# tumaer/lagrangebench

Measured on AMD Instinct MI355X. Metric: rollout particle-steps/sec, higher is better.
Workload: dtype f32 (GEMMs as fp16 hi/lo split products, fp32 accumulate)

## Files before the change

include/lbhip.h:

```cpp
#ifndef LBHIP_H
#define LBHIP_H

#include <stdint.h>

#ifdef __cplusplus
extern "C" {
#endif

#define LB_OK 0
#define LB_ERR_ARG (-1)
#define LB_ERR_HIP (-2)
#define LB_ERR_STATE (-3)
#define LB_ERR_DENSITY (-4)
#define LB_ERR_UNSUPPORTED (-5)

#define LB_FORCE_NONE 0
#define LB_FORCE_PIECEWISE 1
#define LB_FORCE_BUFFER 2

typedef struct lb_engine lb_engine;
typedef struct lb_gns lb_gns;

typedef struct lb_case_desc {
  int32_t dim;
  int32_t n_particles;
  int32_t batch;
  int32_t isl;
  int32_t periodic;
  int32_t has_bound;
  int32_t has_vel_mag;
  int32_t force_kind;
  int32_t force_axis;
  int32_t geometry_f32;
  double box[3];
  double r_cutoff;
  double capacity_multiplier;
  double vel_mean[3], vel_std[3], acc_mean[3], acc_std[3];
  double bound_lo[3], bound_hi[3];
  double force_split;
  double force_lo[3], force_hi[3];
} lb_case_desc;

typedef struct lb_gns_desc {
  int32_t latent_size;
  int32_t blocks_per_step;
  int32_t num_mp_steps;
  int32_t embedding_size;
  int32_t num_particle_types;
  int32_t node_in;
  int32_t edge_in;
  int32_t out_dim;
} lb_gns_desc;

const char* lb_strerror(int code);
const char* lb_last_error(void);
int lb_version(void);


int lb_engine_create(const lb_case_desc* desc, void* hip_stream, lb_engine** out);
void lb_engine_destroy(lb_engine* eng);

int lb_set_particle_type(lb_engine* eng, const int32_t* ptype_dev);

int lb_set_force(lb_engine* eng, const double* force_dev);

int lb_load_window(lb_engine* eng, const double* traj_dev, int32_t T, int32_t t0, int32_t step);

#define LB_TRAIN_BATCH_MAX 128
int lb_train_batch(lb_engine* eng, const void* pos_dev, int32_t pos_is_f64, const int32_t* ptype_dev, int32_t n_traj,
                   int32_t seq_len, const int32_t* traj_host, const int32_t* t0_host, const int32_t* slot_host,
                   uint64_t seed, int64_t step, double noise_std, int32_t T, int32_t unroll_steps, double* traj_out_dev,
                   int32_t* ptype_out_dev, double* target_acc_dev, double* target_vel_dev, double* target_pos_dev,
                   double* want_normals_dev);

int lb_read_window(lb_engine* eng, double* win_out_dev);


int lb_nl_allocate(lb_engine* eng, int32_t* cell_capacity_out, int32_t* e_cap_out,
                   int32_t* occupancy_out );

int lb_nl_set_capacity(lb_engine* eng, int32_t cell_capacity, int32_t e_cap);

int lb_nl_update(lb_engine* eng);

int lb_nl_read_flags(lb_engine* eng, int32_t* overflow_out_dev);

int lb_nl_read_idx(lb_engine* eng, int32_t* idx_out_dev, int32_t* n_edges_out_dev);


int lb_node_features(lb_engine* eng, double* vel_hist_out_dev, double* vel_mag_out_dev,
                     double* bound_out_dev, double* force_out_dev);

int lb_edge_features(lb_engine* eng, double* rel_disp_out_dev, double* rel_dist_out_dev);


int lb_gns_create(lb_engine* eng, const lb_gns_desc* desc, const float* weights_host,
                  int64_t n_floats, lb_gns** out);
void lb_gns_destroy(lb_gns* gns);

int lb_gns_forward(lb_engine* eng, lb_gns* gns, float* acc_out_dev);

int lb_set_fused_aggregation(lb_engine* eng, int32_t on);

int lb_gns_set_tap(lb_gns* gns, float* node_latents_out_dev);


int lb_integrate(lb_engine* eng, const float* acc_dev, const double* target_dev,
                 double* pred_out_dev, int32_t pred_T);

int lb_case_integrate(lb_engine* eng, int32_t mode, const float* pred_dev, const double* pos_seq_dev,
                      int32_t T, double* next_out_dev);

int lb_rollout(lb_engine* eng, lb_gns* gns, const double* traj_dev, int32_t T, int32_t n_steps,
               double* pred_out_dev, int32_t* n_realloc_out);


typedef struct lb_gns_train lb_gns_train;
int lb_gns_train_create(lb_engine* eng, const lb_gns_desc* desc, const float* weights_host, int64_t n_floats,
                        lb_gns_train** out);
void lb_gns_train_destroy(lb_gns_train* t);
int lb_gns_train_loss_grad(lb_gns_train* t, const float* target_dev, float loss_weight, double* loss_out,
                           float* pred_out_dev);
int lb_gns_train_zero_grad(lb_gns_train* t);
int lb_adamw_step(lb_gns_train* t, float lr, float b1, float b2, float eps, float weight_decay);
int lb_gns_train_read(lb_gns_train* t, int32_t which, float* out_host, int64_t n_floats);
int lb_gns_train_write(lb_gns_train* t, int32_t which, const float* in_host, int64_t n_floats, int64_t step);
int64_t lb_gns_train_step_count(lb_gns_train* t);
int lb_gns_train_device_blob(lb_gns_train* t, int32_t which, float** dev_out, int64_t* n_floats_out);
int lb_adamw_step_gathered(lb_gns_train* t, const float* gathered_dev, int32_t world, float grad_scale, float lr,
                           float b1, float b2, float eps, float weight_decay);
int32_t lb_gns_train_math_fallbacks(lb_gns_train* t);
int32_t lb_gns_train_sort_fallbacks(lb_gns_train* t);

int lb_train_forward(lb_gns_train* t, float* pred_out_dev);
int lb_train_backward(lb_gns_train* t, const float* dpred_dev, double* dpos_out_dev);
int lb_train_exact_math(lb_gns_train* t, int32_t exact);

int lb_gns_train_sync_model(lb_gns_train* t, lb_gns* g);
int64_t lb_gns_image_bytes(lb_gns* g);
int lb_gns_image_read(lb_gns* g, void* out_host, int64_t n_bytes);
int64_t lb_gns_pack_selftest(const lb_gns_desc* desc, int32_t node_in_kq, const float* weights_host, int64_t n_floats,
                             int64_t* n_bytes_out);

typedef struct lb_segnn lb_segnn;

typedef struct lb_segnn_desc {
  int32_t hidden;
  int32_t blocks_per_step;
  int32_t num_mp_steps;
  int32_t homogeneous;
  int32_t n_vels;
  int32_t velocity_avg;
  int32_t lmax_hidden;
  int32_t lmax_attributes;
  int32_t norm;
  float norm_eps;
} lb_segnn_desc;

int lb_segnn_create(lb_engine* eng, const lb_segnn_desc* desc, const float* weights_host,
                    int64_t n_floats, lb_segnn** out);

int lb_segnn_train_create(lb_engine* eng, const lb_segnn_desc* desc, const float* weights_host, int64_t n_floats,
                          lb_gns_train** out);
int lb_segnn_train_loss_grad(lb_gns_train* t, const float* target_dev, float loss_weight, double* loss_out,
                             float* pred_out_dev);
void lb_segnn_destroy(lb_segnn* segnn);

int lb_segnn_forward(lb_engine* eng, lb_segnn* segnn, float* acc_out_dev);

typedef struct lb_egnn lb_egnn;
typedef struct lb_egnn_desc {
  int32_t hidden;
  int32_t num_mp_steps;
  int32_t n_vels;
  int32_t homogeneous;
  int32_t residual;
  int32_t normalize;
  int32_t tanh_pos;
} lb_egnn_desc;

int lb_egnn_create(lb_engine* eng, const lb_egnn_desc* desc, const float* weights_host, int64_t n_floats,
                   lb_egnn** out);
void lb_egnn_destroy(lb_egnn* egnn);
int lb_egnn_forward(lb_engine* eng, lb_egnn* egnn, double* pos_out_dev);
int lb_egnn_set_tap(lb_egnn* egnn, float* h_out_dev, float* pos_out_dev);
int lb_egnn_rollout(lb_engine* eng, lb_egnn* egnn, const double* traj_dev, int32_t T, int32_t n_steps,
                    double* pred_out_dev, int32_t* n_realloc_out);

int lb_egnn_train_create(lb_engine* eng, const lb_egnn_desc* desc, const float* weights_host, int64_t n_floats,
                         lb_gns_train** out);
int lb_egnn_train_loss_grad(lb_gns_train* t, const double* tgt_pos, const double* tgt_vel, const double* tgt_acc,
                            float w_pos, float w_vel, float w_acc, double* loss_out, float* pred_pos_out_dev);
int lb_egnn_train_model(lb_gns_train* t, lb_egnn** out);

typedef struct lb_painn lb_painn;
typedef struct lb_painn_desc {
  int32_t hidden;
  int32_t num_mp_steps;
  int32_t n_vels;
  int32_t homogeneous;
  int32_t shared_filters;
  int32_t shared_interactions;
  int32_t n_rbf;
  int32_t has_cutoff;
  float cutoff;
} lb_painn_desc;

int lb_painn_create(lb_engine* eng, const lb_painn_desc* desc, const float* weights_host, int64_t n_floats,
                    lb_painn** out);
void lb_painn_destroy(lb_painn* painn);
int lb_painn_forward(lb_engine* eng, lb_painn* painn, float* acc_out_dev);
int lb_painn_set_tap(lb_painn* painn, float* s_out_dev, float* v_out_dev);
int lb_painn_rollout(lb_engine* eng, lb_painn* painn, const double* traj_dev, int32_t T, int32_t n_steps,
                     double* pred_out_dev, int32_t* n_realloc_out);

int lb_painn_train_create(lb_engine* eng, const lb_painn_desc* desc, const float* weights_host, int64_t n_floats,
                          int32_t rbf_trainable, lb_gns_train** out);
int lb_painn_train_model(lb_gns_train* t, lb_painn** out);

typedef struct lb_linear lb_linear;
typedef struct lb_linear_desc {
  int32_t n_in;
  int32_t out_dim;
} lb_linear_desc;

int lb_linear_create(lb_engine* eng, const lb_linear_desc* desc, const float* weights_host, int64_t n_floats,
                     lb_linear** out);
void lb_linear_destroy(lb_linear* linear);
int lb_linear_forward(lb_engine* eng, lb_linear* linear, float* acc_out_dev);
int lb_linear_rollout(lb_engine* eng, lb_linear* linear, const double* traj_dev, int32_t T, int32_t n_steps,
                      double* pred_out_dev, int32_t* n_realloc_out);
int lb_linear_train_create(lb_engine* eng, const lb_linear_desc* desc, const float* weights_host, int64_t n_floats,
                           lb_gns_train** out);
int lb_linear_train_model(lb_gns_train* t, lb_linear** out);

int lb_blob_train_create(lb_engine* eng, const float* weights_host, int64_t n_floats, lb_gns_train** out);

int lb_math_mode(lb_engine* eng, int32_t set_mode, int32_t* mode_out, int32_t* flags_out);

int32_t lb_math_fallbacks(lb_engine* eng);

int lb_debug_inject_guard(lb_engine* eng, int32_t flags, int32_t step);

int lb_segnn_set_tap(lb_segnn* segnn, float* hidden_out_dev);
int32_t lb_segnn_row_floats(lb_segnn* segnn);

int lb_segnn_rollout(lb_engine* eng, lb_segnn* segnn, const double* traj_dev, int32_t T,
                     int32_t n_steps, double* pred_out_dev, int32_t* n_realloc_out);

int lb_metrics(lb_engine* eng, const double* pred_dev, int32_t pred_T, const double* target_dev,
               int32_t target_T, int32_t n_steps, double* mse_out_dev, double* mae_out_dev);

int lb_ekin(lb_engine* eng, const double* rollout_dev, int32_t T, int32_t stride, double dt, double dx,
            double* out_dev, int32_t n_out);

int lb_sinkhorn(lb_engine* eng, const double* pred_dev, int32_t pred_T, const double* target_dev,
                int32_t target_T, int32_t stride, double threshold, double* out_dev, int32_t n_out,
                int32_t* iters_out_host);

int lb_sinkhorn_pot(lb_engine* eng, const double* pred_dev, int32_t pred_T, const double* target_dev,
                    int32_t target_T, int32_t stride, double reg, int32_t num_iter_max, double stop_thr,
                    double* out_dev, int32_t n_out, int32_t* info_out_host);


int lb_timers_enable(lb_engine* eng, int32_t on);
int lb_timers_reset(lb_engine* eng);
int32_t lb_timer_count(void);
const char* lb_timer_name(int32_t cls);
int lb_timer_get(lb_engine* eng, int32_t cls, double* ms_out, int64_t* launches_out);

int lb_stats(lb_engine* eng, int64_t* n_edges_total, int32_t* e_cap, int32_t* cell_capacity);

int lb_edge_accounting(lb_engine* eng, int64_t* sum_edges, int64_t* n_builds, int64_t* first_edges, int64_t* last_edges,
                       int32_t reset);

int lb_kernel_names(lb_engine* eng, char* out, int32_t cap);

int lb_segment_sum(lb_engine* eng, const float* msg_dev, float* out_dev, int32_t D);

int lb_graph_gather(lb_engine* eng, int32_t role, const float* x_dev , float* out_dev , int32_t C);
int lb_graph_segment_sum(lb_engine* eng, int32_t role, const float* msg_dev , float* out_dev ,
                         int32_t C);
int lb_graph_degree(lb_engine* eng, int32_t role, int32_t* out_dev );
int lb_graph_segment_max(lb_engine* eng, int32_t role, const float* msg_dev , float* out_dev ,
                         int32_t* win_dev , int32_t C);
int lb_graph_segment_min(lb_engine* eng, int32_t role, const float* msg_dev , float* out_dev ,
                         int32_t* win_dev , int32_t C);
int lb_graph_segment_max_backward(lb_engine* eng, int32_t role, const float* d_out_dev ,
                                  const int32_t* win_dev , float* d_msg_dev , int32_t C);
int lb_graph_segment_softmax(lb_engine* eng, int32_t role, const float* logits_dev ,
                             float* out_dev , int32_t C);
int lb_graph_segment_softmax_backward(lb_engine* eng, int32_t role, const float* y_dev ,
                                      const float* d_y_dev , float* d_x_dev , int32_t C);
int lb_graph_attend(lb_engine* eng, int32_t role, const float* logits_dev ,
                    const float* values_dev , float* out_dev , float* m_dev ,
// ... 11 lines not shown
```

lagrangebench_amd/_lib.py:

```python
from __future__ import annotations

import ctypes as C
import os
from typing import Optional

_HERE = os.path.dirname(os.path.abspath(__file__))
LIB_PATH = os.path.join(_HERE, "csrc", "liblbhip.so")

LB_OK = 0
LB_FORCE_NONE, LB_FORCE_PIECEWISE, LB_FORCE_BUFFER = 0, 1, 2
LB_TRAIN_BATCH_MAX = 128

D3 = C.c_double * 3


class CaseDesc(C.Structure):

    _fields_ = [
        ("dim", C.c_int32), ("n_particles", C.c_int32), ("batch", C.c_int32), ("isl", C.c_int32),
        ("periodic", C.c_int32), ("has_bound", C.c_int32), ("has_vel_mag", C.c_int32),
        ("force_kind", C.c_int32), ("force_axis", C.c_int32), ("geometry_f32", C.c_int32),
        ("box", D3), ("r_cutoff", C.c_double), ("capacity_multiplier", C.c_double),
        ("vel_mean", D3), ("vel_std", D3), ("acc_mean", D3), ("acc_std", D3),
        ("bound_lo", D3), ("bound_hi", D3),
        ("force_split", C.c_double), ("force_lo", D3), ("force_hi", D3),
    ]


class GnsDesc(C.Structure):

    _fields_ = [
        ("latent_size", C.c_int32), ("blocks_per_step", C.c_int32), ("num_mp_steps", C.c_int32),
        ("embedding_size", C.c_int32), ("num_particle_types", C.c_int32), ("node_in", C.c_int32),
        ("edge_in", C.c_int32), ("out_dim", C.c_int32),
    ]


class SegnnDesc(C.Structure):

    _fields_ = [
        ("hidden", C.c_int32), ("blocks_per_step", C.c_int32), ("num_mp_steps", C.c_int32),
        ("homogeneous", C.c_int32), ("n_vels", C.c_int32), ("velocity_avg", C.c_int32),
        ("lmax_hidden", C.c_int32), ("lmax_attributes", C.c_int32), ("norm", C.c_int32), ("norm_eps", C.c_float),
    ]

    def __init__(self, *args, **kw):
        super().__init__(*args, **kw)
        if "lmax_hidden" not in kw and len(args) < 7:
            self.lmax_hidden = 1
        if "lmax_attributes" not in kw and len(args) < 8:
            self.lmax_attributes = 1


class EgnnDesc(C.Structure):

    _fields_ = [
        ("hidden", C.c_int32), ("num_mp_steps", C.c_int32), ("n_vels", C.c_int32), ("homogeneous", C.c_int32),
        ("residual", C.c_int32), ("normalize", C.c_int32), ("tanh_pos", C.c_int32),
    ]


class PainnDesc(C.Structure):

    _fields_ = [
        ("hidden", C.c_int32), ("num_mp_steps", C.c_int32), ("n_vels", C.c_int32), ("homogeneous", C.c_int32),
        ("shared_filters", C.c_int32), ("shared_interactions", C.c_int32), ("n_rbf", C.c_int32),
        ("has_cutoff", C.c_int32), ("cutoff", C.c_float),
    ]


class LinearDesc(C.Structure):

    _fields_ = [("n_in", C.c_int32), ("out_dim", C.c_int32)]


_P = C.c_void_p
_SIGS = {
    "lb_strerror": (C.c_char_p, [C.c_int]),
    "lb_last_error": (C.c_char_p, []),
    "lb_version": (C.c_int, []),
    "lb_engine_create": (C.c_int, [C.POINTER(CaseDesc), _P, C.POINTER(_P)]),
    "lb_engine_destroy": (None, [_P]),
    "lb_set_particle_type": (C.c_int, [_P, _P]),
    "lb_set_force": (C.c_int, [_P, _P]),
    "lb_load_window": (C.c_int, [_P, _P, C.c_int32, C.c_int32, C.c_int32]),
    "lb_train_batch": (C.c_int, [_P, _P, C.c_int32, _P, C.c_int32, C.c_int32, C.POINTER(C.c_int32), C.POINTER(C.c_int32),
                                 C.POINTER(C.c_int32), C.c_uint64, C.c_int64, C.c_double, C.c_int32, C.c_int32, _P, _P, _P, _P, _P,
                                 _P]),
    "lb_read_window": (C.c_int, [_P, _P]),
    "lb_nl_allocate": (C.c_int, [_P, C.POINTER(C.c_int32), C.POINTER(C.c_int32), C.POINTER(C.c_int32)]),
    "lb_nl_set_capacity": (C.c_int, [_P, C.c_int32, C.c_int32]),
    "lb_nl_update": (C.c_int, [_P]),
    "lb_nl_read_flags": (C.c_int, [_P, _P]),
    "lb_nl_read_idx": (C.c_int, [_P, _P, _P]),
    "lb_node_features": (C.c_int, [_P, _P, _P, _P, _P]),
    "lb_edge_features": (C.c_int, [_P, _P, _P]),
    "lb_gns_create": (C.c_int, [_P, C.POINTER(GnsDesc), _P, C.c_int64, C.POINTER(_P)]),
    "lb_gns_destroy": (None, [_P]),
    "lb_gns_forward": (C.c_int, [_P, _P, _P]),
    "lb_set_fused_aggregation": (C.c_int, [_P, C.c_int32]),
    "lb_gns_set_tap": (C.c_int, [_P, _P]),
    "lb_math_mode": (C.c_int, [_P, C.c_int32, C.POINTER(C.c_int32), C.POINTER(C.c_int32)]),
    "lb_math_fallbacks": (C.c_int32, [_P]),
    "lb_debug_inject_guard": (C.c_int, [_P, C.c_int32, C.c_int32]),
    "lb_integrate": (C.c_int, [_P, _P, _P, _P, C.c_int32]),
    "lb_case_integrate": (C.c_int, [_P, C.c_int32, _P, _P, C.c_int32, _P]),
    "lb_rollout": (C.c_int, [_P, _P, _P, C.c_int32, C.c_int32, _P, C.POINTER(C.c_int32)]),
    "lb_ekin": (C.c_int, [_P, _P, C.c_int32, C.c_int32, C.c_double, C.c_double, _P, C.c_int32]),
    "lb_sinkhorn": (C.c_int, [_P, _P, C.c_int32, _P, C.c_int32, C.c_int32, C.c_double, _P, C.c_int32, _P]),
    "lb_sinkhorn_pot": (C.c_int, [_P, _P, C.c_int32, _P, C.c_int32, C.c_int32, C.c_double, C.c_int32, C.c_double, _P,
                                  C.c_int32, _P]),
    "lb_metrics": (C.c_int, [_P, _P, C.c_int32, _P, C.c_int32, C.c_int32, _P, _P]),
    "lb_timers_enable": (C.c_int, [_P, C.c_int32]),
    "lb_timers_reset": (C.c_int, [_P]),
    "lb_timer_count": (C.c_int32, []),
    "lb_timer_name": (C.c_char_p, [C.c_int32]),
    "lb_timer_get": (C.c_int, [_P, C.c_int32, C.POINTER(C.c_double), C.POINTER(C.c_int64)]),
    "lb_stats": (C.c_int, [_P, C.POINTER(C.c_int64), C.POINTER(C.c_int32), C.POINTER(C.c_int32)]),
    "lb_edge_accounting": (C.c_int, [_P, C.POINTER(C.c_int64), C.POINTER(C.c_int64), C.POINTER(C.c_int64),
                                     C.POINTER(C.c_int64), C.c_int32]),
    "lb_kernel_names": (C.c_int, [_P, C.c_char_p, C.c_int32]),
    "lb_gns_train_create": (C.c_int, [_P, C.POINTER(GnsDesc), C.POINTER(C.c_float), C.c_int64, C.POINTER(_P)]),
    "lb_gns_train_destroy": (None, [_P]),
    "lb_gns_train_loss_grad": (C.c_int, [_P, _P, C.c_float, C.POINTER(C.c_double), _P]),
    "lb_gns_train_zero_grad": (C.c_int, [_P]),
    "lb_adamw_step": (C.c_int, [_P, C.c_float, C.c_float, C.c_float, C.c_float, C.c_float]),
    "lb_gns_train_read": (C.c_int, [_P, C.c_int32, C.POINTER(C.c_float), C.c_int64]),
    "lb_gns_train_write": (C.c_int, [_P, C.c_int32, C.POINTER(C.c_float), C.c_int64, C.c_int64]),
    "lb_gns_train_step_count": (C.c_int64, [_P]),
    "lb_gns_train_device_blob": (C.c_int, [_P, C.c_int32, C.POINTER(_P), C.POINTER(C.c_int64)]),
    "lb_adamw_step_gathered": (C.c_int, [_P, _P, C.c_int32, C.c_float, C.c_float, C.c_float, C.c_float, C.c_float,
                                         C.c_float]),
    "lb_gns_train_math_fallbacks": (C.c_int32, [_P]),
    "lb_gns_train_sort_fallbacks": (C.c_int32, [_P]),
    "lb_train_forward": (C.c_int, [_P, _P]),
    "lb_train_backward": (C.c_int, [_P, _P, _P]),
    "lb_train_exact_math": (C.c_int, [_P, C.c_int32]),
    "lb_gns_train_sync_model": (C.c_int, [_P, _P]),
    "lb_gns_image_bytes": (C.c_int64, [_P]),
    "lb_gns_image_read": (C.c_int, [_P, _P, C.c_int64]),
    "lb_gns_pack_selftest": (C.c_int64, [C.POINTER(GnsDesc), C.c_int32, C.POINTER(C.c_float), C.c_int64, C.POINTER(C.c_int64)]),
    "lb_segnn_train_create": (C.c_int, [_P, C.POINTER(SegnnDesc), C.POINTER(C.c_float), C.c_int64, C.POINTER(_P)]),
    "lb_segnn_train_loss_grad": (C.c_int, [_P, _P, C.c_float, C.POINTER(C.c_double), _P]),
    "lb_segment_sum": (C.c_int, [_P, _P, _P, C.c_int32]),
    "lb_segnn_create": (C.c_int, [_P, C.POINTER(SegnnDesc), _P, C.c_int64, C.POINTER(_P)]),
    "lb_segnn_destroy": (None, [_P]),
    "lb_segnn_forward": (C.c_int, [_P, _P, _P]),
    "lb_segnn_row_floats": (C.c_int32, [_P]),
    "lb_segnn_set_tap": (C.c_int, [_P, _P]),
    "lb_segnn_rollout": (C.c_int, [_P, _P, _P, C.c_int32, C.c_int32, _P, C.POINTER(C.c_int32)]),
    "lb_egnn_create": (C.c_int, [_P, C.POINTER(EgnnDesc), C.POINTER(C.c_float), C.c_int64, C.POINTER(_P)]),
    "lb_egnn_destroy": (None, [_P]),
    "lb_egnn_forward": (C.c_int, [_P, _P, _P]),
    "lb_egnn_set_tap": (C.c_int, [_P, _P, _P]),
    "lb_egnn_rollout": (C.c_int, [_P, _P, _P, C.c_int32, C.c_int32, _P, C.POINTER(C.c_int32)]),
    "lb_egnn_train_create": (C.c_int, [_P, C.POINTER(EgnnDesc), C.POINTER(C.c_float), C.c_int64, C.POINTER(_P)]),
    "lb_egnn_train_loss_grad": (C.c_int, [_P, _P, _P, _P, C.c_float, C.c_float, C.c_float, C.POINTER(C.c_double), _P]),
    "lb_egnn_train_model": (C.c_int, [_P, C.POINTER(_P)]),
    "lb_painn_create": (C.c_int, [_P, C.POINTER(PainnDesc), C.POINTER(C.c_float), C.c_int64, C.POINTER(_P)]),
    "lb_painn_destroy": (None, [_P]),
    "lb_painn_forward": (C.c_int, [_P, _P, _P]),
    "lb_painn_set_tap": (C.c_int, [_P, _P, _P]),
    "lb_painn_rollout": (C.c_int, [_P, _P, _P, C.c_int32, C.c_int32, _P, C.POINTER(C.c_int32)]),
    "lb_painn_train_create": (C.c_int, [_P, C.POINTER(PainnDesc), C.POINTER(C.c_float), C.c_int64, C.c_int32, C.POINTER(_P)]),
    "lb_painn_train_model": (C.c_int, [_P, C.POINTER(_P)]),
    "lb_linear_create": (C.c_int, [_P, C.POINTER(LinearDesc), C.POINTER(C.c_float), C.c_int64, C.POINTER(_P)]),
    "lb_linear_destroy": (None, [_P]),
    "lb_linear_forward": (C.c_int, [_P, _P, _P]),
    "lb_linear_rollout": (C.c_int, [_P, _P, _P, C.c_int32, C.c_int32, _P, C.POINTER(C.c_int32)]),
    "lb_linear_train_create": (C.c_int, [_P, C.POINTER(LinearDesc), C.POINTER(C.c_float), C.c_int64, C.POINTER(_P)]),
    "lb_linear_train_model": (C.c_int, [_P, C.POINTER(_P)]),
    "lb_blob_train_create": (C.c_int, [_P, C.POINTER(C.c_float), C.c_int64, C.POINTER(_P)]),
    "lb_graph_gather": (C.c_int, [_P, C.c_int32, _P, _P, C.c_int32]),
    "lb_graph_segment_sum": (C.c_int, [_P, C.c_int32, _P, _P, C.c_int32]),
    "lb_graph_sender_sorts": (C.c_int32, [_P]),
    "lb_graph_degree": (C.c_int, [_P, C.c_int32, _P]),
    "lb_graph_segment_max": (C.c_int, [_P, C.c_int32, _P, _P, _P, C.c_int32]),
    "lb_graph_segment_min": (C.c_int, [_P, C.c_int32, _P, _P, _P, C.c_int32]),
    "lb_graph_segment_max_backward": (C.c_int, [_P, C.c_int32, _P, _P, _P, C.c_int32]),
    "lb_graph_segment_softmax": (C.c_int, [_P, C.c_int32, _P, _P, C.c_int32]),
    "lb_graph_segment_softmax_backward": (C.c_int, [_P, C.c_int32, _P, _P, _P, C.c_int32]),
    "lb_graph_attend": (C.c_int, [_P, C.c_int32, _P, _P, _P, _P, _P, C.c_int32, C.c_int32]),
    "lb_graph_attend_backward": (C.c_int, [_P, C.c_int32, _P, _P, _P, _P, _P, _P, _P, C.c_int32, C.c_int32]),
}

_lib: Optional[C.CDLL] = None


class LbHipError(RuntimeError):
    pass


def load() -> C.CDLL:
    global _lib
    if _lib is not None:
        return _lib
    if not os.path.exists(LIB_PATH):
        raise LbHipError(
            f"{LIB_PATH} not found: the HIP engine is not built. Run "
            "`python -m lagrangebench_amd.build` (needs hipcc). There is no CPU fallback."
        )
    lib = C.CDLL(LIB_PATH)
    for name, (res, args) in _SIGS.items():
        fn = getattr(lib, name)
        fn.restype = res
        fn.argtypes = args
    _lib = lib
    return lib


def check(rc: int, what: str = "") -> None:
    if rc != LB_OK:
        lib = load()
        msg = lib.lb_last_error().decode() or lib.lb_strerror(rc).decode()
        raise LbHipError(f"{what or 'liblbhip'} failed ({rc}: {lib.lb_strerror(rc).decode()}): {msg}")


def ptr(t) -> int:
    if t is None:
        return None
    return t.data_ptr()
```

lagrangebench_amd/csrc/lb_edge16.hip:

```cpp
#include <stdlib.h>
#include <string.h>

#include "lb_device.h"
#include "lb_gns_repack.h"

#define MFMA16(a, b, c) __builtin_amdgcn_mfma_f32_16x16x4f32((a), (b), (c), 0, 0, 0)

typedef _Float16 h8 __attribute__((ext_vector_type(8)));
#define MFMA16H(a, b, c) __builtin_amdgcn_mfma_f32_16x16x32_f16((a), (b), (c), 0, 0, 0)


void lb_pack_weight16h(const float* w, int K, int M, int Kpad, float* out, int Mpad) {
  uint16_t* o = reinterpret_cast<uint16_t*>(out);
  const int NP = Kpad / 32, NMBO = Mpad / 16;
  for (int p = 0; p < NP; ++p)
    for (int mbo = 0; mbo < NMBO; ++mbo)
      for (int lane = 0; lane < 64; ++lane)
        for (int i = 0; i < 8; ++i) {
          const int g = lane >> 4;
          const int k = 32 * p + (i < 4 ? 4 * g + i : 16 + 4 * g + (i - 4));
          const int m = 16 * mbo + (lane & 15);
          const float x = (k < K && m < M) ? w[(size_t)k * M + m] : 0.f;
          const uint16_t hi = lb_f32_to_f16_rne(x);
          const uint16_t lo = lb_f32_to_f16_rne(x - lb_f16_to_f32(hi));
// ... 85 lines not shown
      a0 = n0;
      a1 = n1;
      __builtin_amdgcn_sched_barrier(0);
    }
  }
}

template <bool PROC, bool F16, int ABL = 0>
__global__ void __launch_bounds__(E16_THREADS, 2) k_edge16(lb_edge16_args a) {
  constexpr int NW0 = PROC ? 4096 : (F16 ? 1024 : 512);
  __shared__ f32x4 sW[NW0 + 4096 + 128];
  if (a.ctrl->overflow_step >= 0) return;
  const int tid = threadIdx.x;
  {
    const f32x4* g0 = reinterpret_cast<const f32x4*>(a.w0p);
    const f32x4* g1 = reinterpret_cast<const f32x4*>(a.w1p);
    for (int i = tid; i < NW0; i += E16_THREADS) sW[i] = g0[i];
    for (int i = tid; i < 4096; i += E16_THREADS) sW[NW0 + i] = g1[i];
    if (tid < 128) {
      const float* src = tid < 32 ? a.b1 : (tid < 64 ? a.ln_s : (tid < 96 ? a.ln_o : a.b0));
      sW[NW0 + 4096 + tid] = src ? reinterpret_cast<const f32x4*>(src)[tid & 31] : f32x4{0.f, 0.f, 0.f, 0.f};
    }
  }
  __syncthreads();
  const int E = a.ctrl->n_edges_total;
  const int ntiles = (E + 15) >> 4;
  const int lane = tid & 63, wave = tid >> 6;
  const int n = lane & 15, g = lane >> 4;
  const int xcd = blockIdx.x & 7, slot = (blockIdx.x >> 3) * E16_WAVES + wave;
  const int stride = (gridDim.x >> 3) * E16_WAVES;
  const int t_lo = (int)(((int64_t)ntiles * xcd) >> 3), t_hi = (int)(((int64_t)ntiles * (xcd + 1)) >> 3);
  int t = t_lo + slot;
  if (t >= t_hi) return;

  auto ld0 = [&](int step, int hf) -> f32x4 { return sW[(step * 2 + hf) * 64 + lane]; };
  auto ld1 = [&](int step, int hf) -> f32x4 { return sW[NW0 + (step * 2 + hf) * 64 + lane]; };
  auto ldh0 = [&](int p, int mbo, int part) -> f32x4 { return sW[((p * 8 + mbo) * 2 + part) * 64 + lane]; };
  auto ldh1 = [&](int p, int mbo, int part) -> f32x4 {
    return sW[NW0 + ((p * 8 + mbo) * 2 + part) * 64 + lane];
  };
  auto rowc_of = [&](int tt) -> int64_t {
    const int row = tt * 16 + n;
    return row < E ? row : E - 1;
  };
  const f32x4* psr4 = reinterpret_cast<const f32x4*>(a.psr);
  const f32x4* b1_4 = &sW[NW0 + 4096];
  const f32x4* lns4 = &sW[NW0 + 4096 + 32];
  const f32x4* lno4 = &sW[NW0 + 4096 + 64];
  const f32x4* b0_4 = &sW[NW0 + 4096 + 96];

  const int n_iter = (t_hi - 1 - t) / stride + 1;
  const int t_last = t + (n_iter - 1) * stride;
  f32x4 ve_n[8], ps_n[8], pr_n[8];
  f32x4 vin_n = {0.f, 0.f, 0.f, 0.f};
  int s_n = 0, r_n = 0, r_pref = 0;
  auto issue = [&](int tt, int s, int r) {
    const int64_t rc = rowc_of(tt);
    if (PROC) {
      const f32x4* er = reinterpret_cast<const f32x4*>(a.elat) + (int64_t)tt * 512 + lane;
      const f32x4* ps = psr4 + (int64_t)s * 64 + g;
      const f32x4* pr = psr4 + (int64_t)r * 64 + 32 + g;
#pragma unroll
      for (int mb = 0; mb < 8; ++mb) {
        ve_n[mb] = (ABL & 2) ? f32x4{1.f, 2.f, (float)rc, (float)mb} : er[64 * mb];
        ps_n[mb] = (ABL & 1) ? f32x4{.1f, .2f, (float)s, (float)mb} : ps[4 * mb];
        pr_n[mb] = (ABL & 1) ? f32x4{.3f, .1f, (float)r, (float)mb} : pr[4 * mb];
      }
    } else {
      vin_n = reinterpret_cast<const f32x4*>(a.efeat)[rc * 2 + (g & 1)];
    }
  };
  {
    const int64_t rc = rowc_of(t);
    int s0 = 0, r0 = 0;
    if (PROC) {
      s0 = a.senders[rc];
      r0 = a.receivers[rc];
    }
    issue(t, s0, r0);
    r_pref = r0;
    if (PROC) {
      const int64_t rn = rowc_of(min(t + stride, t_last));
      s_n = a.senders[rn];
      r_n = a.receivers[rn];
    }
  }

  for (int it = 0; it < n_iter; ++it, t += stride) {
    f32x4 acc[8], ve[8];
    f32x4 vin[1];
    const int r_cur = r_pref;
    if (PROC) {
#pragma unroll
      for (int mb = 0; mb < 8; ++mb) {
        ve[mb] = ve_n[mb];
        acc[mb] = ps_n[mb] + pr_n[mb];
      }
    } else {
      vin[0] = (g < 2) ? vin_n : f32x4{0.f, 0.f, 0.f, 0.f};
#pragma unroll
      for (int mb = 0; mb < 8; ++mb) acc[mb] = b0_4[4 * mb + g];
    }
    issue(min(t + stride, t_last), s_n, r_n);
    r_pref = r_n;
    if (PROC) {
      const int64_t rn = rowc_of(min(t + 2 * stride, t_last));
      s_n = a.senders[rn];
      r_n = a.receivers[rn];
    }
    if constexpr (ABL & 32) {
    } else if constexpr (F16) {
      if constexpr (PROC) {
        lb_gemm16h<4>(ldh0, ve, acc);
      } else {
        f32x4 vin2[2] = {vin[0], f32x4{0.f, 0.f, 0.f, 0.f}};
        lb_gemm16h<1>(ldh0, vin2, acc);
      }
    } else {
      if (PROC)
        lb_gemm16<8>(ld0, ve, acc);
      else
        lb_gemm16<1>(ld0, vin, acc);
    }
#pragma unroll
    for (int mb = 0; mb < 8; ++mb)
#pragma unroll
      for (int j = 0; j < 4; ++j) acc[mb][j] = fmaxf(acc[mb][j], 0.f);
    f32x4 acc2[8];
#pragma unroll
    for (int mb = 0; mb < 8; ++mb) acc2[mb] = b1_4[4 * mb + g];
    if constexpr (ABL & 16) {
#pragma unroll
      for (int mb = 0; mb < 8; ++mb) acc2[mb] = acc2[mb] + acc[mb];
    } else if constexpr (F16)
      lb_gemm16h<4>(ldh1, acc, acc2);
    else
      lb_gemm16<8>(ld1, acc, acc2);
    float sm = 0.f;
#pragma unroll
    for (int mb = 0; mb < 8; ++mb) sm += (acc2[mb][0] + acc2[mb][1]) + (acc2[mb][2] + acc2[mb][3]);
    sm += __shfl_xor(sm, 16);
    sm += __shfl_xor(sm, 32);
    const float mean = sm * a.ctrl->ln_inv_d;
    float vs = 0.f;
#pragma unroll
    for (int mb = 0; mb < 8; ++mb)
#pragma unroll
      for (int j = 0; j < 4; ++j) {
        const float d = acc2[mb][j] - mean;
        vs += d * d;
      }
    vs += __shfl_xor(vs, 16);
    vs += __shfl_xor(vs, 32);
    const float rs = 1.0f / sqrtf(fmaxf(vs - a.ctrl->ln_pad * (mean * mean), 0.f) * a.ctrl->ln_inv_d + 1e-5f);
    f32x4 y[8];
#pragma unroll
    for (int mb = 0; mb < 8; ++mb) {
      const f32x4 sc = lns4[4 * mb + g], of = lno4[4 * mb + g];
#pragma unroll
      for (int j = 0; j < 4; ++j)
        y[mb][j] = (ABL & 8) ? acc2[mb][j] : (sc[j] * rs) * (acc2[mb][j] - mean) + of[j];
    }
    const int row = t * 16 + n;
    const bool valid = row < E;
    const bool do_store = !((ABL & 4) && a.row_ptr[0] != -12345);
    if (do_store) {
      f32x4* er = reinterpret_cast<f32x4*>(a.elat) + (int64_t)t * 512 + lane;
      if (PROC) {
        if (!a.skip_elat_store) {
#pragma unroll
          for (int mb = 0; mb < 8; ++mb) er[64 * mb] = ve[mb] + y[mb];
        }
        if (!a.fused && valid) {
          f32x4* mr = reinterpret_cast<f32x4*>(a.msg) + (int64_t)row * 32 + g;
#pragma unroll
          for (int mb = 0; mb < 8; ++mb) mr[4 * mb] = y[mb];
        }
      } else {
#pragma unroll
        for (int mb = 0; mb < 8; ++mb) er[64 * mb] = y[mb];
      }
    }
    if (PROC && a.fused && !(ABL & 64)) {
      const int rr = valid ? r_cur : (-1 - n);
      const int r_prev = __builtin_amdgcn_update_dpp(-2, rr, 0x111, 0xF, 0xF, false);
      const bool head = (n == 0) || (rr != r_prev);
      const unsigned H = (unsigned)(__ballot(head) & 0xffffull);
      const unsigned below = H & ((2u << n) - 1u);
      const int segstart = 31 - __clz(below);
      const bool tail = (n == 15) || ((H >> (n + 1)) & 1u);
      const float m1 = (n >= 1 && segstart <= n - 1) ? 1.f : 0.f, m2 = (n >= 2 && segstart <= n - 2) ? 1.f : 0.f;
      const float m4 = (n >= 4 && segstart <= n - 4) ? 1.f : 0.f, m8 = (n >= 8 && segstart <= n - 8) ? 1.f : 0.f;
#pragma unroll
      for (int mb = 0; mb < 8; ++mb)
#pragma unroll
        for (int j = 0; j < 4; ++j) {
          float x = valid ? y[mb][j] : 0.f;
          x = __builtin_fmaf(__builtin_bit_cast(float, __builtin_amdgcn_update_dpp(0, __builtin_bit_cast(int, x), 0x111, 0xF, 0xF, true)), m1, x);
          x = __builtin_fmaf(__builtin_bit_cast(float, __builtin_amdgcn_update_dpp(0, __builtin_bit_cast(int, x), 0x112, 0xF, 0xF, true)), m2, x);
          x = __builtin_fmaf(__builtin_bit_cast(float, __builtin_amdgcn_update_dpp(0, __builtin_bit_cast(int, x), 0x114, 0xF, 0xF, true)), m4, x);
          x = __builtin_fmaf(__builtin_bit_cast(float, __builtin_amdgcn_update_dpp(0, __builtin_bit_cast(int, x), 0x118, 0xF, 0xF, true)), m8, x);
          y[mb][j] = x;
        }
      if (tail && valid && do_store) {
        const int k0 = a.row_ptr[rr], k1 = a.row_ptr[rr + 1];
        const bool complete = (k0 >> 4) == ((k1 - 1) >> 4);
        float* dst = complete ? a.agg + (int64_t)rr * 128
                              : a.part + ((int64_t)t * 2 + (k0 <= t * 16 ? 0 : 1)) * 128;
        f32x4* d4 = reinterpret_cast<f32x4*>(dst) + g;
#pragma unroll
        for (int mb = 0; mb < 8; ++mb) d4[4 * mb] = y[mb];
      }
    }
  }
}

int lbk_edge16(lb_engine* e, const lb_edge16_args& a, bool proc, bool f16x2) {
  if (proc && f16x2)
    hipLaunchKernelGGL((k_edge16<true, true>), dim3(256), dim3(E16_THREADS), 0, e->stream, a);
  else if (proc)
    hipLaunchKernelGGL((k_edge16<true, false>), dim3(256), dim3(E16_THREADS), 0, e->stream, a);
  else
    hipLaunchKernelGGL((k_edge16<false, false>), dim3(256), dim3(E16_THREADS), 0, e->stream, a);
  LB_HIP(hipGetLastError());
  return LB_OK;
}
```

lagrangebench_amd/csrc/lb_edge16v.hip:

```cpp
#include <stdlib.h>

#include "lb_f16x2.h"

template <int WPS, bool RELOAD, bool SKIP, int ABL = 0, bool PRIO = false, bool NT = true, int GUARD = 0, bool TICKET = false>
__global__ void __launch_bounds__(WPS * 256, WPS) k_edge16v(lb_edge16_args a) {
  constexpr int THREADS = WPS * 256, WAVES = WPS * 4;
  constexpr int NW0 = 4096;
  __shared__ f32x4 sW[NW0 + 4096 + 96];
  __shared__ int s_ticket;
  const int poisoned = a.ctrl->overflow_step;
  const int E = a.ctrl->n_edges_total;
  const float ln_inv_d = a.ctrl->ln_inv_d, ln_pad = a.ctrl->ln_pad;
  const int tid = threadIdx.x;
  constexpr int NST = (NW0 + 4096 + THREADS - 1) / THREADS;
  f32x4 st[NST];
  {
    const f32x4* g0 = reinterpret_cast<const f32x4*>(a.w0p);
    const f32x4* g1 = reinterpret_cast<const f32x4*>(a.w1p);
#pragma unroll
    for (int k = 0; k < NST; ++k) {
      const int i = tid + k * THREADS;
      st[k] = i < NW0 ? g0[i] : g1[(i < NW0 + 4096 ? i : NW0 + 4095) - NW0];
    }
  }
  const int ntiles = (E + 15) >> 4;
  const int lane = tid & 63, wave = __builtin_amdgcn_readfirstlane(tid >> 6);
  const int n = lane & 15, g = lane >> 4;
  const int xcd = blockIdx.x & 7;
  int stride = (gridDim.x >> 3) * WAVES;
  int t_lo = (int)(((int64_t)ntiles * xcd) >> 3), t_hi = (int)(((int64_t)ntiles * (xcd + 1)) >> 3);
  int t = t_lo + (blockIdx.x >> 3) * WAVES + wave;
  if constexpr (TICKET) {
    stride = gridDim.x >> 3;
    t_lo += (blockIdx.x >> 3);
    t = t_lo + wave * stride;
  }
  auto rowc_of = [&](int tt) -> int64_t {
    const int row = tt * 16 + n;
    return row < E ? row : (E > 0 ? E - 1 : 0);
  };
  int s_c = 0, r_c = 0;
  if (t < t_hi) {
    const int64_t rc = rowc_of(t);
    s_c = a.senders[rc];
    r_c = a.receivers[rc];
  }
  if (poisoned >= 0) return;
  {
#pragma unroll
    for (int k = 0; k < NST; ++k) {
      const int i = tid + k * THREADS;
      if (i < NW0 + 4096) sW[i] = st[k];
    }
    if (tid < 96) {
      const float* src = tid < 32 ? a.b1 : (tid < 64 ? a.ln_s : a.ln_o);
      sW[NW0 + 4096 + tid] = reinterpret_cast<const f32x4*>(src)[tid & 31];
    }
    if (TICKET && tid == 0) s_ticket = WAVES;
  }
  __syncthreads();
  if (t >= t_hi) return;
  uint32_t off0 = (uint32_t)(uintptr_t)(lds_cptr)(sW + lane);
  uint32_t off1 = (uint32_t)(uintptr_t)(lds_cptr)(sW + NW0 + lane);
  uint32_t off2 = (uint32_t)(uintptr_t)(lds_cptr)(sW + NW0 + 4096 + g);
  asm volatile("" : "+v"(off0), "+v"(off1), "+v"(off2));
  const lds_cptr w0b = (lds_cptr)(uintptr_t)off0, w1b = (lds_cptr)(uintptr_t)off1, vecb = (lds_cptr)(uintptr_t)off2;
  const f32x4* psr4 = reinterpret_cast<const f32x4*>(a.psr);
  const int n_iter = TICKET ? 0x7fffffff : (t_hi - 1 - t) / stride + 1;
  const int t_last = TICKET ? t_hi - 1 : t + (n_iter - 1) * stride;
  asm volatile("" : "+v"(s_c), "+v"(r_c));
  int guard_tiny = 0;
  for (int it = 0; it < n_iter && t < t_hi; ++it) {
    int t_next = t + stride;
    if constexpr (TICKET) {
      int k = 0;
      if (lane == 0) k = atomicAdd(&s_ticket, 1);
      t_next = t_lo + __builtin_amdgcn_readfirstlane(k) * stride;
    }
    f32x4 acc[8], ve[8];
    const int r_cur = r_c;
    const f32x4* er = reinterpret_cast<const f32x4*>(a.elat) + (int64_t)t * 512 + lane;
    {
      const f32x4* ps = psr4 + (int64_t)s_c * 64 + g;
      const f32x4* pr = psr4 + (int64_t)r_c * 64 + 32 + g;
      f32x4 p0[8];
#pragma unroll
      for (int mb = 0; mb < 8; ++mb) {
        ve[mb] = (ABL & 2) ? f32x4{1.f, 2.f, (float)(t & 1023), (float)mb}
                           : ((RELOAD || !NT) ? er[64 * mb] : __builtin_nontemporal_load(&er[64 * mb]));
        p0[mb] = (ABL & 1) ? f32x4{.1f, .2f, (float)(s_c & 255), (float)mb} : ps[4 * mb];
        acc[mb] = (ABL & 1) ? f32x4{.3f, .1f, (float)(r_c & 255), (float)mb} : pr[4 * mb];
      }
      const int64_t rn = rowc_of(min(t_next, t_last));
      s_c = a.senders[rn];
      r_c = a.receivers[rn];
#pragma unroll
      for (int mb = 0; mb < 8; ++mb) acc[mb] = lb_pk_add(acc[mb], p0[mb]);
    }
    int rb = lb_edge_probe(a.receivers, t, lane, E);
    if (it == 0) lb_range_probe(a.ctrl, ve, 8);
    if constexpr (PRIO) __builtin_amdgcn_s_setprio(2);
    uint32_t or_e = 0, or_h = 0;
    if constexpr (!(ABL & 8)) lb_gemm16v<false, 4, GUARD>(w0b, ve, acc, &or_e);
    if (it == 0) lb_range_probe(a.ctrl, acc, 8);
    f32x4 acc2[8];
#pragma unroll
    for (int mb = 0; mb < 8; ++mb) acc2[mb] = vecb[4 * mb];
    if constexpr (!(ABL & 8)) {
      lb_gemm16v<true, 4, GUARD>(w1b, acc, acc2, &or_h);
      if constexpr (PRIO) __builtin_amdgcn_s_setprio(0);
      if constexpr (GUARD == 2) guard_tiny |= (int)lb_tile_tiny(or_e) | (int)lb_tile_tiny(or_h);
      if constexpr (GUARD != 0) guard_tiny |= (int)lb_rows_tiny(or_e) | (int)lb_rows_tiny(or_h);
    } else {
#pragma unroll
      for (int mb = 0; mb < 8; ++mb)
#pragma unroll
        for (int j = 0; j < 4; ++j) acc2[mb][j] += acc[mb][j] + ve[mb][j];
    }
    if constexpr (RELOAD && !SKIP && !(ABL & 2)) {
#pragma unroll
      for (int mb = 0; mb < 8; ++mb) ve[mb] = er[64 * mb];
    }
    asm volatile("" : "+v"(s_c), "+v"(r_c), "+v"(rb));
    f32x4 y[8];
    lb_layernorm16<!(ABL & 16)>(acc2, vecb + 32, vecb + 64, y, ln_inv_d, ln_pad);
    const int row = t * 16 + n;
    const bool valid = row < E;
    if constexpr (!SKIP && !(ABL & 4)) {
      f32x4* ew = reinterpret_cast<f32x4*>(a.elat_out ? a.elat_out : a.elat) + (int64_t)t * 512 + lane;
#pragma unroll
      for (int mb = 0; mb < 8; ++mb) {
        if constexpr (NT)
          __builtin_nontemporal_store(lb_pk_add(ve[mb], y[mb]), &ew[64 * mb]);
        else
          ew[64 * mb] = lb_pk_add(ve[mb], y[mb]);
      }
    }
    const int rr = valid ? r_cur : (-1 - n);
    const int r_prev = __builtin_amdgcn_update_dpp(-2, rr, 0x111, 0xF, 0xF, false);
    const bool head = (n == 0) || (rr != r_prev);
    const unsigned H = (unsigned)(__ballot(head) & 0xffffull);
    const unsigned below = H & ((2u << n) - 1u);
    const int segstart = 31 - __clz(below);
    const bool tail = (n == 15) || ((H >> (n + 1)) & 1u);
    const float m1 = (n >= 1 && segstart <= n - 1) ? 1.f : 0.f, m2 = (n >= 2 && segstart <= n - 2) ? 1.f : 0.f;
    const float m4 = (n >= 4 && segstart <= n - 4) ? 1.f : 0.f, m8 = (n >= 8 && segstart <= n - 8) ? 1.f : 0.f;
    if (!valid) {
#pragma unroll
      for (int mb = 0; mb < 8; ++mb) y[mb] = f32x4{0.f, 0.f, 0.f, 0.f};
    }
    if constexpr (!(ABL & 16))
#pragma unroll
    for (int mb = 0; mb < 8; mb += 2) lb_scan8(y[mb], y[mb + 1], m1, m2, m4, m8);
    if (tail && valid && !(ABL & 4)) {
      int slot01;
      const bool complete = lb_seg_complete(rb, rr, segstart, n, t, E, slot01);
      float* dst = complete ? a.agg + (int64_t)rr * 128 : a.part + ((int64_t)t * 2 + slot01) * 128;
      f32x4* d4 = reinterpret_cast<f32x4*>(dst) + g;
#pragma unroll
      for (int mb = 0; mb < 8; ++mb) d4[4 * mb] = y[mb];
    }
    t = t_next;
  }
  if (guard_tiny && lane == 0) lb_raise_math(a.ctrl, LB_MATH_TINY);
}

template <int WPS>
__global__ void __launch_bounds__(WPS * 256, WPS) k_edge_enc16v(lb_edge16_args a) {
  constexpr int THREADS = WPS * 256, WAVES = WPS * 4;
  constexpr int NW0 = 1024;
  __shared__ f32x4 sW[NW0 + 4096 + 128];
  const int poisoned = a.ctrl->overflow_step;
  const int E = a.ctrl->n_edges_total;
  const int tid = threadIdx.x;
  {
    const f32x4* g0 = reinterpret_cast<const f32x4*>(a.w0p);
    const f32x4* g1 = reinterpret_cast<const f32x4*>(a.w1p);
    for (int i = tid; i < NW0; i += THREADS) sW[i] = g0[i];
    for (int i = tid; i < 4096; i += THREADS) sW[NW0 + i] = g1[i];
    if (tid < 128) {
      const float* src = tid < 32 ? a.b1 : (tid < 64 ? a.ln_s : (tid < 96 ? a.ln_o : a.b0));
      sW[NW0 + 4096 + tid] = reinterpret_cast<const f32x4*>(src)[tid & 31];
    }
  }
  if (poisoned >= 0) return;
  __syncthreads();
  const float ln_inv_d = a.ctrl->ln_inv_d, ln_pad = a.ctrl->ln_pad;
  const int ntiles = (E + 15) >> 4;
  const int lane = tid & 63, wave = __builtin_amdgcn_readfirstlane(tid >> 6);
  const int n = lane & 15, g = lane >> 4;
  const int xcd = blockIdx.x & 7, slot = (blockIdx.x >> 3) * WAVES + wave;
  const int stride = (gridDim.x >> 3) * WAVES;
  const int t_lo = (int)(((int64_t)ntiles * xcd) >> 3), t_hi = (int)(((int64_t)ntiles * (xcd + 1)) >> 3);
  int t = t_lo + slot;
  if (t >= t_hi) return;
  const lds_cptr w0b = (lds_cptr)(sW + lane), w1b = (lds_cptr)(sW + NW0 + lane);
  const lds_cptr vecb = (lds_cptr)(sW + NW0 + 4096 + g);
  const f32x4* ef4 = reinterpret_cast<const f32x4*>(a.efeat);
  const f32x4 zero = {0.f, 0.f, 0.f, 0.f};
  auto feat_of = [&](int tt) -> f32x4 {
    const int row = tt * 16 + n;
    const int64_t rc = row < E ? row : E - 1;
    return ef4[rc * 2 + (g & 1)];
  };
  const int n_iter = (t_hi - 1 - t) / stride + 1;
  const int t_last = t + (n_iter - 1) * stride;
  f32x4 f_n = feat_of(t);
  asm volatile("" : "+v"(f_n));
  for (int it = 0; it < n_iter; ++it, t += stride) {
    const f32x4 v2[2] = {g < 2 ? f_n : zero, zero};
    f_n = feat_of(min(t + stride, t_last));
    f32x4 acc[8], acc2[8];
#pragma unroll
    for (int mb = 0; mb < 8; ++mb) acc[mb] = vecb[96 + 4 * mb];
    lb_gemm16v<false, 1>(w0b, v2, acc);
    if (it == 0) lb_range_probe(a.ctrl, acc, 8);
#pragma unroll
    for (int mb = 0; mb < 8; ++mb) acc2[mb] = vecb[4 * mb];
    lb_gemm16v<true>(w1b, acc, acc2);
    asm volatile("" : "+v"(f_n));
    f32x4 y[8];
    lb_layernorm16<true>(acc2, vecb + 32, vecb + 64, y, ln_inv_d, ln_pad);
    f32x4* ew = reinterpret_cast<f32x4*>(a.elat) + (int64_t)t * 512 + lane;
#pragma unroll
    for (int mb = 0; mb < 8; ++mb) __builtin_nontemporal_store(y[mb], &ew[64 * mb]);
  }
}

int lbk_edge_enc16v(lb_engine* e, const lb_edge16_args& a) {
  const int64_t tiles_cap = ((int64_t)e->e_cap * e->g.B + 15) / 16;
  auto grid_for = [&](int waves_per_block) {
    int64_t g = (tiles_cap + waves_per_block - 1) / waves_per_block;
    g = (g + 7) / 8 * 8;
    return (int)(g < 8 ? 8 : (g > 256 ? 256 : g));
  };
  if (tiles_cap <= 256 * 8 * 2)
    hipLaunchKernelGGL((k_edge_enc16v<2>), dim3(grid_for(8)), dim3(512), 0, e->stream, a);
  else
    hipLaunchKernelGGL((k_edge_enc16v<4>), dim3(256), dim3(1024), 0, e->stream, a);
  LB_HIP(hipGetLastError());
  return LB_OK;
}

int lbk_edge16v(lb_engine* e, const lb_edge16_args& a) {
  const bool small = ((int64_t)e->e_cap * e->g.B + 15) / 16 < 12288;
#define LB_E16V__(NT, G, GU, TK)                                                                        \
  do {                                                                                                  \
    if (a.skip_elat_store)                                                                              \
      LB_LAUNCH_TIMED(e, (k_edge16v<2, false, true, 0, true, NT, GU, TK>), dim3(G), dim3(512), a);      \
    else                                                                                                \
      LB_LAUNCH_TIMED(e, (k_edge16v<2, false, false, 0, true, NT, GU, TK>), dim3(G), dim3(512), a);     \
  } while (0)
#define LB_E16V(NT, G, TK)                       \
  do {                                           \
    if (e->guard_full)                           \
      LB_E16V__(NT, G, 2, TK);                   \
    else if (e->math_auto && !e->guard_sampled)  \
      LB_E16V__(NT, G, 1, TK);                   \
    else                                         \
      LB_E16V__(NT, G, 0, TK);                   \
  } while (0)
  const int64_t tiles_cap = ((int64_t)e->e_cap * e->g.B + 15) / 16;
  int64_t g = (tiles_cap + 7) / 8;
  g = (g + 7) / 8 * 8;
  const int grid = (int)(g < 8 ? 8 : (g > 256 ? 256 : g));
  if (small)
    LB_E16V(false, grid, true);
  else
    LB_E16V(true, grid, false);
#undef LB_E16V
#undef LB_E16V__
  LB_HIP(hipGetLastError());
  return LB_OK;
}
```

lagrangebench_amd/csrc/lb_edge16w.hip:

```cpp
#include <stdlib.h>

#include <type_traits>

#include "lb_f16x2.h"

typedef uint32_t u32x4w __attribute__((ext_vector_type(4)));

__device__ __forceinline__ const f32x4* ew_at(const void* base, uint32_t off) {
  return reinterpret_cast<const f32x4*>(reinterpret_cast<const char*>(base) + off);
}
__device__ __forceinline__ f32x4* ew_at(void* base, uint32_t off) {
  return reinterpret_cast<f32x4*>(reinterpret_cast<char*>(base) + off);
}

struct ew_tile {
  f32x4 a[8];
  f32x4 ve[8];
  int t;
  int r_cur;
  int rb;
  uint32_t or_e, or_h;
};

struct ew_ctx {
  lds_cptr vecb;
  float ln_inv_d, ln_pad;
  int E, n, g, lane;
  float* elat_out;
  __amdgpu_buffer_rsrc_t out_rs;
  uint32_t part_off;
};

struct ew_tmp {
  f32x2v tmp, s2, v2, m2, r2, dl, dh, tlo, thi, ylo, olo, ohi;
  float sm, mean, vs, rs;
  f32x4 scn, ofn, scc, ofc;
  int rr, segstart;
  bool valid, head, tail;
  unsigned H;
  float m1, m2f, m4, m8;
  uint32_t ew;
  uint32_t off;
};

__device__ __forceinline__ float ew_rowsum4(float x) {
  float p = x, q = x;
  asm volatile("s_nop 1\n\tv_permlane16_swap_b32 %0, %1\n\ts_nop 1" : "+v"(p), "+v"(q));
  p = q = p + q;
  asm volatile("s_nop 1\n\tv_permlane32_swap_b32 %0, %1\n\ts_nop 1" : "+v"(p), "+v"(q));
  return p + q;
}


#ifndef EW_SCALAR_LN
#define EW_SCALAR_LN 0
#endif
__device__ __forceinline__ f32x2v ew_add2(f32x2v a, f32x2v b) {
#if EW_SCALAR_LN
  return f32x2v{a[0] + b[0], a[1] + b[1]};
#else
  return a + b;
#endif
}
__device__ __forceinline__ f32x2v ew_sub2(f32x2v a, f32x2v b) {
#if EW_SCALAR_LN
  return f32x2v{a[0] - b[0], a[1] - b[1]};
#else
  return a - b;
#endif
}
__device__ __forceinline__ f32x2v ew_mul2(f32x2v a, f32x2v b) {
#if EW_SCALAR_LN
  return f32x2v{a[0] * b[0], a[1] * b[1]};
#else
  return a * b;
#endif
}
__device__ __forceinline__ f32x2v ew_fma2(f32x2v a, f32x2v b, f32x2v c) {
#if EW_SCALAR_LN
  return f32x2v{__builtin_fmaf(a[0], b[0], c[0]), __builtin_fmaf(a[1], b[1], c[1])};
#else
  return __builtin_elementwise_fma(a, b, c);
#endif
}
template <bool SKIP, int GUARD>
struct ew_plan {
  static constexpr int A0 = 0;
  static constexpr int A1 = A0 + 16;
  static constexpr int B0 = A1 + 3;
  static constexpr int B1 = B0 + 32;
  static constexpr int C0 = B1 + 3;
  static constexpr int D0 = C0 + 48;
  static constexpr int E0 = D0 + (SKIP ? 0 : 25);
  static constexpr int F0 = E0 + 6;
  static constexpr int G0 = F0 + 64;
  static constexpr int H0 = G0 + 9;
  static constexpr int M = H0 + (GUARD ? 1 : 0);
};

#define EW_DPP2(SHR, Y0, Y1, MSK)                                                                     \
  asm volatile("s_nop 1\n\t"                                                                          \
               "v_fmac_f32_dpp %0, %0, %2 row_shr:" #SHR " row_mask:0xf bank_mask:0xf bound_ctrl:1\n\t" \
               "v_fmac_f32_dpp %1, %1, %2 row_shr:" #SHR " row_mask:0xf bank_mask:0xf bound_ctrl:1"      \
               : "+v"(Y0), "+v"(Y1)                                                                   \
               : "v"(MSK))

template <bool SKIP, bool NT, int GUARD, bool PIPE = true>
__device__ __forceinline__ void ew_op(int k, ew_tile& P, ew_tmp& T, const ew_ctx& C, int& guard_tiny) {
  using PL = ew_plan<SKIP, GUARD>;
  if (k < PL::A1) {
    const int mb = k >> 1;
    if (!(k & 1))
      T.tmp = ew_add2(lb_lo2(P.a[mb]), lb_hi2(P.a[mb]));
    else
      T.s2 = mb == 0 ? T.tmp : ew_add2(T.s2, T.tmp);
  } else if (k < PL::B0) {
    const int j = k - PL::A1;
    if (j == 0)
      T.sm = T.s2[0] + T.s2[1];
    else if (j == 1)
      T.sm = ew_rowsum4(T.sm);
    else {
      T.mean = T.sm * C.ln_inv_d;
      T.m2 = f32x2v{T.mean, T.mean};
    }
  } else if (k < PL::B1) {
    const int j = k - PL::B0, mb = j >> 2, sub = j & 3;
    if (sub == 0)
      T.dl = ew_sub2(lb_lo2(P.a[mb]), T.m2);
    else if (sub == 1)
      T.dh = ew_sub2(lb_hi2(P.a[mb]), T.m2);
    else if (sub == 2)
      T.v2 = mb == 0 ? ew_mul2(T.dl, T.dl) : ew_fma2(T.dl, T.dl, T.v2);
    else {
      T.v2 = ew_fma2(T.dh, T.dh, T.v2);
      P.a[mb] = lb_cat2(T.dl, T.dh);
    }
  } else if (k < PL::C0) {
    const int j = k - PL::B1;
    if (j == 0) {
      T.vs = T.v2[0] + T.v2[1];
      if constexpr (PIPE) T.scn = C.vecb[32];
    } else if (j == 1) {
      T.vs = ew_rowsum4(T.vs);
      if constexpr (PIPE) T.ofn = C.vecb[64];
    } else {
      T.rs = 1.0f / sqrtf(fmaxf(T.vs - C.ln_pad * (T.mean * T.mean), 0.f) * C.ln_inv_d + 1e-5f);
      T.r2 = f32x2v{T.rs, T.rs};
    }
  } else if (k < PL::D0) {
    const int j = k - PL::C0, mb = j / 6, sub = j % 6;
    if (sub == 0) {
      if constexpr (PIPE) {
        T.scc = T.scn;
        if (mb < 7) T.scn = C.vecb[32 + 4 * (mb + 1)];
      } else {
        T.scc = C.vecb[32 + 4 * mb];
      }
    } else if (sub == 1) {
      if constexpr (PIPE) {
        T.ofc = T.ofn;
        if (mb < 7) T.ofn = C.vecb[64 + 4 * (mb + 1)];
      } else {
        T.ofc = C.vecb[64 + 4 * mb];
      }
    } else if (sub == 2)
      T.tlo = ew_mul2(lb_lo2(T.scc), T.r2);
    else if (sub == 3)
      T.thi = ew_mul2(lb_hi2(T.scc), T.r2);
    else if (sub == 4)
      T.ylo = ew_fma2(T.tlo, lb_lo2(P.a[mb]), lb_lo2(T.ofc));
    else
      P.a[mb] = lb_cat2(T.ylo, ew_fma2(T.thi, lb_hi2(P.a[mb]), lb_hi2(T.ofc)));
  } else if (!SKIP && k < PL::E0) {
    const int j = k - PL::D0;
    if (j == 0) {
      T.ew = (uint32_t)P.t * 8192u + (uint32_t)C.lane * 16u;
    } else {
      const int q = j - 1, mb = q / 3, sub = q % 3;
      if (sub == 0)
        T.olo = ew_add2(lb_lo2(P.ve[mb]), lb_lo2(P.a[mb]));
      else if (sub == 1)
        T.ohi = ew_add2(lb_hi2(P.ve[mb]), lb_hi2(P.a[mb]));
      else {
        const f32x4 o = lb_cat2(T.olo, T.ohi);
        if constexpr (NT)
          __builtin_nontemporal_store(o, ew_at(C.elat_out, T.ew) + 64 * mb);
        else
          ew_at(C.elat_out, T.ew)[64 * mb] = o;
      }
    }
  } else if (k < PL::F0) {
    const int j = k - PL::E0, n = C.n;
    if (j == 0) {
      T.valid = P.t * 16 + n < C.E;
      T.rr = T.valid ? P.r_cur : (-1 - n);
    } else if (j == 1) {
      const int r_prev = __builtin_amdgcn_update_dpp(-2, T.rr, 0x111, 0xF, 0xF, false);
      T.head = (n == 0) || (T.rr != r_prev);
    } else if (j == 2) {
      T.H = (unsigned)(__ballot(T.head) & 0xffffull);
      T.segstart = 31 - __clz(T.H & ((2u << n) - 1u));
    } else if (j == 3) {
      T.tail = (n == 15) || ((T.H >> (n + 1)) & 1u);
    } else if (j == 4) {
      T.m1 = (n >= 1 && T.segstart <= n - 1) ? 1.f : 0.f;
      T.m2f = (n >= 2 && T.segstart <= n - 2) ? 1.f : 0.f;
    } else {
      T.m4 = (n >= 4 && T.segstart <= n - 4) ? 1.f : 0.f;
      T.m8 = (n >= 8 && T.segstart <= n - 8) ? 1.f : 0.f;
    }
  } else if (k < PL::G0) {
    const int j = k - PL::F0, grp = j >> 4, step = (j >> 2) & 3, r = 2 * (j & 3) + 8 * grp;
    if constexpr (!PIPE) {
      if ((j & 15) == 0) lb_scan8(P.a[2 * grp], P.a[2 * grp + 1], T.m1, T.m2f, T.m4, T.m8);
    } else if (step == 0)
      EW_DPP2(1, P.a[r >> 2][r & 3], P.a[(r + 1) >> 2][(r + 1) & 3], T.m1);
    else if (step == 1)
      EW_DPP2(2, P.a[r >> 2][r & 3], P.a[(r + 1) >> 2][(r + 1) & 3], T.m2f);
    else if (step == 2)
      EW_DPP2(4, P.a[r >> 2][r & 3], P.a[(r + 1) >> 2][(r + 1) & 3], T.m4);
    else
      EW_DPP2(8, P.a[r >> 2][r & 3], P.a[(r + 1) >> 2][(r + 1) & 3], T.m8);
  } else if (k < PL::H0) {
    const int j = k - PL::G0;
    if (j == 0) {
      int slot01;
      const bool complete = lb_seg_complete(P.rb, T.rr, T.segstart, C.n, P.t, C.E, slot01);
      const uint32_t row_off =
          complete ? (uint32_t)T.rr * 512u : C.part_off + ((uint32_t)P.t * 2u + (uint32_t)slot01) * 512u;
      T.off = (T.tail && T.valid) ? row_off + (uint32_t)C.g * 16u : 0x80000000u;
    } else {
      const int mb = j - 1;
      __builtin_amdgcn_raw_buffer_store_b128(__builtin_bit_cast(u32x4w, P.a[mb]), C.out_rs, (int)T.off, 64 * mb, 0);
    }
  } else if (GUARD != 0 && k < PL::M) {
    guard_tiny |= (int)lb_rows_tiny(P.or_e) | (int)lb_rows_tiny(P.or_h);
  }
}

template <int DF, int M>
__device__ __forceinline__ constexpr int ew_slot_lo(int s) { return DF + (s * (M - DF)) / 192; }

template <bool RELU, int GUARD, int S0, typename F>
__device__ __forceinline__ void ew_gemm(lds_cptr wbase, const f32x4 (&v)[8], f32x4 (&acc)[8], uint32_t* orv, F&& fill) {
  constexpr int NP = 4;
  auto frag = [&](int p, int mbo, int part) -> h8 {
    return __builtin_bit_cast(h8, wbase[((p * 8 + mbo) * 2 + part) * 64]);
  };
  h8 X[4], Y[4];
  h8 bh, bl;
  lb_split_regs R;
#pragma unroll
  for (int c = 0; c < 4; ++c) X[c] = frag(0, c, 1);
#pragma unroll
  for (int c = 0; c < 4; ++c) Y[c] = frag(0, c, 0);
  {
    f32x4 a0 = v[0], a1 = v[1];
    if constexpr (RELU) {
#pragma unroll
      for (int j = 0; j < 4; ++j) {
        const float f0 = a0[j], f1 = a1[j];
        a0[j] = __builtin_bit_cast(float, max(__builtin_bit_cast(int, f0), 0));
        a1[j] = __builtin_bit_cast(float, max(__builtin_bit_cast(int, f1), 0));
      }
    }
    lb_split8v(a0, a1, bh, bl);
    if constexpr (GUARD != 0) {
      const u32x4w u = __builtin_bit_cast(u32x4w, bh);
      *orv |= (u[0] | u[1]) | (u[2] | u[3]);
    }
  }
  SB();
#pragma unroll
  for (int blk = 0; blk < 2 * NP; ++blk) {
    const int p = blk >> 1, q = blk & 1;
    const int np = (blk + 1) >> 1, nq = (blk + 1) & 1;
    const bool fs = p < NP - 1;
    const int s0 = 12 * q, sl = S0 + 12 * blk;
    f32x4* a4 = &acc[4 * q];
    __builtin_amdgcn_s_waitcnt(LB_WAIT_LGKM(4));
#pragma unroll
    for (int c = 0; c < 4; ++c) {
      a4[c] = MFMA16H(X[c], bh, a4[c]);
      if (fs) lb_split_slot<RELU, GUARD>(s0 + c, v[2 * p + 2], v[2 * p + 3], R, orv);
      fill(sl + c);
      SB();
    }
    if (blk < 2 * NP - 1) {
#pragma unroll
      for (int c = 0; c < 4; ++c) X[c] = frag(np, 4 * nq + c, 1);
    }
    if (blk < 2 * NP - 1)
      __builtin_amdgcn_s_waitcnt(LB_WAIT_LGKM(4));
    else
      __builtin_amdgcn_s_waitcnt(LB_WAIT_LGKM(0));
#pragma unroll
    for (int c = 0; c < 4; ++c) {
      a4[c] = MFMA16H(Y[c], bl, a4[c]);
      if (fs) lb_split_slot<RELU, GUARD>(s0 + 4 + c, v[2 * p + 2], v[2 * p + 3], R, orv);
      fill(sl + 4 + c);
      SB();
    }
#pragma unroll
    for (int c = 0; c < 4; ++c) {
      a4[c] = MFMA16H(Y[c], bh, a4[c]);
      if (fs) lb_split_slot<RELU, GUARD>(s0 + 8 + c, v[2 * p + 2], v[2 * p + 3], R, orv);
      fill(sl + 8 + c);
      SB();
    }
    if (blk < 2 * NP - 1) {
#pragma unroll
      for (int c = 0; c < 4; ++c) Y[c] = frag(np, 4 * nq + c, 0);
    }
    if (q == 1 && fs) {
      bh = __builtin_bit_cast(h8, u32x4w{R.H[0], R.H[1], R.H[2], R.H[3]});
      bl = __builtin_bit_cast(h8, u32x4w{R.L[0], R.L[1], R.L[2], R.L[3]});
    }
    SB();
  }
}

template <bool SKIP, bool NT, int GUARD, bool TICKET, int DEFER = 1, int ABL = 0, int WPS = 2, int PF = 0, int WALK = 0>
__global__ void __launch_bounds__(WPS * 256, 1) k_edge16w(lb_edge16_args a) {
  static_assert(PF == 0 || PF == 2, "PF: 0 or 2");
  static_assert(!(PF == 2 && DEFER == 2 && !SKIP), "DEEP prefetch overwrites the previous tile's latents");
  constexpr int THREADS = WPS * 256, WAVES = WPS * 4;
  constexpr int NW0 = 4096;
  using PL = ew_plan<SKIP, GUARD>;
  constexpr int DF = DEFER == 2 ? 0 : (DEFER == 1 ? PL::E0 : PL::M);
  __shared__ f32x4 sW[NW0 + 4096 + 96];
  __shared__ int s_ticket;
  const int poisoned = a.ctrl->overflow_step;
  const int E = a.ctrl->n_edges_total;
  const float ln_inv_d = a.ctrl->ln_inv_d, ln_pad = a.ctrl->ln_pad;
  const int tid = threadIdx.x;
  constexpr int NST = (NW0 + 4096 + THREADS - 1) / THREADS;
  f32x4 st[NST];
  {
    const f32x4* g0 = reinterpret_cast<const f32x4*>(a.w0p);
    const f32x4* g1 = reinterpret_cast<const f32x4*>(a.w1p);
#pragma unroll
    for (int k = 0; k < NST; ++k) {
      const int i = tid + k * THREADS;
      st[k] = i < NW0 ? g0[i] : g1[(i < NW0 + 4096 ? i : NW0 + 4095) - NW0];
    }
  }
  const int ntiles = (E + 15) >> 4;
  const int lane = tid & 63, wave = __builtin_amdgcn_readfirstlane(tid >> 6);
  const int n = lane & 15, g = lane >> 4;
  const int xcd = blockIdx.x & 7;
  int stride = (gridDim.x >> 3) * WAVES;
  int t_lo = (int)(((int64_t)ntiles * xcd) >> 3), t_hi = (int)(((int64_t)ntiles * (xcd + 1)) >> 3);
  int t = t_lo + (blockIdx.x >> 3) * WAVES + wave;
  if constexpr (TICKET) {
    stride = gridDim.x >> 3;
    t_lo += (blockIdx.x >> 3);
    t = t_lo + wave * stride;
  }
  auto rowc_of = [&](int tt) -> int64_t {
    const int row = tt * 16 + n;
    return row < E ? row : (E > 0 ? E - 1 : 0);
  };
  const int t_lo0 = (int)(((int64_t)ntiles * xcd) >> 3);
  const int rev_sum = a.reverse ? t_lo0 + t_hi - 1 : 0;
  if constexpr (WALK == 1) {
    const int slot = (blockIdx.x >> 3) * WAVES + wave, nslot = (gridDim.x >> 3) * WAVES, ntx = t_hi - t_lo0;
    t = t_lo0 + (int)(((int64_t)ntx * slot) / nslot);
    t_hi = t_lo0 + (int)(((int64_t)ntx * (slot + 1)) / nslot);
    stride = 1;
  }
  auto tmap = [&](int tw) -> int { return a.reverse ? rev_sum - tw : tw; };
  int s_c = 0, r_c = 0;
  if (t < t_hi) {
    const int64_t rc = rowc_of(tmap(t));
    s_c = a.senders[rc];
    r_c = a.receivers[rc];
  }
  if (poisoned >= 0) return;
  {
#pragma unroll
    for (int k = 0; k < NST; ++k) {
      const int i = tid + k * THREADS;
      if (i < NW0 + 4096) sW[i] = st[k];
    }
    if (tid < 96) {
      const float* src = tid < 32 ? a.b1 : (tid < 64 ? a.ln_s : a.ln_o);
      sW[NW0 + 4096 + tid] = reinterpret_cast<const f32x4*>(src)[tid & 31];
    }
    if (TICKET && tid == 0) s_ticket = WAVES;
  }
  __syncthreads();
  if (t >= t_hi) return;
  uint32_t off0 = (uint32_t)(uintptr_t)(lds_cptr)(sW + lane);
  uint32_t off1 = (uint32_t)(uintptr_t)(lds_cptr)(sW + NW0 + lane);
  uint32_t off2 = (uint32_t)(uintptr_t)(lds_cptr)(sW + NW0 + 4096 + g);
  asm volatile("" : "+v"(off0), "+v"(off1), "+v"(off2));
  const lds_cptr w0b = (lds_cptr)(uintptr_t)off0, w1b = (lds_cptr)(uintptr_t)off1, vecb = (lds_cptr)(uintptr_t)off2;
  const int t_last = TICKET ? t_hi - 1 : t + ((t_hi - 1 - t) / stride) * stride;
  ew_ctx C;
  C.vecb = vecb;
  C.ln_inv_d = ln_inv_d;
  C.ln_pad = ln_pad;
  C.E = E;
  C.n = n;
  C.g = g;
  C.lane = lane;
  C.elat_out = a.elat_out ? a.elat_out : a.elat;
  C.out_rs = __builtin_amdgcn_make_buffer_rsrc(a.agg, 0, (int)a.aggpart_bytes, 0x00020000);
  C.part_off = (uint32_t)((const char*)a.part - (const char*)a.agg);
  asm volatile("" : "+v"(s_c), "+v"(r_c));
  int guard_tiny = 0;
  ew_tile S0, S1;
  ew_tmp T;
  f32x4 acc[8], p0[8];
  int t_next = 0, s_cur = 0;

  auto draw_next = [&](int tw) -> int {
    if constexpr (TICKET) {
      int k = 0;
      if (lane == 0) k = atomicAdd(&s_ticket, 1);
      return t_lo + __builtin_amdgcn_readfirstlane(k) * stride;
    } else {
      return tw + stride;
    }
  };
  auto issue_ve = [&](ew_tile& X, int tw) {
    const f32x4* er = ew_at(a.elat, (uint32_t)tmap(tw) * 8192u + (uint32_t)lane * 16u);
#pragma unroll
    for (int mb = 0; mb < 8; ++mb) X.ve[mb] = NT ? __builtin_nontemporal_load(&er[64 * mb]) : er[64 * mb];
  };
  auto issue_rest = [&](ew_tile& X, int tw, int tw_after, auto with_ps) {
    const int tt = tmap(tw);
    X.t = tt;
    X.r_cur = r_c;
    s_cur = s_c;
    const f32x4* pr = ew_at(a.psr, (uint32_t)r_c * 1024u + 512u + (uint32_t)g * 16u);
    const f32x4* ps = ew_at(a.psr, (uint32_t)s_c * 1024u + (uint32_t)g * 16u);
    const uint32_t rn = (uint32_t)rowc_of(tmap(min(tw_after, t_last))) * 4u;
    s_c = *reinterpret_cast<const int32_t*>(reinterpret_cast<const char*>(a.senders) + rn);
    r_c = *reinterpret_cast<const int32_t*>(reinterpret_cast<const char*>(a.receivers) + rn);
    int lane_o = lane;
    asm volatile("" : "+v"(lane_o));
    X.rb = lb_edge_probe(a.receivers, tt, lane_o, E);
#pragma unroll
    for (int mb = 0; mb < 8; ++mb) {
      acc[mb] = pr[4 * mb];
      if constexpr (decltype(with_ps)::value) p0[mb] = ps[4 * mb];
    }
  };
  std::true_type yes;
  std::false_type no;
  auto body = [&](auto has_prev, auto first, ew_tile& cur, ew_tile& prev) {
    constexpr bool HAS_PREV = decltype(has_prev)::value, FIRST = decltype(first)::value;
    if constexpr (PF == 0) {
      t_next = draw_next(t);
      issue_ve(cur, t);
      issue_rest(cur, t, t_next, no);
      {
        const f32x4* ps = ew_at(a.psr, (uint32_t)s_cur * 1024u + (uint32_t)g * 16u);
#pragma unroll
        for (int mb = 0; mb < 8; ++mb) p0[mb] = ps[4 * mb];
      }
      asm volatile("" : "+v"(s_c), "+v"(r_c), "+v"(cur.rb));
    } else {
      if (t_next < t_hi) issue_ve(prev, t_next);
    }
    f32x4 h[8];
#pragma unroll
    for (int mb = 0; mb < 8; ++mb) h[mb] = acc[mb];
    if constexpr (FIRST) lb_range_probe(a.ctrl, cur.ve, 8);
    if constexpr (ABL & 2) __builtin_amdgcn_s_setprio(2);
    cur.or_e = 0;
    cur.or_h = 0;
    if constexpr (HAS_PREV && (ABL & 1)) {
#pragma unroll
      for (int k = DF; k < PL::M; ++k) ew_op<SKIP, NT, GUARD, false>(k, prev, T, C, guard_tiny);
    }
    auto fill = [&](int s) {
      if constexpr (HAS_PREV && DF < PL::M && !(ABL & 1)) {
        const int lo = ew_slot_lo<DF, PL::M>(s), hi = ew_slot_lo<DF, PL::M>(s + 1);
#pragma unroll
        for (int u = 0; u < 3; ++u)
          if (lo + u < hi) ew_op<SKIP, NT, GUARD>(lo + u, prev, T, C, guard_tiny);
      }
    };
    ew_gemm<false, GUARD, 0>(w0b, cur.ve, h, &cur.or_e, fill);
#pragma unroll
    for (int mb = 0; mb < 8; ++mb) h[mb] = lb_pk_add(h[mb], p0[mb]);
    if constexpr (FIRST) lb_range_probe(a.ctrl, h, 8);
#pragma unroll
    for (int mb = 0; mb < 8; ++mb) cur.a[mb] = vecb[4 * mb];
    ew_gemm<true, GUARD, 96>(w1b, h, cur.a, &cur.or_h, fill);
    if constexpr (ABL & 2) __builtin_amdgcn_s_setprio(0);
    if constexpr (PF == 2) {
      const int t_nn = t_next < t_hi ? draw_next(t_next) : t_next;
      if (t_next < t_hi) issue_rest(prev, t_next, t_nn, yes);
      t = t_next;
      t_next = t_nn;
    } else {
      t = t_next;
    }
#pragma unroll
    for (int k = 0; k < DF; ++k) ew_op<SKIP, NT, GUARD, false>(k, cur, T, C, guard_tiny);
  };
  auto drain = [&](ew_tile& last) {
#pragma unroll
    for (int k = DF; k < PL::M; ++k) ew_op<SKIP, NT, GUARD, false>(k, last, T, C, guard_tiny);
  };
  if constexpr (PF == 2) {
    t_next = draw_next(t);
    issue_ve(S0, t);
    issue_rest(S0, t, t_next, yes);
  }
  body(no, yes, S0, S1);
  for (;;) {
    if (t >= t_hi) {
      drain(S0);
      break;
    }
    body(yes, no, S1, S0);
    if (t >= t_hi) {
      drain(S1);
      break;
    }
    body(yes, no, S0, S1);
  }
  if (guard_tiny && lane == 0) lb_raise_math(a.ctrl, LB_MATH_TINY);
}

#ifndef EW_NO_LAUNCHER
int lbk_edge16w(lb_engine* e, const lb_edge16_args& a) {
  const int64_t tiles_cap = ((int64_t)e->e_cap * e->g.B + 15) / 16;
  const bool small = tiles_cap < 12288;
  int64_t g = (tiles_cap + 7) / 8;
  g = (g + 7) / 8 * 8;
  const int grid = (int)(g < 8 ? 8 : (g > 256 ? 256 : g));
  const bool guard = e->math_auto && !e->guard_sampled;
#define LB_EW4(SK, NT_, GU, TK) \
  LB_LAUNCH_TIMED(e, (k_edge16w<SK, NT_, GU, TK, (SK ? 2 : 0)>), dim3(grid), dim3(512), a)
#define LB_EW2(SK, NT_, TK)  \
  do {                       \
    if (guard)               \
      LB_EW4(SK, NT_, 1, TK);\
    else                     \
      LB_EW4(SK, NT_, 0, TK);\
  } while (0)
#define LB_EW1(SK)              \
  do {                          \
    if (small)                  \
      LB_EW2(SK, false, true);  \
    else                        \
      LB_EW2(SK, true, false);  \
  } while (0)
  if (a.skip_elat_store)
    LB_EW1(true);
// ... 10 lines not shown
```

lagrangebench_amd/csrc/lb_f16x2.h:

```cpp
#pragma once
#include "lb_device.h"

typedef _Float16 h8 __attribute__((ext_vector_type(8)));
typedef _Float16 h2_t __attribute__((ext_vector_type(2)));
typedef __attribute__((address_space(3))) const f32x4* lds_cptr;
#define MFMA16H(a, b, c) __builtin_amdgcn_mfma_f32_16x16x32_f16((a), (b), (c), 0, 0, 0)
#define SB() __builtin_amdgcn_sched_barrier(0)
#define LB_WAIT_LGKM(n) (0xC07F | ((n) << 8))
typedef float f32x2v __attribute__((ext_vector_type(2)));
__device__ __forceinline__ f32x2v lb_lo2(const f32x4& x) { return f32x2v{x[0], x[1]}; }
__device__ __forceinline__ f32x2v lb_hi2(const f32x4& x) { return f32x2v{x[2], x[3]}; }
__device__ __forceinline__ f32x4 lb_cat2(f32x2v a, f32x2v b) { return f32x4{a[0], a[1], b[0], b[1]}; }
__device__ __forceinline__ f32x4 lb_pk_add(const f32x4& a, const f32x4& b) {
  return lb_cat2(lb_lo2(a) + lb_lo2(b), lb_hi2(a) + lb_hi2(b));
}

__device__ __forceinline__ void lb_range_probe(const lb_ctrl* ctrl, const f32x4* v, int nvec) {
  float m = 0.f;
  for (int i = 0; i < nvec; ++i)
#pragma unroll
    for (int j = 0; j < 4; ++j) m = fmaxf(m, fabsf(v[i][j]));
  bool bad = !(m == m) || m >= 32768.f;
#pragma unroll
  for (int off = 32; off > 0; off >>= 1) m = fmaxf(m, __shfl_xor(m, off));
  const bool any_bad = __any(bad);
  if ((threadIdx.x & 63) == 0) {
    int f = 0;
    if (any_bad || m >= 32768.f) f |= LB_MATH_LARGE;
    if (m > 0.f && m < 0.0009765625f) f |= LB_MATH_TINY;
    if (f) lb_raise_math(ctrl, f);
  }
}

__device__ __forceinline__ bool lb_tile_tiny(uint32_t orv) {
  return !__any((orv & 0x70007000u) != 0u) && __any((orv & 0x7fff7fffu) != 0u);
}

__device__ __forceinline__ bool lb_rows_tiny(uint32_t orv) {
  uint32_t a = orv, b = orv;
  asm volatile("s_nop 1\n\tv_permlane16_swap_b32 %0, %1\n\ts_nop 1" : "+v"(a), "+v"(b));
  a = b = a | b;
  asm volatile("s_nop 1\n\tv_permlane32_swap_b32 %0, %1\n\ts_nop 1" : "+v"(a), "+v"(b));
  const uint32_t r = a | b;
  return __any((r & 0x70007000u) == 0u && (r & 0x7fff7fffu) != 0u);
}

__device__ __forceinline__ void lb_split8v(const f32x4& x0, const f32x4& x1, h8& hi, h8& lo) {
  union {
    h8 v;
    uint32_t u[4];
  } H, L;
  asm("v_cvt_pk_f16_f32 %0, %8, %9\n"
      "v_cvt_pk_f16_f32 %1, %10, %11\n"
      "v_cvt_pk_f16_f32 %2, %12, %13\n"
      "v_cvt_pk_f16_f32 %3, %14, %15\n"
      "v_fma_mixlo_f16 %4, %8, 1.0, -%0 op_sel:[0,0,0] op_sel_hi:[0,0,1]\n"
      "v_fma_mixlo_f16 %5, %10, 1.0, -%1 op_sel:[0,0,0] op_sel_hi:[0,0,1]\n"
      "v_fma_mixlo_f16 %6, %12, 1.0, -%2 op_sel:[0,0,0] op_sel_hi:[0,0,1]\n"
      "v_fma_mixlo_f16 %7, %14, 1.0, -%3 op_sel:[0,0,0] op_sel_hi:[0,0,1]\n"
      "v_fma_mixhi_f16 %4, %9, 1.0, -%0 op_sel:[0,0,1] op_sel_hi:[0,0,1]\n"
      "v_fma_mixhi_f16 %5, %11, 1.0, -%1 op_sel:[0,0,1] op_sel_hi:[0,0,1]\n"
      "v_fma_mixhi_f16 %6, %13, 1.0, -%2 op_sel:[0,0,1] op_sel_hi:[0,0,1]\n"
      "v_fma_mixhi_f16 %7, %15, 1.0, -%3 op_sel:[0,0,1] op_sel_hi:[0,0,1]\n"
      "s_nop 1"
      : "=&v"(H.u[0]), "=&v"(H.u[1]), "=&v"(H.u[2]), "=&v"(H.u[3]), "=&v"(L.u[0]), "=&v"(L.u[1]), "=&v"(L.u[2]),
        "=&v"(L.u[3])
      : "v"(x0[0]), "v"(x0[1]), "v"(x0[2]), "v"(x0[3]), "v"(x1[0]), "v"(x1[1]), "v"(x1[2]), "v"(x1[3]));
  hi = H.v;
  lo = L.v;
}

template <bool RELU, int NP = 4, int GUARD = 0>
__device__ __forceinline__ void lb_gemm16v_r03(lds_cptr wbase, const f32x4 (&v)[2 * NP], f32x4 (&acc)[8], uint32_t* orv = nullptr) {
  auto note = [&](const h8& h, bool first = false) {
    if constexpr (GUARD == 2 || GUARD == 1) {
      if (GUARD == 1 && !first) return;
      typedef uint32_t u32x4g __attribute__((ext_vector_type(4)));
      const u32x4g u = __builtin_bit_cast(u32x4g, h);
      *orv |= (u[0] | u[1]) | (u[2] | u[3]);
    }
  };
  auto frag = [&](int p, int mbo, int part) -> h8 {
    return __builtin_bit_cast(h8, wbase[((p * 8 + mbo) * 2 + part) * 64]);
  };
  auto relu4 = [&](const f32x4& x) -> f32x4 {
    if (!RELU) return x;
    f32x4 r;
#pragma unroll
    for (int j = 0; j < 4; ++j) {
      const float f = x[j];
      r[j] = __builtin_bit_cast(float, max(__builtin_bit_cast(int, f), 0));
    }
    return r;
  };
  h8 X[4], Y[4];
  h8 bh, bl, nbh, nbl;
#pragma unroll
  for (int c = 0; c < 4; ++c) X[c] = frag(0, c, 1);
#pragma unroll
  for (int c = 0; c < 4; ++c) Y[c] = frag(0, c, 0);
  lb_split8v(relu4(v[0]), relu4(v[1]), bh, bl);
  note(bh, true);
  SB();
#pragma unroll
  for (int blk = 0; blk < 2 * NP; ++blk) {
    const int p = blk >> 1, q = blk & 1;
    const int np = (blk + 1) >> 1, nq = (blk + 1) & 1;
    f32x4* a4 = &acc[4 * q];
    __builtin_amdgcn_s_waitcnt(LB_WAIT_LGKM(4));
#pragma unroll
    for (int c = 0; c < 4; ++c) a4[c] = MFMA16H(X[c], bh, a4[c]);
    SB();
    if (blk < 2 * NP - 1) {
#pragma unroll
      for (int c = 0; c < 4; ++c) X[c] = frag(np, 4 * nq + c, 1);
    }
    if (q == 1 && p < NP - 1) {
      lb_split8v(relu4(v[2 * p + 2]), relu4(v[2 * p + 3]), nbh, nbl);
      note(nbh);
    }
    if (blk < 2 * NP - 1)
      __builtin_amdgcn_s_waitcnt(LB_WAIT_LGKM(4));
    else
      __builtin_amdgcn_s_waitcnt(LB_WAIT_LGKM(0));
#pragma unroll
    for (int c = 0; c < 4; ++c) a4[c] = MFMA16H(Y[c], bl, a4[c]);
#pragma unroll
    for (int c = 0; c < 4; ++c) a4[c] = MFMA16H(Y[c], bh, a4[c]);
    SB();
    if (blk < 2 * NP - 1) {
#pragma unroll
      for (int c = 0; c < 4; ++c) Y[c] = frag(np, 4 * nq + c, 0);
    }
    if (q == 1 && p < NP - 1) {
      bh = nbh;
      bl = nbl;
    }
    SB();
  }
}


#ifndef LB_GEMM_INTERLEAVE
#define LB_GEMM_INTERLEAVE 1
#endif
struct lb_split_regs {
  uint32_t H[4], L[4];
  f32x4 r0, r1;
};
template <bool RELU, int GUARD>
__device__ __forceinline__ void lb_split_slot(int s, const f32x4& x0, const f32x4& x1, lb_split_regs& R, uint32_t* orv) {
  if (s < 4) {
    if constexpr (RELU) {
      const float a = s < 2 ? x0[2 * s] : x1[2 * (s - 2)], b = s < 2 ? x0[2 * s + 1] : x1[2 * (s - 2) + 1];
      const float ra = __builtin_bit_cast(float, max(__builtin_bit_cast(int, a), 0));
      const float rb = __builtin_bit_cast(float, max(__builtin_bit_cast(int, b), 0));
      if (s < 2) {
        R.r0[2 * s] = ra;
        R.r0[2 * s + 1] = rb;
      } else {
        R.r1[2 * (s - 2)] = ra;
        R.r1[2 * (s - 2) + 1] = rb;
      }
    }
  } else if (s < 8) {
    const int i = s - 4;
    const f32x4& y = i < 2 ? (RELU ? R.r0 : x0) : (RELU ? R.r1 : x1);
    const float a = y[2 * (i & 1)], b = y[2 * (i & 1) + 1];
    asm volatile("v_cvt_pk_f16_f32 %0, %1, %2" : "=v"(R.H[i]) : "v"(a), "v"(b));
  } else if (s < 12) {
    const int i = s - 8;
    const f32x4& y = i < 2 ? (RELU ? R.r0 : x0) : (RELU ? R.r1 : x1);
    const float a = y[2 * (i & 1)];
    asm volatile("v_fma_mixlo_f16 %0, %1, 1.0, -%2 op_sel:[0,0,0] op_sel_hi:[0,0,1]" : "=&v"(R.L[i]) : "v"(a), "v"(R.H[i]));
  } else if (s < 16) {
    const int i = s - 12;
    const f32x4& y = i < 2 ? (RELU ? R.r0 : x0) : (RELU ? R.r1 : x1);
    const float b = y[2 * (i & 1) + 1];
    asm volatile("v_fma_mixhi_f16 %0, %1, 1.0, -%2 op_sel:[0,0,1] op_sel_hi:[0,0,1]" : "+v"(R.L[i]) : "v"(b), "v"(R.H[i]));
  } else if (s == 16) {
    if constexpr (GUARD == 2) *orv |= (R.H[0] | R.H[1]) | (R.H[2] | R.H[3]);
  }
}
template <bool RELU, int NP = 4, int GUARD = 0>
__device__ __forceinline__ void lb_gemm16v(lds_cptr wbase, const f32x4 (&v)[2 * NP], f32x4 (&acc)[8], uint32_t* orv = nullptr) {
  if constexpr (!LB_GEMM_INTERLEAVE || NP == 1) {
    lb_gemm16v_r03<RELU, NP, GUARD>(wbase, v, acc, orv);
    return;
  } else {
  auto frag = [&](int p, int mbo, int part) -> h8 {
    return __builtin_bit_cast(h8, wbase[((p * 8 + mbo) * 2 + part) * 64]);
  };
  h8 X[4], Y[4];
  h8 bh, bl;
  lb_split_regs R;
#pragma unroll
  for (int c = 0; c < 4; ++c) X[c] = frag(0, c, 1);
#pragma unroll
  for (int c = 0; c < 4; ++c) Y[c] = frag(0, c, 0);
  {
    f32x4 a0 = v[0], a1 = v[1];
    if constexpr (RELU) {
#pragma unroll
      for (int j = 0; j < 4; ++j) {
        const float f0 = a0[j], f1 = a1[j];
        a0[j] = __builtin_bit_cast(float, max(__builtin_bit_cast(int, f0), 0));
        a1[j] = __builtin_bit_cast(float, max(__builtin_bit_cast(int, f1), 0));
      }
    }
    lb_split8v(a0, a1, bh, bl);
    if constexpr (GUARD != 0) {
      typedef uint32_t u32x4g __attribute__((ext_vector_type(4)));
      const u32x4g u = __builtin_bit_cast(u32x4g, bh);
      *orv |= (u[0] | u[1]) | (u[2] | u[3]);
    }
  }
  SB();
#pragma unroll
  for (int blk = 0; blk < 2 * NP; ++blk) {
    const int p = blk >> 1, q = blk & 1;
    const int np = (blk + 1) >> 1, nq = (blk + 1) & 1;
    const bool fill = p < NP - 1;
    const int s0 = 12 * q;
    f32x4* a4 = &acc[4 * q];
    __builtin_amdgcn_s_waitcnt(LB_WAIT_LGKM(4));
#pragma unroll
    for (int c = 0; c < 4; ++c) {
      a4[c] = MFMA16H(X[c], bh, a4[c]);
      if (fill) lb_split_slot<RELU, GUARD>(s0 + c, v[2 * p + 2], v[2 * p + 3], R, orv);
      SB();
    }
    if (blk < 2 * NP - 1) {
#pragma unroll
      for (int c = 0; c < 4; ++c) X[c] = frag(np, 4 * nq + c, 1);
    }
    if (blk < 2 * NP - 1)
      __builtin_amdgcn_s_waitcnt(LB_WAIT_LGKM(4));
    else
      __builtin_amdgcn_s_waitcnt(LB_WAIT_LGKM(0));
#pragma unroll
    for (int c = 0; c < 4; ++c) {
      a4[c] = MFMA16H(Y[c], bl, a4[c]);
      if (fill) lb_split_slot<RELU, GUARD>(s0 + 4 + c, v[2 * p + 2], v[2 * p + 3], R, orv);
      SB();
    }
#pragma unroll
    for (int c = 0; c < 4; ++c) {
      a4[c] = MFMA16H(Y[c], bh, a4[c]);
      if (fill) lb_split_slot<RELU, GUARD>(s0 + 8 + c, v[2 * p + 2], v[2 * p + 3], R, orv);
      SB();
    }
    if (blk < 2 * NP - 1) {
#pragma unroll
      for (int c = 0; c < 4; ++c) Y[c] = frag(np, 4 * nq + c, 0);
    }
    if (q == 1 && fill) {
      typedef uint32_t u32x4s __attribute__((ext_vector_type(4)));
      bh = __builtin_bit_cast(h8, u32x4s{R.H[0], R.H[1], R.H[2], R.H[3]});
      bl = __builtin_bit_cast(h8, u32x4s{R.L[0], R.L[1], R.L[2], R.L[3]});
    }
    SB();
  }
  }
}

template <bool ENABLE = true>
__device__ __forceinline__ void lb_layernorm16(f32x4 (&pre)[8], lds_cptr lns, lds_cptr lno, f32x4 (&y)[8],
                                               float inv_d = 1.0f / 128.0f, float pad = 0.f) {
  if constexpr (!ENABLE) {
#pragma unroll
    for (int mb = 0; mb < 8; ++mb) y[mb] = pre[mb];
    return;
  }
  f32x2v s2 = {0.f, 0.f};
#pragma unroll
  for (int mb = 0; mb < 8; ++mb) s2 = s2 + (lb_lo2(pre[mb]) + lb_hi2(pre[mb]));
  float sm = s2[0] + s2[1];
  sm += __shfl_xor(sm, 16);
  sm += __shfl_xor(sm, 32);
  const float mean = sm * inv_d;
  const f32x2v m2 = {mean, mean};
  f32x2v v2 = {0.f, 0.f};
#pragma unroll
  for (int mb = 0; mb < 8; ++mb) {
    const f32x2v dl = lb_lo2(pre[mb]) - m2, dh = lb_hi2(pre[mb]) - m2;
    v2 = __builtin_elementwise_fma(dl, dl, v2);
    v2 = __builtin_elementwise_fma(dh, dh, v2);
    pre[mb] = lb_cat2(dl, dh);
  }
  float vs = v2[0] + v2[1];
  vs += __shfl_xor(vs, 16);
  vs += __shfl_xor(vs, 32);
  const float rs = 1.0f / sqrtf(fmaxf(vs - pad * (mean * mean), 0.f) * inv_d + 1e-5f);
  const f32x2v r2 = {rs, rs};
#pragma unroll
  for (int mb = 0; mb < 8; ++mb) {
    const f32x4 sc = lns[4 * mb], of = lno[4 * mb];
    y[mb] = lb_cat2(__builtin_elementwise_fma(lb_lo2(sc) * r2, lb_lo2(pre[mb]), lb_lo2(of)),
                    __builtin_elementwise_fma(lb_hi2(sc) * r2, lb_hi2(pre[mb]), lb_hi2(of)));
  }
}

__device__ __forceinline__ int lb_edge_probe(const int32_t* __restrict__ receivers, int t, int lane, int E) {
  int idx = t * 16 - 1 + 17 * (lane & 1);
  idx = idx < 0 ? 0 : (idx < E ? idx : E - 1);
  return receivers[idx];
}
__device__ __forceinline__ bool lb_seg_complete(int rb, int rr, int segstart, int n, int t, int E, int& slot01) {
  const int r_before = __builtin_amdgcn_readlane(rb, 0), r_after = __builtin_amdgcn_readlane(rb, 1);
  const bool starts_before = segstart == 0 && t > 0 && r_before == rr;
  const bool ends_after = n == 15 && t * 16 + 16 < E && r_after == rr;
  slot01 = segstart == 0 ? 0 : 1;
  return !starts_before && !ends_after;
}

__device__ __forceinline__ void lb_scan8(f32x4& a, f32x4& b, float m1, float m2, float m4, float m8) {
  asm volatile(
      "s_nop 1\n"
      "v_fmac_f32_dpp %0, %0, %8 row_shr:1 row_mask:0xf bank_mask:0xf bound_ctrl:1\n"
      "v_fmac_f32_dpp %1, %1, %8 row_shr:1 row_mask:0xf bank_mask:0xf bound_ctrl:1\n"
      "v_fmac_f32_dpp %2, %2, %8 row_shr:1 row_mask:0xf bank_mask:0xf bound_ctrl:1\n"
      "v_fmac_f32_dpp %3, %3, %8 row_shr:1 row_mask:0xf bank_mask:0xf bound_ctrl:1\n"
      "v_fmac_f32_dpp %4, %4, %8 row_shr:1 row_mask:0xf bank_mask:0xf bound_ctrl:1\n"
      "v_fmac_f32_dpp %5, %5, %8 row_shr:1 row_mask:0xf bank_mask:0xf bound_ctrl:1\n"
      "v_fmac_f32_dpp %6, %6, %8 row_shr:1 row_mask:0xf bank_mask:0xf bound_ctrl:1\n"
      "v_fmac_f32_dpp %7, %7, %8 row_shr:1 row_mask:0xf bank_mask:0xf bound_ctrl:1\n"
      "v_fmac_f32_dpp %0, %0, %9 row_shr:2 row_mask:0xf bank_mask:0xf bound_ctrl:1\n"
      "v_fmac_f32_dpp %1, %1, %9 row_shr:2 row_mask:0xf bank_mask:0xf bound_ctrl:1\n"
      "v_fmac_f32_dpp %2, %2, %9 row_shr:2 row_mask:0xf bank_mask:0xf bound_ctrl:1\n"
      "v_fmac_f32_dpp %3, %3, %9 row_shr:2 row_mask:0xf bank_mask:0xf bound_ctrl:1\n"
      "v_fmac_f32_dpp %4, %4, %9 row_shr:2 row_mask:0xf bank_mask:0xf bound_ctrl:1\n"
      "v_fmac_f32_dpp %5, %5, %9 row_shr:2 row_mask:0xf bank_mask:0xf bound_ctrl:1\n"
      "v_fmac_f32_dpp %6, %6, %9 row_shr:2 row_mask:0xf bank_mask:0xf bound_ctrl:1\n"
      "v_fmac_f32_dpp %7, %7, %9 row_shr:2 row_mask:0xf bank_mask:0xf bound_ctrl:1\n"
      "v_fmac_f32_dpp %0, %0, %10 row_shr:4 row_mask:0xf bank_mask:0xf bound_ctrl:1\n"
      "v_fmac_f32_dpp %1, %1, %10 row_shr:4 row_mask:0xf bank_mask:0xf bound_ctrl:1\n"
      "v_fmac_f32_dpp %2, %2, %10 row_shr:4 row_mask:0xf bank_mask:0xf bound_ctrl:1\n"
      "v_fmac_f32_dpp %3, %3, %10 row_shr:4 row_mask:0xf bank_mask:0xf bound_ctrl:1\n"
      "v_fmac_f32_dpp %4, %4, %10 row_shr:4 row_mask:0xf bank_mask:0xf bound_ctrl:1\n"
      "v_fmac_f32_dpp %5, %5, %10 row_shr:4 row_mask:0xf bank_mask:0xf bound_ctrl:1\n"
      "v_fmac_f32_dpp %6, %6, %10 row_shr:4 row_mask:0xf bank_mask:0xf bound_ctrl:1\n"
      "v_fmac_f32_dpp %7, %7, %10 row_shr:4 row_mask:0xf bank_mask:0xf bound_ctrl:1\n"
      "v_fmac_f32_dpp %0, %0, %11 row_shr:8 row_mask:0xf bank_mask:0xf bound_ctrl:1\n"
      "v_fmac_f32_dpp %1, %1, %11 row_shr:8 row_mask:0xf bank_mask:0xf bound_ctrl:1\n"
      "v_fmac_f32_dpp %2, %2, %11 row_shr:8 row_mask:0xf bank_mask:0xf bound_ctrl:1\n"
      "v_fmac_f32_dpp %3, %3, %11 row_shr:8 row_mask:0xf bank_mask:0xf bound_ctrl:1\n"
      "v_fmac_f32_dpp %4, %4, %11 row_shr:8 row_mask:0xf bank_mask:0xf bound_ctrl:1\n"
      "v_fmac_f32_dpp %5, %5, %11 row_shr:8 row_mask:0xf bank_mask:0xf bound_ctrl:1\n"
      "v_fmac_f32_dpp %6, %6, %11 row_shr:8 row_mask:0xf bank_mask:0xf bound_ctrl:1\n"
      "v_fmac_f32_dpp %7, %7, %11 row_shr:8 row_mask:0xf bank_mask:0xf bound_ctrl:1\n"
      "s_nop 1\n"
      : "+v"(a[0]), "+v"(a[1]), "+v"(a[2]), "+v"(a[3]), "+v"(b[0]), "+v"(b[1]), "+v"(b[2]), "+v"(b[3])
      : "v"(m1), "v"(m2), "v"(m4), "v"(m8));
}
```

lagrangebench_amd/csrc/lb_gns.hip:

```cpp
#include <stdio.h>

#include <algorithm>
#include <stdlib.h>

#include "lb_device.h"
#include "lb_msplit.h"

#define MFMA(a, b, c) __builtin_amdgcn_mfma_f32_32x32x2f32((a), (b), (c), 0, 0, 0)

void lb_pack_weight(const float* w, int K, int M, int Kpad, int Mpad, float* out) {
  const int NKQ = Kpad / 8, NMB = Mpad / 32;
  for (int kq = 0; kq < NKQ; ++kq)
    for (int mb = 0; mb < NMB; ++mb)
      for (int lane = 0; lane < 64; ++lane)
        for (int j = 0; j < 4; ++j) {
          const int k = 8 * kq + 4 * (lane >> 5) + j;
          const int m = 32 * mb + (lane & 31);
          out[(((size_t)kq * NMB + mb) * 64 + lane) * 4 + j] =
              (k < K && m < M) ? w[(size_t)k * M + m] : 0.f;
        }
}

template <int NKQ, int NMB, int PF = 1, typename LD>
__device__ __forceinline__ void lb_gemm(LD ld, const f32x4 (&v)[NKQ], f32x16 (&acc)[NMB]) {
// ... 180 lines not shown
      }
    }
  }
}

template <int D4>
__global__ void __launch_bounds__(256) k_segment_sum(const lb_ctrl* __restrict__ ctrl,
                                                    const int32_t* __restrict__ row_ptr,
                                                    const float* __restrict__ msg,
                                                    float* __restrict__ out, int64_t n_rows) {
  if (ctrl->overflow_step >= 0) return;
  const int per_block = 256 / D4;
  const int64_t row = (int64_t)blockIdx.x * per_block + threadIdx.x / D4;
  const int c = threadIdx.x % D4;
  if (row >= n_rows) return;
  const int E = ctrl->n_edges_total;
  int k0 = row_ptr[row], k1 = row_ptr[row + 1];
  k0 = k0 < E ? k0 : E;
  k1 = k1 < E ? k1 : E;
  const f32x4* m4 = reinterpret_cast<const f32x4*>(msg);
  f32x4 s = {0.f, 0.f, 0.f, 0.f};
  int k = k0;
  for (; k + 4 <= k1; k += 4) {
    const f32x4 a0 = m4[(int64_t)(k + 0) * D4 + c];
    const f32x4 a1 = m4[(int64_t)(k + 1) * D4 + c];
    const f32x4 a2 = m4[(int64_t)(k + 2) * D4 + c];
    const f32x4 a3 = m4[(int64_t)(k + 3) * D4 + c];
    s = s + a0;
    s = s + a1;
    s = s + a2;
    s = s + a3;
  }
  for (; k < k1; ++k) s = s + m4[(int64_t)k * D4 + c];
  reinterpret_cast<f32x4*>(out)[row * D4 + c] = s;
}

int lbk_segment_sum(lb_engine* e, const float* msg, float* out, int D) {
  if (D != 128) return lb_fail(LB_ERR_UNSUPPORTED, "segment_sum: D=%d not built (128 only)", D);
  const int64_t rows = e->BN;
  const int per_block = 256 / 32;
  const int nb = (int)((rows + per_block - 1) / per_block);
  hipLaunchKernelGGL((k_segment_sum<32>), dim3(nb), dim3(256), 0, e->stream, e->ctrl, e->row_ptr,
                     msg, out, rows);
  LB_HIP(hipGetLastError());
  return LB_OK;
}

static int lb_msplit_env() {
  static const int env = getenv("LB_MSPLIT") ? atoi(getenv("LB_MSPLIT")) : -1;
  return env;
}
static bool lb_use_msplit_edge(const lb_engine* e) {
  const int64_t max_tiles = 3072;
  const int env = lb_msplit_env();
  if (!e->f16x2 || !e->fused_agg || env == 0) return false;
  if (env == 1) return true;
  return ((int64_t)e->e_cap * e->g.B + 15) / 16 <= max_tiles;
}
static bool lb_use_edge_w(const lb_engine* e) {
  return !e->guard_full && e->aggpart_bytes < ((int64_t)1 << 31) &&
         (int64_t)(e->e_alloc + 32) * 512 < ((int64_t)1 << 32) && e->BN * 1024 < ((int64_t)1 << 32);
}
static bool lb_use_msplit_node(const lb_engine* e) {
  const int64_t max_nodes = 16384;
  const int env = lb_msplit_env();
  if (!e->f16x2 || env == 0) return false;
  if (env == 1) return true;
  return e->BN <= max_nodes;
}

extern "C" int lb_kernel_names(lb_engine* e, char* out, int32_t cap) {
  if (!e || !out || cap < 1) return lb_fail(LB_ERR_ARG, "null argument");
  const char* edge = !e->f16x2 ? "k_edge16<PROC,f32>"
                     : !e->fused_agg ? "k_edge16<PROC,f16x2> + k_segment_sum"
                     : lb_use_msplit_edge(e) ? "k_edge_ms (M-split, f16x2, fused segment_sum)"
                     : lb_use_edge_w(e) ? "k_edge16w<2 waves/SIMD, resident latents; last layer: deferred epilogue> (PROC, f16x2, fused segment_sum)"
                                        : "k_edge16v<2 waves/SIMD, resident latents, GEMM-phase priority> (PROC, f16x2, fused segment_sum)";
  const char* node = !e->f16x2 ? "k_node_mlp<f32>" : lb_use_msplit_node(e) ? "k_node_ms (M-split, f16x2)" : "k_node16s (f16x2)";
  snprintf(out, (size_t)cap, "edge=%s;node=%s", edge, node);
  return LB_OK;
}

int lbk_gns_forward(lb_engine* e, lb_gns* g) {
  LB_TRY(lb_gns_bind(e, g));
  if (g->generic) return lbk_gns_forward_generic(e, g);
  const bool ms_e = lb_use_msplit_edge(e), ms_n = lb_use_msplit_node(e);
  const bool ms_en = ms_n, ms_ee = ms_e, ms_pe = ms_e, ms_pn = ms_n;
  hipStream_t s = e->stream;
  const int64_t BN = e->BN;
  const int ntile_n = (int)((BN + LB_TILE - 1) / LB_TILE);
  const int L = g->desc.num_mp_steps;
  int rc;

  if (!(e->feat_done && e->feat_job.xnode == e->xnode)) {
    lb_tic(e, LB_T_NODEFEAT);
    rc = lbk_node_features(e, e->xnode, g->embed, g->desc.embedding_size,
                           g->desc.num_particle_types, nullptr, nullptr, nullptr, nullptr);
    lb_toc(e);
    if (rc) return rc;
  }

  auto node_mlp = [&](const lb_mlp_w& w, const float* xin, int kq, bool with_agg, bool resid, int next, bool ms,
                      bool dec = false) -> int {
    const bool proj = next < L;
    lb_node_args a{};
    a.ctrl = e->ctrl;
    a.n_rows = BN;
    a.xin = xin;
    a.agg = e->agg;
    a.nlat = e->nlat;
    a.w0p = w.w0;
    a.b0 = w.b0;
    a.w1p = w.w1;
    a.b1 = w.b1;
    a.ln_s = w.ln_s;
    a.ln_o = w.ln_o;
    a.wpp = proj ? g->proc_edge[next].proj_w : nullptr;
    a.bp = proj ? g->proc_edge[next].proj_b : nullptr;
    a.psr = e->psr;
    a.fused = e->fused_agg;
    a.tile_shift = 4;
    a.row_ptr = e->row_ptr;
    a.part = e->part;
    if (ms) {
      lb_nms_args m{};
      m.ctrl = e->ctrl;
      m.n_rows = BN;
      m.xin = xin;
      m.agg = e->agg;
      m.row_ptr = e->row_ptr;
      m.part = e->part;
      m.fused = e->fused_agg;
      m.nlat = e->nlat;
      m.w = w.ms;
      m.b0 = a.b0;
      m.b1 = a.b1;
      m.ln_s = a.ln_s;
      m.ln_o = a.ln_o;
      m.bp = a.bp;
      m.psr = e->psr;
      if (dec) {
        m.bd0 = g->dec.b0;
        m.bd1 = g->dec.b1;
        m.dec_unscale = g->dec_unscale;
        m.acc_out = e->acc;
        m.out_dim = g->desc.out_dim;
        if (e->integ_job.on && g->desc.out_dim == e->g.dim) {
          m.integ = e->integ_job;
          e->integ_done = true;
        }
      }
      return lbk_node_ms(e, m, kq / 4, with_agg, resid, proj, dec);
    }
    if (e->f16x2)
      return lbk_node16s(e, a, w.w0_16h, w.w1_16h, proj ? g->proc_edge[next].proj_w_h2 : nullptr, kq / 4, with_agg ? 4 : 0,
                         resid);
    if (with_agg)
      hipLaunchKernelGGL((k_node_mlp<16, 16, true>), dim3(ntile_n), dim3(64), 0, s, a);
    else if (kq == 4)
      hipLaunchKernelGGL((k_node_mlp<4, 0, false>), dim3(ntile_n), dim3(64), 0, s, a);
    else if (kq == 8)
      hipLaunchKernelGGL((k_node_mlp<8, 0, false>), dim3(ntile_n), dim3(64), 0, s, a);
    else if (kq == 12)
      hipLaunchKernelGGL((k_node_mlp<12, 0, false>), dim3(ntile_n), dim3(64), 0, s, a);
    else
      hipLaunchKernelGGL((k_node_mlp<16, 0, false>), dim3(ntile_n), dim3(64), 0, s, a);
    return LB_OK;
  };

  lb_tic(e, LB_T_ENC_NODE);
  rc = node_mlp(g->enc_node, e->xnode, g->kq_node, false, false, 0, ms_en);
  lb_toc(e);
  if (rc) return rc;

  bool decoded = false;
  lb_tic(e, LB_T_ENC_EDGE);
  if (ms_ee) {
    lb_ems_args m{};
    m.ctrl = e->ctrl;
    m.efeat = e->efeat;
    m.elat = e->elat;
    m.w = g->enc_edge.ms;
    m.b0 = g->enc_edge.b0;
    m.b1 = g->enc_edge.b1;
    m.ln_s = g->enc_edge.ln_s;
    m.ln_o = g->enc_edge.ln_o;
    rc = lbk_edge_enc_ms(e, m);
  } else {
    lb_edge16_args b{};
    b.ctrl = e->ctrl;
    b.efeat = e->efeat;
    b.elat = e->elat;
    b.w0p = e->f16x2 ? g->enc_edge.w0_16h : g->enc_edge.w0_16;
    b.b0 = g->enc_edge.b0;
    b.w1p = e->f16x2 ? g->enc_edge.w1_16h : g->enc_edge.w1_16;
    b.b1 = g->enc_edge.b1;
    b.ln_s = g->enc_edge.ln_s;
    b.ln_o = g->enc_edge.ln_o;
    rc = e->f16x2 ? lbk_edge_enc16v(e, b) : lbk_edge16(e, b, false, false);
  }
  lb_toc(e);
  if (rc) return rc;
  if (g->tap) LB_HIP(hipMemcpyAsync(g->tap, e->nlat, sizeof(float) * BN * LB_D, hipMemcpyDeviceToDevice, s));

  for (int k = 0; k < L; ++k) {
    const lb_mlp_w& pe = g->proc_edge[k];
    const bool skip = (k == L - 1) && e->fused_agg && !g->tap;
    lb_tic_single(e, skip ? LB_T_EDGE_LAST : LB_T_EDGE_MLP);
    if (ms_pe) {
      lb_ems_args m{};
      m.ctrl = e->ctrl;
      m.senders = e->senders;
      m.receivers = e->receivers;
      m.elat = e->elat;
      m.psr = e->psr;
      m.w = pe.ms;
      m.b1 = pe.b1;
      m.ln_s = pe.ln_s;
      m.ln_o = pe.ln_o;
      m.agg = e->agg;
      m.part = e->part;
      m.skip_elat_store = skip;
      rc = lbk_edge_ms(e, m);
    } else {
      lb_edge16_args b{};
      b.ctrl = e->ctrl;
      b.senders = e->senders;
      b.receivers = e->receivers;
      b.elat = e->elat;
      b.msg = e->msg;
      b.psr = e->psr;
      b.w0p = e->f16x2 ? pe.w0_16h : pe.w0_16;
      b.w1p = e->f16x2 ? pe.w1_16h : pe.w1_16;
      b.b1 = pe.b1;
      b.ln_s = pe.ln_s;
      b.ln_o = pe.ln_o;
      b.fused = e->fused_agg;
      b.row_ptr = e->row_ptr;
      b.agg = e->agg;
      b.part = e->part;
      b.aggpart_bytes = e->aggpart_bytes;
      b.skip_elat_store = skip;
      if (e->f16x2 && e->fused_agg)
        rc = lb_use_edge_w(e) ? lbk_edge16w(e, b) : lbk_edge16v(e, b);
      else
        rc = lbk_edge16(e, b, true, e->f16x2 != 0);
    }
    lb_toc(e);
    if (rc) return rc;
    if (!e->fused_agg) {
      lb_tic(e, LB_T_AGGREGATE);
      rc = lbk_segment_sum(e, e->msg, e->agg, LB_D);
      lb_toc(e);
      if (rc) return rc;
    }
    const bool ms_dec_ok = lb_fused_launches();
    const bool with_dec = ms_pn && ms_dec_ok && k == L - 1 && e->f16x2 && g->desc.out_dim <= 4;
    lb_tic_single(e, LB_T_NODE_MLP);
    rc = node_mlp(g->proc_node[k], e->nlat, 16, true, true, k + 1, ms_pn, with_dec);
    lb_toc(e);
    decoded = with_dec;
    if (rc) return rc;
    if (g->tap)
      LB_HIP(hipMemcpyAsync(g->tap + (size_t)(k + 1) * BN * LB_D, e->nlat, sizeof(float) * BN * LB_D,
                            hipMemcpyDeviceToDevice, s));
  }
  if (decoded) return LB_OK;
  lb_tic(e, LB_T_DECODER);
  rc = lbk_decoder16(e, g);
  lb_toc(e);
  if (rc) return rc;
  LB_HIP(hipGetLastError());
  return LB_OK;
}
```

lagrangebench_amd/csrc/lb_gns_repack.h:

```cpp
#pragma once
#include <stdint.h>

#include <vector>

#include "../../include/lbhip.h"

#if defined(__HIPCC__)
#define LB_HD __host__ __device__
#else
#define LB_HD
#endif

LB_HD static inline uint16_t lb_f32_to_f16_rne(float f) {
  uint32_t x = __builtin_bit_cast(uint32_t, f);
  const uint32_t sign = (x >> 16) & 0x8000u;
  x &= 0x7fffffffu;
  if (x >= 0x47800000u) return (uint16_t)(sign | (x > 0x7f800000u ? 0x7e00u : 0x7c00u));
  if (x < 0x38800000u) {
    if (x < 0x33000000u) return (uint16_t)sign;
    const int shift = 126 - (int)(x >> 23);
    uint32_t m = (x & 0x7fffffu) | 0x800000u;
    const uint32_t lsb = 1u << shift, half = lsb >> 1;
    uint32_t r = m >> shift;
    const uint32_t rem = m & (lsb - 1);
    if (rem > half || (rem == half && (r & 1))) ++r;
    return (uint16_t)(sign | r);
  }
  uint32_t r = x - 0x38000000u;
  const uint32_t rem = r & 0x1fffu;
  r >>= 13;
  if (rem > 0x1000u || (rem == 0x1000u && (r & 1))) ++r;
  return (uint16_t)(sign | r);
}
LB_HD static inline float lb_f16_to_f32(uint16_t h) {
  const uint32_t sign = (uint32_t)(h & 0x8000u) << 16;
  const uint32_t e = (h >> 10) & 0x1f, m = h & 0x3ffu;
  uint32_t x;
  if (e == 0) {
    if (m == 0) {
      x = sign;
    } else {
      int k = 0;
      uint32_t mm = m;
      while (!(mm & 0x400u)) {
        mm <<= 1;
        ++k;
      }
      x = sign | ((uint32_t)(113 - k) << 23) | ((mm & 0x3ffu) << 13);
    }
  } else if (e == 31) {
    x = sign | 0x7f800000u | (m << 13);
  } else {
    x = sign | ((e + 112) << 23) | (m << 13);
  }
  return __builtin_bit_cast(float, x);
}

enum lb_pack_kind {
  LB_PK_VEC = 0,
  LB_PK_P32,
  LB_PK_P16,
  LB_PK_P16H,
  LB_PK_MS
};
struct lb_pack_piece {
  int64_t off;
  int32_t row0, rows, stride, col0, cols, pad_;
};
struct lb_pack_job {
  int64_t dst;
  int32_t kind, K, M, Kpad, Mpad;
  int32_t nkb;
  int32_t perm;
  int32_t at;
  int32_t scaled;
  int32_t n_ent;
  int32_t piece0, n_pieces;
};
struct lb_pack_red {
  int32_t piece0, n_pieces;
};
struct lb_pack_block {
  int32_t job, ent0;
};
struct lb_pack_plan {
  std::vector<lb_pack_job> jobs;
  std::vector<lb_pack_piece> pieces;
  std::vector<lb_pack_red> rms;
  lb_pack_red head{0, 0};
  std::vector<lb_pack_block> blocks;
  int64_t blob_floats = 0;
  int64_t src_floats = 0;
};
struct lb_pack_stats {
  float scale;
  float unscale;
  double rms_min;
};
#define LB_PACK_LANES 256

LB_HD static inline float lb_pack_src(const lb_pack_job& j, const lb_pack_piece* pc, const float* w, int k, int m) {
  if (k >= j.K || m >= j.M) return 0.f;
  for (int i = 0; i < j.n_pieces; ++i) {
    const lb_pack_piece& p = pc[j.piece0 + i];
    const int r = k - p.row0, c = m - p.col0;
    if (r >= 0 && r < p.rows && c >= 0 && c < p.cols) return w[p.off + (int64_t)r * p.stride + c];
  }
  return 0.f;
}

LB_HD static inline void lb_pack_entry(const lb_pack_job& j, const lb_pack_piece* pc, const float* w, float scale, int ent,
                                       uint32_t out[4]) {
  const int lane = ent & 63, blk = ent >> 6;
  auto src = [&](int k, int m) {
    const float x = lb_pack_src(j, pc, w, k, m);
    return j.scaled ? x * scale : x;
  };
  if (j.kind == LB_PK_VEC) {
    for (int i = 0; i < 4; ++i) {
      const int c = 4 * ent + i - j.at;
      out[i] = __builtin_bit_cast(uint32_t, (c >= 0 && c < j.M) ? src(0, c) : 0.f);
    }
    return;
  }
  if (j.kind == LB_PK_P32) {
    const int NMB = j.Mpad / 32, kq = blk / NMB, mb = blk % NMB;
    for (int i = 0; i < 4; ++i) out[i] = __builtin_bit_cast(uint32_t, src(8 * kq + 4 * (lane >> 5) + i, 32 * mb + (lane & 31)));
    return;
  }
  if (j.kind == LB_PK_P16) {
    const int hf = blk & 1, jj = (blk >> 1) & 3, mbk = blk >> 3;
    for (int c = 0; c < 4; ++c)
      out[c] = __builtin_bit_cast(uint32_t, src(16 * mbk + 4 * (lane >> 4) + jj, 16 * (4 * hf + c) + (lane & 15)));
    return;
  }
  const int part = blk & 1, outer = blk >> 1, g = lane >> 4;
  int kb, m;
  bool perm = true;
  if (j.kind == LB_PK_P16H) {
    const int NMBO = j.Mpad / 16;
    kb = outer / NMBO;
    m = 16 * (outer % NMBO) + (lane & 15);
  } else {
    kb = outer % j.nkb;
    m = 16 * (outer / j.nkb) + (lane & 15);
    perm = j.perm != 0;
  }
  uint16_t h[8];
  for (int i = 0; i < 8; ++i) {
    const int k = perm ? 32 * kb + 16 * (i >> 2) + 4 * g + (i & 3) : 32 * kb + 8 * g + i;
    const float x = src(k, m);
    const uint16_t hi = lb_f32_to_f16_rne(x);
    h[i] = part ? lb_f32_to_f16_rne(x - lb_f16_to_f32(hi)) : hi;
  }
  for (int i = 0; i < 4; ++i) out[i] = (uint32_t)h[2 * i] | ((uint32_t)h[2 * i + 1] << 16);
}

LB_HD static inline int lb_head_shift(float mx) {
  const uint32_t b = __builtin_bit_cast(uint32_t, mx) & 0x7fffffffu;
  const int ef = (int)(b >> 23);
  if (b == 0 || ef == 255) return 0;
  if (ef == 0) return 60;
  const int sh = ((b & 0x7fffffu) ? -2 : -1) - (ef - 127);
  return sh < -60 ? -60 : sh > 60 ? 60 : sh;
}
LB_HD static inline float lb_pow2f(int sh) { return __builtin_bit_cast(float, (uint32_t)(127 + sh) << 23); }

LB_HD static inline void lb_pack_red_lane(const lb_pack_red& r, const lb_pack_piece* pc, const float* w, int lane, double* s2,
                                          double* nz, uint32_t* mx) {
  double s = 0, n = 0;
  uint32_t m = 0;
  for (int i = 0; i < r.n_pieces; ++i) {
    const lb_pack_piece& p = pc[r.piece0 + i];
    const int cnt = p.rows * p.cols;
    for (int q = lane; q < cnt; q += LB_PACK_LANES) {
      const float x = w[p.off + (int64_t)(q / p.cols) * p.stride + (q % p.cols)];
      s += (double)x * x;
      n += x != 0.f;
      const uint32_t a = __builtin_bit_cast(uint32_t, x) & 0x7fffffffu;
      if (a <= 0x7f800000u && a > m) m = a;
    }
  }
  *s2 = s;
  *nz = n;
  *mx = m;
}
LB_HD static inline double lb_pack_red_rms(const double* s2, const double* nz) {
  double s = 0, n = 0;
  for (int i = 0; i < LB_PACK_LANES; ++i) {
    s += s2[i];
    n += nz[i];
  }
  return n > 0 ? __builtin_sqrt(s / n) : 1e30;
}

struct lb_gns;
struct lb_engine;
int lb_gns_pack_plan_build(const lb_gns_desc* d, int kq_node, const std::vector<int64_t>* cmap, int64_t n_compact,
                           int64_t n_src, lb_pack_plan* plan);
int lb_gns_train_padded_map(const lb_gns_desc* d, std::vector<int64_t>* cmap, int64_t* n_dev, int64_t* n_compact);
struct lb_repack;
int lbk_gns_repack(lb_engine* e, lb_gns* g, const float* w_dev, const std::vector<int64_t>& cmap, int64_t n_compact,
                   int64_t n_src);
void lb_repack_free(lb_repack* r);
```

lagrangebench_amd/csrc/lb_gns_weights.hip:

```cpp
#include <algorithm>
#include <cmath>
#include <cstdio>
#include <cstring>
#include <utility>
#include <vector>

#include "lb_gns_repack.h"
#include "lb_msplit.h"

struct lb_lin_view {
  const float* w;
  int blocks, rows, out;
  const float* b;
  const float* block(int i) const { return w + (size_t)i * rows * out; }
};
struct lb_mlp_view {
  std::vector<lb_lin_view> lin;
  const float* ln_s = nullptr;
  const float* ln_o = nullptr;
};
struct lb_gns_view {
  const float* embed = nullptr;
  lb_mlp_view enc_node, enc_edge, dec;
  std::vector<lb_mlp_view> proc_edge, proc_node;
};

static int lb_gns_walk(const lb_gns_desc* d, const float* w, int64_t n_floats, lb_gns_view* v) {
  const int dl = d->latent_size, nl = d->blocks_per_step;
  const int emb = d->num_particle_types > 1 ? d->embedding_size : 0;
  int64_t off = 0;
  auto take = [&](int64_t n) {
    const float* p = off + n <= n_floats ? w + off : nullptr;
    off += n;
    return p;
  };
  auto mlp = [&](int blocks, int rows, int out, bool ln) {
    lb_mlp_view m;
    for (int li = 0; li < nl; ++li) {
      lb_lin_view l;
      l.blocks = li ? 1 : blocks;
      l.rows = li ? dl : rows;
      l.out = li == nl - 1 ? out : dl;
      l.w = take((int64_t)l.blocks * l.rows * l.out);
      l.b = take(l.out);
      m.lin.push_back(l);
    }
    if (ln) {
      m.ln_s = take(out);
      m.ln_o = take(out);
    }
    return m;
  };
  if (emb) v->embed = take((int64_t)d->num_particle_types * emb);
  v->enc_node = mlp(1, d->node_in + emb, dl, true);
  v->enc_edge = mlp(1, d->edge_in, dl, true);
  for (int k = 0; k < d->num_mp_steps; ++k) {
    v->proc_edge.push_back(mlp(3, dl, dl, true));
    v->proc_node.push_back(mlp(2, dl, dl, true));
  }
  v->dec = mlp(1, dl, d->out_dim, false);
  if (off != n_floats) {
    if (nl == 2)
      return lb_fail(LB_ERR_ARG, "weight blob has %lld floats, expected %lld", (long long)n_floats, (long long)off);
    return lb_fail(LB_ERR_ARG, "weight blob has %lld floats, the model (num_mlp_layers %d, latent %d) needs %s",
                   (long long)n_floats, nl, dl, off > n_floats ? "more" : "fewer");
  }
  return LB_OK;
}

struct lb_src_piece {
  const float* w;
  int row0, rows, stride, col0, cols;
};
struct lb_src {
  std::vector<lb_src_piece> pc;
  int K = 0, M = 0;
  bool scaled = false;
};
static lb_src lb_src_plain(const float* w, int K, int M) { return {{{w, 0, K, M, 0, M}}, K, M, false}; }
static lb_src lb_src_padded(const lb_lin_view& l) {
  lb_src s;
  s.K = l.blocks * LB_D;
  s.M = LB_D;
  for (int b = 0; b < l.blocks; ++b) s.pc.push_back({l.block(b), b * LB_D, l.rows, l.out, 0, l.out});
  return s;
}
static lb_src lb_src_ws_wr(const lb_lin_view& l) {
  lb_src s;
  s.K = LB_D;
  s.M = 2 * LB_D;
  for (int b = 0; b < 2; ++b) s.pc.push_back({l.block(b), 0, l.rows, l.out, b * LB_D, l.out});
  return s;
}

struct lb_ms_piece {
  lb_src s;
  int nkb, npw;
  bool perm;
  size_t keep;
};

struct lb_stage {
  std::vector<float> host;
  std::vector<std::pair<const float**, size_t>> fix;
  double w_rms_min = 1e30;
  int sh = 0;
  lb_pack_plan* rec = nullptr;
  const float* base = nullptr;
  const std::vector<int64_t>* cmap = nullptr;
  size_t n = 0;

  size_t next(const float** field, size_t count) {
    const size_t off = (n + 63) & ~(size_t)63;
    n = off + count;
    if (!rec) host.resize(n, 0.f);
    if (field) fix.push_back({field, off});
    return off;
  }
  int rec_pieces(const std::vector<lb_src_piece>& pc) {
    auto at = [&](int64_t i) { return cmap ? (*cmap)[(size_t)i] : i; };
    for (const lb_src_piece& p : pc) {
      const int64_t o = p.w - base;
      const int stride = p.rows > 1 ? (int)(at(o + p.stride) - at(o)) : p.stride;
      rec->pieces.push_back({at(o), p.row0, p.rows, stride, p.col0, p.cols, 0});
    }
    return (int)pc.size();
  }
  void rec_job(size_t off, int kind, const lb_src& s, int Kpad, int Mpad, int nkb, bool perm, int at, size_t floats) {
    lb_pack_job j{};
    j.dst = (int64_t)off;
    j.kind = kind;
    j.K = s.K;
    j.M = s.M;
    j.Kpad = Kpad;
    j.Mpad = Mpad;
    j.nkb = nkb;
    j.perm = perm;
    j.at = at;
    j.scaled = s.scaled;
    j.n_ent = (int32_t)((floats + 3) / 4);
    j.piece0 = (int32_t)rec->pieces.size();
    j.n_pieces = rec_pieces(s.pc);
    rec->jobs.push_back(j);
  }
  std::vector<float> dense(const lb_src& s) const {
    std::vector<float> o((size_t)s.K * s.M, 0.f);
    for (const lb_src_piece& p : s.pc)
      for (int r = 0; r < p.rows; ++r)
        memcpy(&o[(size_t)(p.row0 + r) * s.M + p.col0], p.w + (size_t)r * p.stride, sizeof(float) * p.cols);
    if (s.scaled)
      for (float& x : o) x = std::ldexp(x, sh);
    return o;
  }

  void vec(const float** field, size_t count, const float* src = nullptr, size_t n_src = 0, size_t at = 0) {
    const size_t off = next(field, count);
    if (rec)
      rec_job(off, LB_PK_VEC, src ? lb_src_plain(src, 1, (int)n_src) : lb_src(), 1, (int)count, 0, false, (int)at, count);
    else if (src)
      memcpy(host.data() + off + at, src, n_src * sizeof(float));
  }
  void img(const float** field, int kind, const lb_src& s, int Kp, int Mp) {
    const size_t off = next(field, (size_t)Kp * Mp);
    if (rec) return rec_job(off, kind, s, Kp, Mp, 0, false, 0, (size_t)Kp * Mp);
    const std::vector<float> w = dense(s);
    float* out = host.data() + off;
    if (kind == LB_PK_P32) lb_pack_weight(w.data(), s.K, s.M, Kp, Mp, out);
    else if (kind == LB_PK_P16) lb_pack_weight16(w.data(), s.K, s.M, Kp, out);
    else lb_pack_weight16h(w.data(), s.K, s.M, Kp, out, Mp);
  }
  void ms(const float** field, const std::vector<lb_ms_piece>& pieces) {
    size_t total = 0;
    for (const lb_ms_piece& m : pieces) total += m.keep ? m.keep : (size_t)m.nkb * m.npw * 4096;
    size_t off = next(field, total);
    std::vector<float> tmp;
    for (const lb_ms_piece& m : pieces) {
      const size_t full = (size_t)m.nkb * m.npw * 4096, kept = m.keep ? m.keep : full;
      if (rec) {
        rec_job(off, LB_PK_MS, m.s, 32 * m.nkb, 128 * m.npw, m.nkb, m.perm, 0, kept);
      } else {
        tmp.assign(full, 0.f);
        lb_pack_ms(dense(m.s).data(), m.s.K, m.s.M, m.nkb, m.npw, m.perm, tmp.data());
        memcpy(host.data() + off, tmp.data(), kept * sizeof(float));
      }
      off += kept;
    }
  }
  void note_rms(const lb_lin_view& l) {
    if (rec) {
      std::vector<lb_src_piece> pc;
      for (int b = 0; b < l.blocks; ++b) pc.push_back({l.block(b), 0, l.rows, l.out, 0, l.out});
      const int32_t p0 = (int32_t)rec->pieces.size();
      rec->rms.push_back({p0, rec_pieces(pc)});
      return;
    }
    const size_t cnt = (size_t)l.blocks * l.rows * l.out;
    double s2 = 0;
    size_t nz = 0;
    for (size_t i = 0; i < cnt; ++i) {
      s2 += (double)l.w[i] * l.w[i];
      nz += l.w[i] != 0.f;
    }
    if (nz) w_rms_min = std::min(w_rms_min, std::sqrt(s2 / (double)nz));
  }
  void head_shift(const lb_lin_view& l) {
    if (rec) {
      const int32_t p0 = (int32_t)rec->pieces.size();
      rec->head = {p0, rec_pieces({{l.w, 0, l.rows, l.out, 0, l.out}})};
      return;
    }
    float mx = 0.f;
    for (size_t i = 0; i < (size_t)l.rows * l.out; ++i) mx = std::max(mx, std::fabs(l.w[i]));
    sh = lb_head_shift(mx);
  }
  int upload(lb_arena& mem, float** blob) {
    LB_TRY(mem.get(blob, host.size()));
    if (hipMemcpy(*blob, host.data(), host.size() * sizeof(float), hipMemcpyHostToDevice) != hipSuccess)
      return lb_fail(LB_ERR_HIP, "weight upload failed");
    for (const auto& f : fix) *f.first = *blob + f.second;
    return LB_OK;
  }
};

static void lb_pack_fused(lb_stage& st, const lb_gns_view& v, lb_gns* g) {
  const int D = LB_D, L = g->desc.num_mp_steps, dl = g->desc.latent_size;
  auto p32 = [&](const float** f, const lb_src& s, int Kp, int Mp) { st.img(f, LB_PK_P32, s, Kp, Mp); };
  auto p16 = [&](const float** f, const lb_src& s, int Kp) { st.img(f, LB_PK_P16, s, Kp, 128); };
  auto p16h = [&](const float** f, const lb_src& s, int Kp, int Mp = 128) { st.img(f, LB_PK_P16H, s, Kp, Mp); };
  auto lin = [&](const lb_lin_view& l, int b = 0) { return lb_src_plain(l.block(b), l.rows, l.out); };
  auto vecs = [&](lb_mlp_w& m, const lb_mlp_view& s, bool b0, int b1_pad = LB_D) {
    if (b0) st.vec(&m.b0, D, s.lin[0].b, dl);
    st.vec(&m.b1, b1_pad, s.lin[1].b, s.lin[1].out);
    if (s.ln_s) {
      st.vec(&m.ln_s, D, s.ln_s, dl);
      st.vec(&m.ln_o, D, s.ln_o, dl);
    }
  };

  const lb_lin_view &d0 = v.dec.lin[0], &d1 = v.dec.lin[1];
  st.head_shift(d1);
  g->dec_unscale = std::ldexp(1.f, -st.sh);
  lb_src d1s = lin(d1);
  d1s.scaled = true;
  st.note_rms(d0);
  p16(&g->dec.w0_16, lin(d0), D);
  p16h(&g->dec.w0_16h, lin(d0), D);
  p16(&g->dec.w1_16, lin(d1), D);
  p16h(&g->dec.w1_16h, d1s, D, 16);
  vecs(g->dec, v.dec, true, 32);

  {
    const lb_lin_view &l0 = v.enc_edge.lin[0], &l1 = v.enc_edge.lin[1];
    lb_mlp_w& m = g->enc_edge;
    st.note_rms(l0);
    st.note_rms(l1);
    p16(&m.w0_16, lin(l0), 16);
    p16h(&m.w0_16h, lin(l0), 32);
    p16(&m.w1_16, lin(l1), D);
    p16h(&m.w1_16h, lin(l1), D);
    vecs(m, v.enc_edge, true);
    st.ms(&m.ms, {{lin(l0), 1, 1, false, 0}, {lin(l1), 4, 1, true, 0}});
  }

  auto node_mlp = [&](lb_mlp_w& m, const lb_mlp_view& s, const lb_src& w0, int K0p, std::vector<lb_ms_piece> ms) {
    const lb_lin_view& l1 = s.lin[1];
    st.note_rms(s.lin[0]);
    st.note_rms(l1);
    p32(&m.w0, w0, K0p, D);
    p16h(&m.w0_16h, w0, K0p);
    p32(&m.w1, lin(l1), D, D);
    p16h(&m.w1_16h, lin(l1), D);
    vecs(m, s, true);
    ms.insert(ms.begin(), {{w0, K0p / 32, 1, true, 0}, {lin(l1), 4, 1, true, 0}});
    st.ms(&m.ms, ms);
  };
  auto proj_piece = [&](const lb_src& wsr) { return std::vector<lb_ms_piece>{{wsr, 4, 2, true, 0}}; };

  lb_src wsr, wsr_next;
  if (L) wsr = lb_src_ws_wr(v.proc_edge[0].lin[0]);
  node_mlp(g->enc_node, v.enc_node, lin(v.enc_node.lin[0]), g->kq_node * 8, L ? proj_piece(wsr) : std::vector<lb_ms_piece>());
  g->proc_edge.resize(L);
  g->proc_node.resize(L);
  for (int k = 0; k < L; ++k) {
    {
      const lb_lin_view &l0 = v.proc_edge[k].lin[0], &l1 = v.proc_edge[k].lin[1];
      lb_mlp_w& m = g->proc_edge[k];
      p32(&m.proj_w, wsr, D, 2 * D);
      p16h(&m.proj_w_h2, lin(l0, 0), D, D);
      p16h(nullptr, lin(l0, 1), D, D);
      st.vec(&m.proj_b, 2 * D, l0.b, dl, D);
      p16(&m.w0_16, lin(l0, 2), D);
      p16h(&m.w0_16h, lin(l0, 2), D);
      p16(&m.w1_16, lin(l1), D);
      p16h(&m.w1_16h, lin(l1), D);
      vecs(m, v.proc_edge[k], false);
      st.ms(&m.ms, {{lin(l0, 2), 4, 1, true, 0}, {lin(l1), 4, 1, true, 0}});
    }
    std::vector<lb_ms_piece> ms = {{lin(d0), 4, 1, true, 0}, {d1s, 4, 1, true, 2048}};
    if (k + 1 < L) {
      wsr_next = lb_src_ws_wr(v.proc_edge[k + 1].lin[0]);
      ms = proj_piece(wsr_next);
    }
    node_mlp(g->proc_node[k], v.proc_node[k], lb_src_padded(v.proc_node[k].lin[0]), 2 * D, ms);
    std::swap(wsr, wsr_next);
  }
}

static void lb_pack_dense(lb_stage& st, const lb_gns_view& v, lb_gns* g) {
  const int D = LB_D, L = g->desc.num_mp_steps;
  auto mlp = [&](lb_gen_mlp& m, const lb_mlp_view& s) {
    m.lin.resize(s.lin.size());
    for (size_t li = 0; li < s.lin.size(); ++li) {
      const lb_lin_view& l = s.lin[li];
      lb_gen_lin& x = m.lin[li];
      st.note_rms(l);
      x.wh.resize(l.blocks);
      x.wf.resize(l.blocks);
      for (int b = 0; b < l.blocks; ++b) {
        st.img(&x.wh[b], LB_PK_P16H, lb_src_plain(l.block(b), l.rows, l.out), D, D);
        st.img(&x.wf[b], LB_PK_P16, lb_src_plain(l.block(b), l.rows, l.out), D, D);
      }
      st.vec(&x.b, D, l.b, l.out);
    }
    if (s.ln_s) {
      st.vec(&m.ln_s, D, s.ln_s, s.lin.back().out);
      st.vec(&m.ln_o, D, s.ln_o, s.lin.back().out);
    }
  };
  mlp(g->g_enc_node, v.enc_node);
  mlp(g->g_enc_edge, v.enc_edge);
  g->g_proc_edge.resize(L);
  g->g_proc_node.resize(L);
  for (int k = 0; k < L; ++k) {
    mlp(g->g_proc_edge[k], v.proc_edge[k]);
    mlp(g->g_proc_node[k], v.proc_node[k]);
  }
  mlp(g->g_dec, v.dec);
}

static void lb_gns_stage_all(lb_stage& st, const lb_gns_view& v, lb_gns* g) {
  const lb_gns_desc* d = &g->desc;
  if (v.embed) st.vec(&g->embed, (size_t)d->num_particle_types * d->embedding_size, v.embed,
                      (size_t)d->num_particle_types * d->embedding_size);
  if (g->generic)
    lb_pack_dense(st, v, g);
  else
    lb_pack_fused(st, v, g);
}

static int lb_gns_check_desc(const lb_gns_desc* d, const lb_engine* e) {
  const int dl = d->latent_size, nl = d->blocks_per_step;
  if (dl < 16 || dl > LB_D || dl % 16)
    return lb_fail(LB_ERR_UNSUPPORTED, "latent_size %d not built (multiples of 16 up to 128)", dl);
  if (e && d->out_dim != e->g.dim) return lb_fail(LB_ERR_ARG, "out_dim %d != case dim %d", d->out_dim, e->g.dim);
  if (e && d->node_in != e->g.node_in) return lb_fail(LB_ERR_ARG, "node_in %d != case feature width %d", d->node_in, e->g.node_in);
  if (e && d->edge_in != e->g.dim + 1) return lb_fail(LB_ERR_ARG, "edge_in %d != dim+1", d->edge_in);
  if (!e && (d->out_dim < 1 || d->out_dim > 3 || d->node_in < 1 || d->edge_in < 1 || d->edge_in > 16))
    return lb_fail(LB_ERR_ARG, "bad input / output widths");
  if (d->num_mp_steps < 0 || d->num_mp_steps > 64) return lb_fail(LB_ERR_ARG, "bad num_mp_steps");
  if (nl < 1 || nl > 16) return lb_fail(LB_ERR_ARG, "num_mlp_layers %d out of range (1..16)", nl);
  const int nin = d->node_in + (d->num_particle_types > 1 ? d->embedding_size : 0);
  if (nin > 128) return lb_fail(LB_ERR_UNSUPPORTED, "node input width %d > 128 not built", nin);
  return LB_OK;
}
static void lb_gns_init(lb_gns* g, const lb_gns_desc* d, lb_engine* e, int kq_node) {
  const int nin = d->node_in + (d->num_particle_types > 1 ? d->embedding_size : 0);
  g->desc = *d;
  g->eng = e;
  g->generic = d->blocks_per_step != 2;
  g->kq_node = kq_node > 0 ? kq_node : (nin + 31) / 32 * 4;
  g->lnc[0] = 1.0f / (float)d->latent_size;
  g->lnc[1] = (float)(LB_D - d->latent_size);
}

extern "C" int lb_gns_create(lb_engine* e, const lb_gns_desc* d, const float* w, int64_t n_floats, lb_gns** out) {
  if (!e || !d || !w || !out) return lb_fail(LB_ERR_ARG, "null argument");
  LB_TRY(lb_gns_check_desc(d, e));
  lb_gns_view v;
  LB_TRY(lb_gns_walk(d, w, n_floats, &v));

  lb_gns* g = new lb_gns();
  lb_gns_init(g, d, e, 0);
  lb_stage st;
  lb_gns_stage_all(st, v, g);
  g->blob_floats = (int64_t)st.host.size();
  int rc = st.upload(g->mem, &g->blob);
  if (!rc) lb_gns_rms_guard(e, st.w_rms_min);
  if (!rc) rc = lb_ensure_node_scratch(e);
  if (!rc) rc = lb_gns_bind(e, g);
  for (int i = 0; i < 3 && g->generic && !rc; ++i) rc = g->mem.get(&g->gen_hn[i], (size_t)e->BN * LB_D);
  if (rc) {
    lb_gns_destroy(g);
    return rc;
  }
  *out = g;
  return LB_OK;
}

void lb_gns_rms_guard(lb_engine* e, double w_rms_min) {
  if (w_rms_min < 0.0078125 && e->f16x2 && e->math_auto) {
    fprintf(stderr, "[lbhip] a weight matrix has rms %.3g < 2^-7: its fp16 hi/lo split would fall short of the 1e-5 class - "
                    "this engine uses exact-fp32 MFMA arithmetic\n", w_rms_min);
    e->f16x2 = 0;
  }
}

int lb_gns_pack_plan_build(const lb_gns_desc* d, int kq_node, const std::vector<int64_t>* cmap, int64_t n_compact,
                           int64_t n_src, lb_pack_plan* plan) {
  LB_TRY(lb_gns_check_desc(d, nullptr));
  if (cmap && (int64_t)cmap->size() != n_compact) return lb_fail(LB_ERR_ARG, "index map of %lld entries for %lld weights",
                                                                 (long long)cmap->size(), (long long)n_compact);
  const std::vector<float> dummy((size_t)std::max<int64_t>(n_compact, 1));
  lb_gns_view v;
  LB_TRY(lb_gns_walk(d, dummy.data(), n_compact, &v));
  lb_gns g{};
  lb_gns_init(&g, d, nullptr, kq_node);
  *plan = lb_pack_plan();
  lb_stage st;
  st.rec = plan;
  st.base = dummy.data();
  st.cmap = cmap;
  lb_gns_stage_all(st, v, &g);
  plan->blob_floats = (int64_t)st.n;
  plan->src_floats = n_src;
  for (const lb_pack_piece& p : plan->pieces)
    if (p.off < 0 || p.rows < 1 || p.cols < 1 || p.stride < p.cols ||
        p.off + (int64_t)(p.rows - 1) * p.stride + p.cols > n_src)
      return lb_fail(LB_ERR_STATE, "repack table: a source rectangle leaves the weight blob");
  for (size_t ji = 0; ji < plan->jobs.size(); ++ji) {
    const lb_pack_job& j = plan->jobs[ji];
    if (j.dst % 4 || j.dst < 0 || j.dst + (int64_t)4 * j.n_ent > ((plan->blob_floats + 3) & ~(int64_t)3))
      return lb_fail(LB_ERR_STATE, "repack table: an image leaves the packed blob");
    for (int e0 = 0; e0 < j.n_ent; e0 += LB_PACK_LANES) plan->blocks.push_back({(int32_t)ji, e0});
  }
  if (plan->blob_floats % 4) return lb_fail(LB_ERR_UNSUPPORTED, "repack table: packed blob of %lld floats", (long long)plan->blob_floats);
  return LB_OK;
}

static void lb_pack_plan_interpret(const lb_pack_plan& plan, const float* w, float* out, lb_pack_stats* stats) {
  const lb_pack_piece* pc = plan.pieces.data();
  std::vector<double> s2(LB_PACK_LANES), nz(LB_PACK_LANES);
  uint32_t mxb = 0, m;
  stats->rms_min = 1e30;
  for (const lb_pack_red& r : plan.rms) {
    for (int l = 0; l < LB_PACK_LANES; ++l) lb_pack_red_lane(r, pc, w, l, &s2[l], &nz[l], &m);
    stats->rms_min = std::min(stats->rms_min, lb_pack_red_rms(s2.data(), nz.data()));
  }
  for (int l = 0; l < LB_PACK_LANES && plan.head.n_pieces; ++l) {
    lb_pack_red_lane(plan.head, pc, w, l, &s2[l], &nz[l], &m);
    mxb = std::max(mxb, m);
  }
  const int sh = lb_head_shift(__builtin_bit_cast(float, mxb));
  stats->scale = lb_pow2f(sh);
  stats->unscale = lb_pow2f(-sh);
  for (const lb_pack_job& j : plan.jobs)
    for (int ent = 0; ent < j.n_ent; ++ent)
      lb_pack_entry(j, pc, w, stats->scale, ent, reinterpret_cast<uint32_t*>(out + j.dst + (int64_t)4 * ent));
}

extern "C" int64_t lb_gns_pack_selftest(const lb_gns_desc* d, int32_t node_in_kq, const float* w, int64_t n_floats,
                                        int64_t* n_bytes_out) {
  if (!d || !w) return lb_fail(LB_ERR_ARG, "null argument");
  LB_TRY(lb_gns_check_desc(d, nullptr));
  if (node_in_kq < 0 || node_in_kq > 16 || node_in_kq % 4) return lb_fail(LB_ERR_ARG, "node_in_kq %d: 0 or 4, 8, 12, 16", (int)node_in_kq);
  lb_gns_view v;
  LB_TRY(lb_gns_walk(d, w, n_floats, &v));
  lb_gns ga{};
  lb_gns_init(&ga, d, nullptr, node_in_kq);
  if (node_in_kq && node_in_kq < (d->node_in + (d->num_particle_types > 1 ? d->embedding_size : 0) + 7) / 8)
    return lb_fail(LB_ERR_ARG, "node_in_kq %d is narrower than the node input", (int)node_in_kq);
  lb_stage st;
  lb_gns_stage_all(st, v, &ga);
  std::vector<int64_t> cmap;
  int64_t n_dev = 0, n_compact = 0;
  LB_TRY(lb_gns_train_padded_map(d, &cmap, &n_dev, &n_compact));
  if (n_compact != n_floats) return lb_fail(LB_ERR_ARG, "weight blob has %lld floats, expected %lld", (long long)n_floats, (long long)n_compact);
  std::vector<float> padded;
  const float* src = w;
  if (!cmap.empty()) {
    padded.assign((size_t)n_dev, 0.f);
    for (int64_t i = 0; i < n_floats; ++i) padded[(size_t)cmap[(size_t)i]] = w[i];
    src = padded.data();
  }
  lb_pack_plan plan;
  LB_TRY(lb_gns_pack_plan_build(d, ga.kq_node, cmap.empty() ? nullptr : &cmap, n_compact, n_dev, &plan));
  if (plan.blob_floats != (int64_t)st.host.size())
    return lb_fail(LB_ERR_STATE, "the recorded blob has %lld floats, the packed one %lld", (long long)plan.blob_floats, (long long)st.host.size());
  std::vector<float> img((size_t)plan.blob_floats, 0.f);
  lb_pack_stats stats;
  lb_pack_plan_interpret(plan, src, img.data(), &stats);
  int64_t diff = 0;
  const unsigned char *a = reinterpret_cast<const unsigned char*>(st.host.data()), *b = reinterpret_cast<const unsigned char*>(img.data());
  for (size_t i = 0; i < img.size() * sizeof(float); ++i) diff += a[i] != b[i];
  diff += 4 * (int64_t)(__builtin_bit_cast(uint32_t, stats.unscale) != __builtin_bit_cast(uint32_t, ga.dec_unscale));
  const double r0 = st.w_rms_min, r1 = stats.rms_min;
  diff += 8 * (int64_t)(std::fabs(r0 - r1) > 1e-12 * std::max(r0, r1));
  if (n_bytes_out) *n_bytes_out = (int64_t)(img.size() * sizeof(float));
  return diff;
}

extern "C" int64_t lb_gns_image_bytes(lb_gns* g) { return g ? g->blob_floats * (int64_t)sizeof(float) : -1; }
extern "C" int lb_gns_image_read(lb_gns* g, void* out_host, int64_t n_bytes) {
  if (!g || !out_host || n_bytes != g->blob_floats * (int64_t)sizeof(float)) return lb_fail(LB_ERR_ARG, "bad argument");
  LB_HIP(hipStreamSynchronize(g->eng->stream));
  LB_HIP(hipMemcpy(out_host, g->blob, (size_t)n_bytes, hipMemcpyDeviceToHost));
  return LB_OK;
}

int lb_gns_bind(lb_engine* e, lb_gns* g) {
  if (e->bound_model == g) return LB_OK;
  LB_HIP(hipMemcpyAsync(&e->ctrl->ln_inv_d, g->lnc, sizeof(g->lnc), hipMemcpyHostToDevice, e->stream));
  e->g.kpad = g->kq_node * 8;
  e->bound_model = g;
  return LB_OK;
}

extern "C" void lb_gns_destroy(lb_gns* g) {
  if (!g) return;
  if (g->eng && g->eng->bound_model == g) g->eng->bound_model = nullptr;
  lb_repack_free(g->repack);
  delete g;
}

extern "C" int lb_gns_set_tap(lb_gns* g, float* tap) {
  if (!g) return lb_fail(LB_ERR_ARG, "null model");
  g->tap = tap;
  return LB_OK;
}
```

lagrangebench_amd/csrc/lb_internal.h:

```cpp
#pragma once
#include <cstdlib>
#include <hip/hip_ext.h>
#include <hip/hip_runtime.h>
#include <stdint.h>

#include <string>
#include <vector>

#include "../../include/lbhip.h"
#include "lb_arena.h"

#define LB_MAX_STENCIL_CAND 2048
#define LB_MAX_ROW 256
#define LB_MAX_ROW_DENSE 4096
#define LB_TILE 32
#define LB_D 128
#define LB_PAD_TYPE (-1)

typedef float f32x4 __attribute__((ext_vector_type(4)));
typedef float f32x16 __attribute__((ext_vector_type(16)));

struct lb_ctrl {
  int32_t step;
  int32_t overflow_step;
// ... 28 lines not shown
  int32_t dim, N, B, isl, periodic, has_bound, has_vel_mag, force_kind, force_axis;
  int32_t use_cell_list;
  int32_t ncell[3];
  int32_t ncells;
  int32_t nstencil;
  int32_t node_in;
  int32_t kpad;
  int32_t f32;
  double cell_size[3];
  double box[3], half_box[3];
  double rc, rc2;
  double vel_mean[3], vel_std[3], acc_mean[3], acc_std[3];
  double bound_lo[3], bound_hi[3];
  double force_split, force_lo[3], force_hi[3];
};

struct lb_feat_job {
  float* xnode;
  const float* embed;
  int32_t emb, ntypes, kpad;
  const int32_t* ptype;
  const double* force;
};

struct lb_integ_job {
  double* win;
  int32_t* blocks_done;
  const int32_t* ptype;
  const double* traj;
  int32_t T;
  double* pred;
  int32_t pred_T;
  int32_t on;
};

enum lb_timer_class {
  LB_T_CELLS = 0,
  LB_T_NEIGH,
  LB_T_NODEFEAT,
  LB_T_ENC_NODE,
  LB_T_ENC_EDGE,
  LB_T_EDGE_MLP,
  LB_T_AGGREGATE,
  LB_T_NODE_MLP,
  LB_T_DECODER,
  LB_T_INTEGRATE,
  LB_T_MISC,
  LB_T_PROCESSOR,
  LB_T_EDGE_LAST,
  LB_T_COUNT
};

struct lb_timer_rec {
  hipEvent_t a, b;
  int cls;
};

struct lb_engine {
  lb_arena mem;
  lb_case_desc desc;
  lb_geom g;
  hipStream_t stream;
  int64_t BN;

  double* win;
  int32_t* ptype;
  int32_t* live_cnt = nullptr;
  double* force;
  lb_ctrl* ctrl;
  int32_t* blocks_done = nullptr;
  lb_ctrl* ctrl_host;
  int32_t* host_flag;
  int32_t* host_flag_dev;
  hipEvent_t step_ev[4];
  hipStream_t gstream;

  int32_t cell_capacity, e_cap;
  int64_t e_alloc;
  int32_t* cell_of;
  int32_t* cell_count;
  int32_t* cell_start;
  int32_t* cell_fill;
  bool cells_traj_ready = false;
  int32_t* cell_part;
  int32_t* deg;
  lb_feat_job feat_job{};
  bool feat_done = false;
  lb_integ_job integ_job{};
  bool integ_done = false;
  bool nl_one_off = false;
  unsigned long long* nl_wg_sum = nullptr;
  int32_t* row_ptr;
  int32_t* scan_part;
  double* cpos;
  int64_t cell_slots = 0;
  bool nl_dense = false;
  int32_t row_cap = 0;
  int32_t maxd;
  int32_t* tmp_send;
  float* tmp_feat;
  double* tmp_feat64;
  int32_t* senders;
  int32_t* receivers;
  float* efeat;
  double* efeat64;
  int32_t* overflow;
  int32_t* nedges_b;

  uint64_t nl_gen = 0;
  bool graph_seen = false, graph_bad = false;
  uint64_t graph_gen = 0;
  int32_t graph_ecap = 0, graph_E = 0;
  bool snd_seen = false;
  uint64_t snd_gen = 0;
  int32_t *snd_perm = nullptr, *snd_ptr = nullptr;
  int32_t *snd_key = nullptr, *snd_iota = nullptr;
  int32_t* snd_flag = nullptr;
  void* snd_tmp = nullptr;
  size_t snd_tmp_bytes = 0;
  int64_t snd_cap = 0;
  bool snd_radix = false;
  int32_t snd_sorts = 0;

  float* xnode;
  float* nlat;
  float* agg;
  float* psr;
  float* elat;
  float* msg;
  float* part;
  int64_t aggpart_bytes = 0;
  int fused_agg;
  int f16x2;
  int math_auto;
  int guard_sampled;
  int math_fallbacks = 0;
  int debug_guard_step = -1;
  int debug_guard_flags = 0;
  int guard_full;
  float* acc;
  const void* bound_model = nullptr;

  bool timers_on;
  std::vector<lb_timer_rec> trecs;
  bool ext_armed = false, ext_used = false;
  std::vector<hipEvent_t> epool;
  double t_ms[LB_T_COUNT];
  int64_t t_n[LB_T_COUNT];
};

struct lb_mlp_w {
  const float* b0;
  const float* b1;
  const float* ln_s;
  const float* ln_o;
  const float* w0;
  const float* w1;
  const float* w0_16;
  const float* w1_16;
  const float* w0_16h;
  const float* w1_16h;
  const float* ms;
  const float* proj_w;
  const float* proj_w_h2;
  const float* proj_b;
};

struct lb_edge16_args {
  const lb_ctrl* ctrl;
  const int32_t* senders;
  const int32_t* receivers;
  const float* efeat;
  float* elat;
  float* elat_out;
  float* msg;
  const float* psr;
  const float* w0p;
  const float* b0;
  const float* w1p;
  const float* b1;
  const float* ln_s;
  const float* ln_o;
  int fused;
  const int32_t* row_ptr;
  float* agg;
  float* part;
  int64_t aggpart_bytes;
  int reverse;
  int skip_elat_store;
};

struct lb_node_args {
  const lb_ctrl* ctrl;
  int64_t n_rows;
  const float* xin;
  const float* agg;
  float* nlat;
  const float* w0p;
  const float* b0;
  const float* w1p;
  const float* b1;
  const float* ln_s;
  const float* ln_o;
  const float* wpp;
  const float* bp;
  float* psr;
  int fused;
  int tile_shift;
  const int32_t* row_ptr;
  const float* part;
};

struct lb_gen_lin {
  std::vector<const float*> wh, wf;
  const float* b;
};
struct lb_gen_mlp {
  std::vector<lb_gen_lin> lin;
  const float* ln_s = nullptr;
  const float* ln_o = nullptr;
};

struct lb_gns {
  lb_arena mem;
  lb_gns_desc desc;
  lb_engine* eng;
  float* blob;
  int64_t blob_floats = 0;
  struct lb_repack* repack = nullptr;
  const float* embed;
  int kq_node;
  float lnc[2] = {1.0f / LB_D, 0.f};
  float* tap;
  lb_mlp_w enc_node, enc_edge, dec;
  std::vector<lb_mlp_w> proc_edge, proc_node;
  float dec_unscale = 1.f;
  bool generic = false;
  lb_gen_mlp g_enc_node, g_enc_edge, g_dec;
  std::vector<lb_gen_mlp> g_proc_edge, g_proc_node;
  float* gen_hn[3] = {nullptr, nullptr, nullptr};
  float* gen_he = nullptr;
  int64_t gen_he_cap = 0;
};

extern thread_local std::string g_lb_err;
int lb_fail(int code, const char* fmt, ...);
#define LB_HIP(call)                                                                   \
  do {                                                                                 \
    hipError_t _e = (call);                                                            \
    if (_e != hipSuccess)                                                              \
      return lb_fail(LB_ERR_HIP, "%s failed: %s (%s:%d)", #call, hipGetErrorString(_e), \
                     __FILE__, __LINE__);                                              \
  } while (0)

#define LB_TRY(x)          \
  do {                     \
    int _rc = (x);         \
    if (_rc) return _rc;   \
  } while (0)

static inline bool lb_fused_launches() {
  static const bool ok = !(getenv("LB_SMALL_FUSED") && getenv("LB_SMALL_FUSED")[0] == '0');
  return ok;
}
void lb_tic(lb_engine* e, int cls);
void lb_toc(lb_engine* e);
void lb_tic_single(lb_engine* e, int cls);
#define LB_LAUNCH_TIMED(e, kern, grid, block, ...)                                                        \
  do {                                                                                                    \
    if ((e)->ext_armed && !(e)->ext_used) {                                                               \
      hipExtLaunchKernelGGL(kern, grid, block, 0, (e)->stream, (e)->trecs.back().a, (e)->trecs.back().b, \
                            0, __VA_ARGS__);                                                              \
      (e)->ext_used = true;                                                                               \
    } else {                                                                                              \
      hipLaunchKernelGGL(kern, grid, block, 0, (e)->stream, __VA_ARGS__);                                 \
    }                                                                                                     \
  } while (0)

int lb_ensure_edges(lb_engine* e, int64_t need);
int lb_alloc_aggpart(lb_engine* e, int64_t n_edges);

int lbk_nl_build(lb_engine* e, bool want_efeat64);
int lbk_nl_export(lb_engine* e, int32_t* idx_out, int32_t* n_edges_out);
int lbk_edge_features_export(lb_engine* e, double* rel_disp, double* rel_dist);

int lbk_load_window(lb_engine* e, const double* traj, int T, int t0, int step);
int lbk_load_window_resume(lb_engine* e, const double* traj, int T, const double* pred, int pred_T, int step);
int lbk_read_window(lb_engine* e, double* out);
int lbk_node_features(lb_engine* e, float* xnode, const float* embed, int emb, int ntypes,
                      double* vel_hist, double* vel_mag, double* bound, double* force);
int lbk_integrate(lb_engine* e, const float* acc, int acc_stride, const double* target,
                  const double* traj, int T, double* pred, int pred_T);
int lbk_ekin(lb_engine* e, const double* roll, int T, int stride, int n_out, double dt, double dx,
             double* out);
int lbk_case_integrate(lb_engine* e, int mode, const float* pred, const double* pos_seq, int T,
                       double* out);
int lbk_metrics(lb_engine* e, const double* pred, int pred_T, const double* target, int target_T,
                int n_steps, double* mse, double* mae);

int lbk_sinkhorn(lb_engine* e, const double* pred, int pred_T, const double* target, int target_T, int stride,
                 int n_out, double threshold, double* out_dev, int32_t* iters_host);
int lbk_sinkhorn_pot(lb_engine* e, const double* pred, int pred_T, const double* target, int target_T, int stride,
                     int n_out, double reg, int max_it, double thr, double* out_dev, int32_t* info_host);

int lbk_node_features_raw(lb_engine* e, float* xnode, int kpad);

// ... 84 lines not shown
```

lagrangebench_amd/csrc/lb_node16s.hip:

```cpp
#include <stdlib.h>

#include "lb_f16x2.h"

#define NS_CHUNK 2048

typedef __attribute__((address_space(3))) f32x4* lds_ptr;
typedef const __attribute__((address_space(1))) void* gbl_cvptr;

template <int MB0>
__device__ __forceinline__ void lb_load_agg_half(const lb_node_args& a, int64_t gnode, int g, int k0, int k1,
                                                 f32x4 (&v)[4]) {
  if (!a.fused) {
    const f32x4* gr = reinterpret_cast<const f32x4*>(a.agg) + gnode * 32 + g;
#pragma unroll
    for (int mb = 0; mb < 4; ++mb) v[mb] = gr[4 * (MB0 + mb)];
#pragma unroll
    for (int mb = 0; mb < 4; ++mb) asm volatile("" : "+v"(v[mb]));
    return;
  }
  const int t0 = k0 >> a.tile_shift, t1 = (k1 - 1) >> a.tile_shift;
  const bool single = t0 == t1;
  const int nsrc = (k1 <= k0) ? 0 : (single ? 1 : t1 - t0 + 1);
#pragma unroll
  for (int mb = 0; mb < 4; ++mb) v[mb] = f32x4{0.f, 0.f, 0.f, 0.f};
// ... 14 lines not shown
    k_node16s(lb_node_args a, const f32x4* __restrict__ w0h, const f32x4* __restrict__ w1h,
              const f32x4* __restrict__ wph) {
  __shared__ f32x4 sB[NS_SLOTS][NS_CHUNK];
  __shared__ f32x4 sP[192];
  if (a.ctrl->overflow_step >= 0) return;
  const int tid = threadIdx.x, lane = tid & 63, wave = __builtin_amdgcn_readfirstlane(tid >> 6);
  const int n = lane & 15, g = lane >> 4;
  constexpr int NP0 = NPA + NPB;
  constexpr int NCH0 = (NP0 + 1) / 2;
  constexpr int n_chunks = NCH0 + 2 + (PROJ ? 4 : 0);
  static_assert(NPB == 0 || (NPA == 4 && NPB == 4), "processor shape: 4 + 4 k-steps");

  if (tid < 128) {
    const float* src = tid < 32 ? a.b0 : (tid < 64 ? a.b1 : (tid < 96 ? a.ln_s : a.ln_o));
    sP[tid] = reinterpret_cast<const f32x4*>(src)[tid & 31];
  } else if (tid < 192) {
    sP[tid] = (PROJ && a.bp) ? reinterpret_cast<const f32x4*>(a.bp)[tid - 128] : f32x4{0.f, 0.f, 0.f, 0.f};
  }

  auto issue_chunk = [&](int c) {
    const f32x4* src;
    int nvec = NS_CHUNK;
    if (c < NCH0) {
      src = w0h + (size_t)c * NS_CHUNK;
      if (2 * c + 2 > NP0) nvec = NS_CHUNK / 2;
    } else if (c < NCH0 + 2) {
      src = w1h + (size_t)(c - NCH0) * NS_CHUNK;
    } else {
      src = wph + (size_t)(c - NCH0 - 2) * NS_CHUNK;
    }
    f32x4* slot = sB[c % NS_SLOTS];
#pragma unroll
    for (int i = 0; i < 32 / NW; ++i) {
      const int piece = wave + NW * i;
      if (piece * 64 < nvec) {
        const uint32_t voff = (uint32_t)(piece * 64 + lane) * 16u;
        const uint32_t lo = (uint32_t)(uintptr_t)(lds_ptr)(slot + piece * 64);
        asm volatile("s_mov_b32 m0, %2\n\tglobal_load_lds_dwordx4 %0, %1" ::"v"(voff), "s"(src), "s"(lo) : "memory");
      }
    }
  };
  constexpr int DPC = 32 / NW;
#define NS_STEP(c)                                                                     \
  do {                                                                                 \
    constexpr int later = ((c) + NS_SLOTS - 2 < n_chunks ? NS_SLOTS - 2 : n_chunks - 1 - (c)); \
    if constexpr (later * DPC == 0) asm volatile("s_waitcnt vmcnt(0)" ::: "memory");   \
    if constexpr (later * DPC == 1) asm volatile("s_waitcnt vmcnt(1)" ::: "memory");   \
    if constexpr (later * DPC == 2) asm volatile("s_waitcnt vmcnt(2)" ::: "memory");   \
    if constexpr (later * DPC == 4) asm volatile("s_waitcnt vmcnt(4)" ::: "memory");   \
    if constexpr (later * DPC == 8) asm volatile("s_waitcnt vmcnt(8)" ::: "memory");   \
    if constexpr (later * DPC == 16) asm volatile("s_waitcnt vmcnt(16)" ::: "memory"); \
    if constexpr ((c) == 0) {                                                          \
      __syncthreads();                \
    } else {                                                                           \
      asm volatile("s_waitcnt lgkmcnt(0)\n\ts_barrier" ::: "memory");                  \
    }                                                                                  \
  } while (0)
#define NS_REFILL(c)                                                           \
  do {                                                                         \
    if constexpr ((c) >= 1 && (c)-1 + NS_SLOTS < n_chunks) issue_chunk((c)-1 + NS_SLOTS); \
  } while (0)
#pragma unroll
  for (int c = 0; c < (n_chunks < NS_SLOTS ? n_chunks : NS_SLOTS); ++c) issue_chunk(c);

  const int64_t row = ((int64_t)blockIdx.x * NW + wave) * 16 + n;
  const bool valid = row < a.n_rows;
  const int64_t rowc = valid ? row : a.n_rows - 1;
  lds_cptr lane_b[NS_SLOTS];
#pragma unroll
  for (int i = 0; i < NS_SLOTS; ++i) lane_b[i] = (lds_cptr)(sB[i] + lane);
  const lds_cptr vecp = (lds_cptr)(sP + g);

  f32x4 va[2 * NPA];
  int k0 = 0, k1 = 0;
  {
    const f32x4* xr = reinterpret_cast<const f32x4*>(a.xin) + rowc * (8 * NPA) + g;
#pragma unroll
    for (int mb = 0; mb < 2 * NPA; ++mb) va[mb] = xr[4 * mb];
    if (NPB > 0 && a.fused) {
      k0 = a.row_ptr[rowc];
      k1 = a.row_ptr[rowc + 1];
    }
  }
  const bool probe = wave == 0;
#define NS_BUF(c) lane_b[(c) % NS_SLOTS]
  constexpr int C1 = NCH0;
  constexpr int CP = NCH0 + 2;
  f32x4 acc[8];
  if constexpr (NPB == 0) {
    NS_STEP(0);
    if (probe) lb_range_probe(a.ctrl, va, 2 * NPA);
#pragma unroll
    for (int mb = 0; mb < 8; ++mb) acc[mb] = vecp[4 * mb];
    lb_gemm16v<false, NPA>(NS_BUF(0), va, acc);
  } else {
    f32x4 h0[4], h1[4];
    NS_STEP(0);
    if (probe) lb_range_probe(a.ctrl, va, 8);
#pragma unroll
    for (int mb = 0; mb < 8; ++mb) acc[mb] = vecp[4 * mb];
    {
      const f32x4 v01[4] = {va[0], va[1], va[2], va[3]};
      lb_gemm16v<false, 2>(NS_BUF(0), v01, acc);
    }
    NS_STEP(1);
    lb_load_agg_half<0>(a, rowc, g, k0, k1, h0);
    NS_REFILL(1);
    {
      const f32x4 v23[4] = {va[4], va[5], va[6], va[7]};
      lb_gemm16v<false, 2>(NS_BUF(1), v23, acc);
    }
    NS_STEP(2);
    lb_load_agg_half<4>(a, rowc, g, k0, k1, h1);
    NS_REFILL(2);
    lb_gemm16v<false, 2>(NS_BUF(2), h0, acc);
    NS_STEP(3);
    NS_REFILL(3);
    if (probe) {
      lb_range_probe(a.ctrl, h0, 4);
      lb_range_probe(a.ctrl, h1, 4);
    }
    lb_gemm16v<false, 2>(NS_BUF(3), h1, acc);
  }
  if (probe) lb_range_probe(a.ctrl, acc, 8);
  f32x4 acc2[8];
  NS_STEP(C1);
  NS_REFILL(C1);
#pragma unroll
  for (int mb = 0; mb < 8; ++mb) acc2[mb] = vecp[32 + 4 * mb];
  {
    const f32x4 v01[4] = {acc[0], acc[1], acc[2], acc[3]};
    uint32_t or_h = 0;
    lb_gemm16v<true, 2, 1>(NS_BUF(C1), v01, acc2, &or_h);
    if (lb_rows_tiny(or_h) && lane == 0) lb_raise_math(a.ctrl, LB_MATH_TINY);
  }
  NS_STEP(C1 + 1);
  f32x4 res[8];
  if constexpr (RESID) {
    const f32x4* xr = reinterpret_cast<const f32x4*>(a.xin) + rowc * 32 + g;
#pragma unroll
    for (int mb = 0; mb < 4; ++mb) res[mb] = xr[4 * mb];
  }
  NS_REFILL(C1 + 1);
  {
    const f32x4 v23[4] = {acc[4], acc[5], acc[6], acc[7]};
    lb_gemm16v<true, 2>(NS_BUF(C1 + 1), v23, acc2);
  }
  if constexpr (RESID) {
    const f32x4* xr = reinterpret_cast<const f32x4*>(a.xin) + rowc * 32 + g;
#pragma unroll
    for (int mb = 4; mb < 8; ++mb) res[mb] = xr[4 * mb];
  }
  f32x4 y[8];
  lb_layernorm16(acc2, vecp + 64, vecp + 96, y, a.ctrl->ln_inv_d, a.ctrl->ln_pad);
  if constexpr (RESID) {
#pragma unroll
    for (int mb = 0; mb < 8; ++mb) y[mb] = lb_pk_add(res[mb], y[mb]);
  }
  if (probe) lb_range_probe(a.ctrl, y, 8);
  if (valid) {
    f32x4* nr = reinterpret_cast<f32x4*>(a.nlat) + row * 32 + g;
#pragma unroll
    for (int mb = 0; mb < 8; ++mb) nr[4 * mb] = y[mb];
  }
  if constexpr (PROJ) {
    {
      f32x4 accp[8];
      NS_STEP(CP);
      NS_REFILL(CP);
#pragma unroll
      for (int mb = 0; mb < 8; ++mb) accp[mb] = vecp[128 + 4 * mb];
      {
        const f32x4 v01[4] = {y[0], y[1], y[2], y[3]};
        lb_gemm16v<false, 2>(NS_BUF(CP), v01, accp);
      }
      NS_STEP(CP + 1);
      NS_REFILL(CP + 1);
      {
        const f32x4 v23[4] = {y[4], y[5], y[6], y[7]};
        lb_gemm16v<false, 2>(NS_BUF(CP + 1), v23, accp);
      }
      if (valid) {
        f32x4* pr = reinterpret_cast<f32x4*>(a.psr) + row * 64 + g;
#pragma unroll
        for (int mb = 0; mb < 8; ++mb) pr[4 * mb] = accp[mb];
      }
    }
    {
      f32x4 accp[8];
      NS_STEP(CP + 2);
      NS_REFILL(CP + 2);
#pragma unroll
      for (int mb = 0; mb < 8; ++mb) accp[mb] = vecp[128 + 32 + 4 * mb];
      {
        const f32x4 v01[4] = {y[0], y[1], y[2], y[3]};
        lb_gemm16v<false, 2>(NS_BUF(CP + 2), v01, accp);
      }
      NS_STEP(CP + 3);
      NS_REFILL(CP + 3);
      {
        const f32x4 v23[4] = {y[4], y[5], y[6], y[7]};
        lb_gemm16v<false, 2>(NS_BUF(CP + 3), v23, accp);
      }
      if (valid) {
        f32x4* pr = reinterpret_cast<f32x4*>(a.psr) + row * 64 + 32 + g;
#pragma unroll
        for (int mb = 0; mb < 8; ++mb) pr[4 * mb] = accp[mb];
      }
    }
  }
#undef NS_BUF
}
#undef NS_STEP
#undef NS_REFILL


int lbk_node16s(lb_engine* e, const lb_node_args& a, const float* w0h, const float* w1h, const float* wph2,
                int npa, int npb, bool resid) {
  const f32x4* w0 = reinterpret_cast<const f32x4*>(w0h);
  const f32x4* w1 = reinterpret_cast<const f32x4*>(w1h);
  const f32x4* wp = reinterpret_cast<const f32x4*>(wph2);
  const bool proj = wph2 != nullptr;
  const int64_t tiles = (a.n_rows + 15) / 16;
  const int nw = tiles < 8 * 256 ? 4 : 8;
  const int nblk = (int)((tiles + nw - 1) / nw);
  dim3 grid(nblk), block(nw * 64);
#define LB_NS(A, B, R, P, W, S) \
  LB_LAUNCH_TIMED(e, (k_node16s<A, B, R, P, W, S>), grid, block, a, w0, w1, wp)
#define LB_NS_W(A, B, R, P)            \
  do {                                 \
    if (nw == 8)                       \
      LB_NS(A, B, R, P, 8, 2);         \
    else                               \
      LB_NS(A, B, R, P, 4, 2);         \
  } while (0)
#define LB_NS_P(A, B, R)               \
  do {                                 \
    if (proj)                          \
      LB_NS_W(A, B, R, true);          \
    else                               \
      LB_NS_W(A, B, R, false);         \
  } while (0)
  if (npa == 4 && npb == 4 && resid)
    LB_NS_P(4, 4, true);
  else if (npa == 1 && npb == 0 && !resid)
    LB_NS_P(1, 0, false);
  else if (npa == 2 && npb == 0 && !resid)
    LB_NS_P(2, 0, false);
  else if (npa == 3 && npb == 0 && !resid)
    LB_NS_P(3, 0, false);
  else if (npa == 4 && npb == 0 && !resid)
    LB_NS_P(4, 0, false);
  else
    return lb_fail(LB_ERR_UNSUPPORTED, "k_node16s<%d,%d,%d> not instantiated", npa, npb, (int)resid);
  LB_HIP(hipGetLastError());
  return LB_OK;
}
```

Before: 21.71 million.

## Pre-centre second-layer weights so LayerNorm skips the mean pass

Row-centres the second linear layer's weights and bias on the host and scales them by 64. The GEMM output is then already zero-mean, so the LayerNorm in the edge, edge-encoder and node fp16 kernels drops the mean reduction and subtraction and computes only the variance, with epsilon rescaled to match. It also moves the p0 add after the first GEMM and simplifies the buffer-store offset. It changes weight packing, adds a host image export entry point, and risks fp16 precision differences from the scaled, centred weights.

```diff
diff --git a/include/lbhip.h b/include/lbhip.h
--- a/include/lbhip.h
+++ b/include/lbhip.h
@@ -141,6 +141,9 @@
 int lb_gns_image_read(lb_gns* g, void* out_host, int64_t n_bytes);
 int64_t lb_gns_pack_selftest(const lb_gns_desc* desc, int32_t node_in_kq, const float* weights_host, int64_t n_floats,
                              int64_t* n_bytes_out);
+
+int64_t lb_gns_pack_host_image(const lb_gns_desc* desc, const float* weights_host, int64_t n_floats, int32_t mlp,
+                               int32_t field, float* out, int64_t cap_floats);
 
 typedef struct lb_segnn lb_segnn;
 
diff --git a/lagrangebench_amd/_lib.py b/lagrangebench_amd/_lib.py
--- a/lagrangebench_amd/_lib.py
+++ b/lagrangebench_amd/_lib.py
@@ -140,6 +140,8 @@
     "lb_gns_image_bytes": (C.c_int64, [_P]),
     "lb_gns_image_read": (C.c_int, [_P, _P, C.c_int64]),
     "lb_gns_pack_selftest": (C.c_int64, [C.POINTER(GnsDesc), C.c_int32, C.POINTER(C.c_float), C.c_int64, C.POINTER(C.c_int64)]),
+    "lb_gns_pack_host_image": (C.c_int64, [C.POINTER(GnsDesc), C.POINTER(C.c_float), C.c_int64, C.c_int32, C.c_int32,
+                                           C.POINTER(C.c_float), C.c_int64]),
     "lb_segnn_train_create": (C.c_int, [_P, C.POINTER(SegnnDesc), C.POINTER(C.c_float), C.c_int64, C.POINTER(_P)]),
     "lb_segnn_train_loss_grad": (C.c_int, [_P, _P, C.c_float, C.POINTER(C.c_double), _P]),
     "lb_segment_sum": (C.c_int, [_P, _P, _P, C.c_int32]),
diff --git a/lagrangebench_amd/csrc/lb_edge16.hip b/lagrangebench_amd/csrc/lb_edge16.hip
--- a/lagrangebench_amd/csrc/lb_edge16.hip
+++ b/lagrangebench_amd/csrc/lb_edge16.hip
@@ -261,7 +261,8 @@
       }
     vs += __shfl_xor(vs, 16);
     vs += __shfl_xor(vs, 32);
-    const float rs = 1.0f / sqrtf(fmaxf(vs - a.ctrl->ln_pad * (mean * mean), 0.f) * a.ctrl->ln_inv_d + 1e-5f);
+    const float eps = F16 ? LB_LNC_EPS : 1e-5f;
+    const float rs = 1.0f / sqrtf(fmaxf(vs - a.ctrl->ln_pad * (mean * mean), 0.f) * a.ctrl->ln_inv_d + eps);
     f32x4 y[8];
 #pragma unroll
     for (int mb = 0; mb < 8; ++mb) {
diff --git a/lagrangebench_amd/csrc/lb_edge16v.hip b/lagrangebench_amd/csrc/lb_edge16v.hip
--- a/lagrangebench_amd/csrc/lb_edge16v.hip
+++ b/lagrangebench_amd/csrc/lb_edge16v.hip
@@ -10,7 +10,7 @@
   __shared__ int s_ticket;
   const int poisoned = a.ctrl->overflow_step;
   const int E = a.ctrl->n_edges_total;
-  const float ln_inv_d = a.ctrl->ln_inv_d, ln_pad = a.ctrl->ln_pad;
+  const float ln_inv_d = a.ctrl->ln_inv_d;
   const int tid = threadIdx.x;
   constexpr int NST = (NW0 + 4096 + THREADS - 1) / THREADS;
   f32x4 st[NST];
@@ -77,13 +77,12 @@
       if (lane == 0) k = atomicAdd(&s_ticket, 1);
       t_next = t_lo + __builtin_amdgcn_readfirstlane(k) * stride;
     }
-    f32x4 acc[8], ve[8];
+    f32x4 acc[8], ve[8], p0[8];
     const int r_cur = r_c;
     const f32x4* er = reinterpret_cast<const f32x4*>(a.elat) + (int64_t)t * 512 + lane;
     {
       const f32x4* ps = psr4 + (int64_t)s_c * 64 + g;
       const f32x4* pr = psr4 + (int64_t)r_c * 64 + 32 + g;
-      f32x4 p0[8];
 #pragma unroll
       for (int mb = 0; mb < 8; ++mb) {
         ve[mb] = (ABL & 2) ? f32x4{1.f, 2.f, (float)(t & 1023), (float)mb}
@@ -94,14 +93,14 @@
       const int64_t rn = rowc_of(min(t_next, t_last));
       s_c = a.senders[rn];
       r_c = a.receivers[rn];
-#pragma unroll
-      for (int mb = 0; mb < 8; ++mb) acc[mb] = lb_pk_add(acc[mb], p0[mb]);
     }
     int rb = lb_edge_probe(a.receivers, t, lane, E);
     if (it == 0) lb_range_probe(a.ctrl, ve, 8);
     if constexpr (PRIO) __builtin_amdgcn_s_setprio(2);
     uint32_t or_e = 0, or_h = 0;
     if constexpr (!(ABL & 8)) lb_gemm16v<false, 4, GUARD>(w0b, ve, acc, &or_e);
+#pragma unroll
+    for (int mb = 0; mb < 8; ++mb) acc[mb] = lb_pk_add(acc[mb], p0[mb]);
     if (it == 0) lb_range_probe(a.ctrl, acc, 8);
     f32x4 acc2[8];
 #pragma unroll
@@ -123,7 +122,7 @@
     }
     asm volatile("" : "+v"(s_c), "+v"(r_c), "+v"(rb));
     f32x4 y[8];
-    lb_layernorm16<!(ABL & 16)>(acc2, vecb + 32, vecb + 64, y, ln_inv_d, ln_pad);
+    lb_layernorm16<!(ABL & 16), true>(acc2, vecb + 32, vecb + 64, y, ln_inv_d);
     const int row = t * 16 + n;
     const bool valid = row < E;
     if constexpr (!SKIP && !(ABL & 4)) {
@@ -185,7 +184,7 @@
   }
   if (poisoned >= 0) return;
   __syncthreads();
-  const float ln_inv_d = a.ctrl->ln_inv_d, ln_pad = a.ctrl->ln_pad;
+  const float ln_inv_d = a.ctrl->ln_inv_d;
   const int ntiles = (E + 15) >> 4;
   const int lane = tid & 63, wave = __builtin_amdgcn_readfirstlane(tid >> 6);
   const int n = lane & 15, g = lane >> 4;
@@ -220,7 +219,7 @@
     lb_gemm16v<true>(w1b, acc, acc2);
     asm volatile("" : "+v"(f_n));
     f32x4 y[8];
-    lb_layernorm16<true>(acc2, vecb + 32, vecb + 64, y, ln_inv_d, ln_pad);
+    lb_layernorm16<true, true>(acc2, vecb + 32, vecb + 64, y, ln_inv_d);
     f32x4* ew = reinterpret_cast<f32x4*>(a.elat) + (int64_t)t * 512 + lane;
 #pragma unroll
     for (int mb = 0; mb < 8; ++mb) __builtin_nontemporal_store(y[mb], &ew[64 * mb]);
diff --git a/lagrangebench_amd/csrc/lb_edge16w.hip b/lagrangebench_amd/csrc/lb_edge16w.hip
--- a/lagrangebench_amd/csrc/lb_edge16w.hip
+++ b/lagrangebench_amd/csrc/lb_edge16w.hip
@@ -24,7 +24,7 @@
 
 struct ew_ctx {
   lds_cptr vecb;
-  float ln_inv_d, ln_pad;
+  float ln_inv_d;
   int E, n, g, lane;
   float* elat_out;
   __amdgpu_buffer_rsrc_t out_rs;
@@ -32,8 +32,8 @@
 };
 
 struct ew_tmp {
-  f32x2v tmp, s2, v2, m2, r2, dl, dh, tlo, thi, ylo, olo, ohi;
-  float sm, mean, vs, rs;
+  f32x2v v2, r2, tlo, thi, ylo, olo, ohi;
+  float vs, rs;
   f32x4 scn, ofn, scc, ofc;
   int rr, segstart;
   bool valid, head, tail;
@@ -62,13 +62,6 @@
   return a + b;
 #endif
 }
-__device__ __forceinline__ f32x2v ew_sub2(f32x2v a, f32x2v b) {
-#if EW_SCALAR_LN
-  return f32x2v{a[0] - b[0], a[1] - b[1]};
-#else
-  return a - b;
-#endif
-}
 __device__ __forceinline__ f32x2v ew_mul2(f32x2v a, f32x2v b) {
 #if EW_SCALAR_LN
   return f32x2v{a[0] * b[0], a[1] * b[1]};
@@ -85,10 +78,8 @@
 }
 template <bool SKIP, int GUARD>
 struct ew_plan {
-  static constexpr int A0 = 0;
-  static constexpr int A1 = A0 + 16;
-  static constexpr int B0 = A1 + 3;
-  static constexpr int B1 = B0 + 32;
+  static constexpr int B0 = 0;
+  static constexpr int B1 = B0 + 16;
   static constexpr int C0 = B1 + 3;
   static constexpr int D0 = C0 + 48;
   static constexpr int E0 = D0 + (SKIP ? 0 : 25);
@@ -108,34 +99,12 @@
 template <bool SKIP, bool NT, int GUARD, bool PIPE = true>
 __device__ __forceinline__ void ew_op(int k, ew_tile& P, ew_tmp& T, const ew_ctx& C, int& guard_tiny) {
   using PL = ew_plan<SKIP, GUARD>;
-  if (k < PL::A1) {
+  if (k < PL::B1) {
     const int mb = k >> 1;
     if (!(k & 1))
-      T.tmp = ew_add2(lb_lo2(P.a[mb]), lb_hi2(P.a[mb]));
+      T.v2 = mb == 0 ? ew_mul2(lb_lo2(P.a[mb]), lb_lo2(P.a[mb])) : ew_fma2(lb_lo2(P.a[mb]), lb_lo2(P.a[mb]), T.v2);
     else
-      T.s2 = mb == 0 ? T.tmp : ew_add2(T.s2, T.tmp);
-  } else if (k < PL::B0) {
-    const int j = k - PL::A1;
-    if (j == 0)
-      T.sm = T.s2[0] + T.s2[1];
-    else if (j == 1)
-      T.sm = ew_rowsum4(T.sm);
-    else {
-      T.mean = T.sm * C.ln_inv_d;
-      T.m2 = f32x2v{T.mean, T.mean};
-    }
-  } else if (k < PL::B1) {
-    const int j = k - PL::B0, mb = j >> 2, sub = j & 3;
-    if (sub == 0)
-      T.dl = ew_sub2(lb_lo2(P.a[mb]), T.m2);
-    else if (sub == 1)
-      T.dh = ew_sub2(lb_hi2(P.a[mb]), T.m2);
-    else if (sub == 2)
-      T.v2 = mb == 0 ? ew_mul2(T.dl, T.dl) : ew_fma2(T.dl, T.dl, T.v2);
-    else {
-      T.v2 = ew_fma2(T.dh, T.dh, T.v2);
-      P.a[mb] = lb_cat2(T.dl, T.dh);
-    }
+      T.v2 = ew_fma2(lb_hi2(P.a[mb]), lb_hi2(P.a[mb]), T.v2);
   } else if (k < PL::C0) {
     const int j = k - PL::B1;
     if (j == 0) {
@@ -145,7 +114,7 @@
       T.vs = ew_rowsum4(T.vs);
       if constexpr (PIPE) T.ofn = C.vecb[64];
     } else {
-      T.rs = 1.0f / sqrtf(fmaxf(T.vs - C.ln_pad * (T.mean * T.mean), 0.f) * C.ln_inv_d + 1e-5f);
+      T.rs = 1.0f / sqrtf(T.vs * C.ln_inv_d + LB_LNC_EPS);
       T.r2 = f32x2v{T.rs, T.rs};
     }
   } else if (k < PL::D0) {
@@ -232,7 +201,7 @@
       T.off = (T.tail && T.valid) ? row_off + (uint32_t)C.g * 16u : 0x80000000u;
     } else {
       const int mb = j - 1;
-      __builtin_amdgcn_raw_buffer_store_b128(__builtin_bit_cast(u32x4w, P.a[mb]), C.out_rs, (int)T.off, 64 * mb, 0);
+      __builtin_amdgcn_raw_buffer_store_b128(__builtin_bit_cast(u32x4w, P.a[mb]), C.out_rs, (int)(T.off + 64u * (uint32_t)mb), 0, 0);
     }
   } else if (GUARD != 0 && k < PL::M) {
     guard_tiny |= (int)lb_rows_tiny(P.or_e) | (int)lb_rows_tiny(P.or_h);
@@ -333,7 +302,7 @@
   __shared__ int s_ticket;
   const int poisoned = a.ctrl->overflow_step;
   const int E = a.ctrl->n_edges_total;
-  const float ln_inv_d = a.ctrl->ln_inv_d, ln_pad = a.ctrl->ln_pad;
+  const float ln_inv_d = a.ctrl->ln_inv_d;
   const int tid = threadIdx.x;
   constexpr int NST = (NW0 + 4096 + THREADS - 1) / THREADS;
   f32x4 st[NST];
@@ -401,7 +370,6 @@
   ew_ctx C;
   C.vecb = vecb;
   C.ln_inv_d = ln_inv_d;
-  C.ln_pad = ln_pad;
   C.E = E;
   C.n = n;
   C.g = g;
diff --git a/lagrangebench_amd/csrc/lb_f16x2.h b/lagrangebench_amd/csrc/lb_f16x2.h
--- a/lagrangebench_amd/csrc/lb_f16x2.h
+++ b/lagrangebench_amd/csrc/lb_f16x2.h
@@ -1,5 +1,6 @@
 #pragma once
 #include "lb_device.h"
+#include "lb_gns_repack.h"
 
 typedef _Float16 h8 __attribute__((ext_vector_type(8)));
 typedef _Float16 h2_t __attribute__((ext_vector_type(2)));
@@ -264,12 +265,33 @@
   }
 }
 
-template <bool ENABLE = true>
+template <bool ENABLE = true, bool CENTRED = false>
 __device__ __forceinline__ void lb_layernorm16(f32x4 (&pre)[8], lds_cptr lns, lds_cptr lno, f32x4 (&y)[8],
                                                float inv_d = 1.0f / 128.0f, float pad = 0.f) {
   if constexpr (!ENABLE) {
 #pragma unroll
     for (int mb = 0; mb < 8; ++mb) y[mb] = pre[mb];
+    return;
+  }
+  if constexpr (CENTRED) {
+    f32x2v v2 = {0.f, 0.f};
+#pragma unroll
+    for (int mb = 0; mb < 8; ++mb) {
+      const f32x2v dl = lb_lo2(pre[mb]), dh = lb_hi2(pre[mb]);
+      v2 = __builtin_elementwise_fma(dl, dl, v2);
+      v2 = __builtin_elementwise_fma(dh, dh, v2);
+    }
+    float vs = v2[0] + v2[1];
+    vs += __shfl_xor(vs, 16);
+    vs += __shfl_xor(vs, 32);
+    const float rs = 1.0f / sqrtf(vs * inv_d + LB_LNC_EPS);
+    const f32x2v r2 = {rs, rs};
+#pragma unroll
+    for (int mb = 0; mb < 8; ++mb) {
+      const f32x4 sc = lns[4 * mb], of = lno[4 * mb];
+      y[mb] = lb_cat2(__builtin_elementwise_fma(lb_lo2(sc) * r2, lb_lo2(pre[mb]), lb_lo2(of)),
+                      __builtin_elementwise_fma(lb_hi2(sc) * r2, lb_hi2(pre[mb]), lb_hi2(of)));
+    }
     return;
   }
   f32x2v s2 = {0.f, 0.f};
diff --git a/lagrangebench_amd/csrc/lb_gns.hip b/lagrangebench_amd/csrc/lb_gns.hip
--- a/lagrangebench_amd/csrc/lb_gns.hip
+++ b/lagrangebench_amd/csrc/lb_gns.hip
@@ -356,6 +356,7 @@
       }
       return lbk_node_ms(e, m, kq / 4, with_agg, resid, proj, dec);
     }
+    if (e->f16x2) a.b1 = w.b1c;
     if (e->f16x2)
       return lbk_node16s(e, a, w.w0_16h, w.w1_16h, proj ? g->proc_edge[next].proj_w_h2 : nullptr, kq / 4, with_agg ? 4 : 0,
                          resid);
@@ -398,7 +399,7 @@
     b.w0p = e->f16x2 ? g->enc_edge.w0_16h : g->enc_edge.w0_16;
     b.b0 = g->enc_edge.b0;
     b.w1p = e->f16x2 ? g->enc_edge.w1_16h : g->enc_edge.w1_16;
-    b.b1 = g->enc_edge.b1;
+    b.b1 = e->f16x2 ? g->enc_edge.b1c : g->enc_edge.b1;
     b.ln_s = g->enc_edge.ln_s;
     b.ln_o = g->enc_edge.ln_o;
     rc = e->f16x2 ? lbk_edge_enc16v(e, b) : lbk_edge16(e, b, false, false);
@@ -436,7 +437,7 @@
       b.psr = e->psr;
       b.w0p = e->f16x2 ? pe.w0_16h : pe.w0_16;
       b.w1p = e->f16x2 ? pe.w1_16h : pe.w1_16;
-      b.b1 = pe.b1;
+      b.b1 = e->f16x2 ? pe.b1c : pe.b1;
       b.ln_s = pe.ln_s;
       b.ln_o = pe.ln_o;
       b.fused = e->fused_agg;
diff --git a/lagrangebench_amd/csrc/lb_gns_repack.h b/lagrangebench_amd/csrc/lb_gns_repack.h
--- a/lagrangebench_amd/csrc/lb_gns_repack.h
+++ b/lagrangebench_amd/csrc/lb_gns_repack.h
@@ -74,11 +74,13 @@
   int32_t perm;
   int32_t at;
   int32_t scaled;
+  int32_t centred;
   int32_t n_ent;
   int32_t piece0, n_pieces;
 };
 struct lb_pack_red {
   int32_t piece0, n_pieces;
+  int32_t centred;
 };
 struct lb_pack_block {
   int32_t job, ent0;
@@ -87,7 +89,7 @@
   std::vector<lb_pack_job> jobs;
   std::vector<lb_pack_piece> pieces;
   std::vector<lb_pack_red> rms;
-  lb_pack_red head{0, 0};
+  lb_pack_red head{0, 0, 0};
   std::vector<lb_pack_block> blocks;
   int64_t blob_floats = 0;
   int64_t src_floats = 0;
@@ -107,6 +109,18 @@
     if (r >= 0 && r < p.rows && c >= 0 && c < p.cols) return w[p.off + (int64_t)r * p.stride + c];
   }
   return 0.f;
+}
+
+#define LB_LNC_SHIFT 6
+#define LB_LNC_SCALE 64.0f
+#define LB_LNC_EPS (1e-5f * 4096.0f)
+LB_HD static inline float lb_pack_centre(float x, double sum, int M) {
+  return (float)((double)x - sum / (double)M) * LB_LNC_SCALE;
+}
+LB_HD static inline double lb_pack_row_sum(const lb_pack_job& j, const lb_pack_piece* pc, const float* w, int k) {
+  double s = 0;
+  for (int c = 0; c < j.M; ++c) s += (double)lb_pack_src(j, pc, w, k, c);
+  return s;
 }
 
 LB_HD static inline void lb_pack_entry(const lb_pack_job& j, const lb_pack_piece* pc, const float* w, float scale, int ent,
@@ -117,9 +131,12 @@
     return j.scaled ? x * scale : x;
   };
   if (j.kind == LB_PK_VEC) {
+    const double sum = j.centred ? lb_pack_row_sum(j, pc, w, 0) : 0.0;
     for (int i = 0; i < 4; ++i) {
       const int c = 4 * ent + i - j.at;
-      out[i] = __builtin_bit_cast(uint32_t, (c >= 0 && c < j.M) ? src(0, c) : 0.f);
+      float x = (c >= 0 && c < j.M) ? src(0, c) : 0.f;
+      if (j.centred && c >= 0 && c < j.M) x = lb_pack_centre(x, sum, j.M);
+      out[i] = __builtin_bit_cast(uint32_t, x);
     }
     return;
   }
@@ -149,7 +166,8 @@
   uint16_t h[8];
   for (int i = 0; i < 8; ++i) {
     const int k = perm ? 32 * kb + 16 * (i >> 2) + 4 * g + (i & 3) : 32 * kb + 8 * g + i;
-    const float x = src(k, m);
+    float x = src(k, m);
+    if (j.centred && k < j.K && m < j.M) x = lb_pack_centre(x, lb_pack_row_sum(j, pc, w, k), j.M);
     const uint16_t hi = lb_f32_to_f16_rne(x);
     h[i] = part ? lb_f32_to_f16_rne(x - lb_f16_to_f32(hi)) : hi;
   }
@@ -174,7 +192,13 @@
     const lb_pack_piece& p = pc[r.piece0 + i];
     const int cnt = p.rows * p.cols;
     for (int q = lane; q < cnt; q += LB_PACK_LANES) {
-      const float x = w[p.off + (int64_t)(q / p.cols) * p.stride + (q % p.cols)];
+      const float* row = w + p.off + (int64_t)(q / p.cols) * p.stride;
+      float x = row[q % p.cols];
+      if (r.centred) {
+        double sum = 0;
+        for (int c = 0; c < p.cols; ++c) sum += (double)row[c];
+        x = lb_pack_centre(x, sum, p.cols);
+      }
       s += (double)x * x;
       n += x != 0.f;
       const uint32_t a = __builtin_bit_cast(uint32_t, x) & 0x7fffffffu;
diff --git a/lagrangebench_amd/csrc/lb_gns_weights.hip b/lagrangebench_amd/csrc/lb_gns_weights.hip
--- a/lagrangebench_amd/csrc/lb_gns_weights.hip
+++ b/lagrangebench_amd/csrc/lb_gns_weights.hip
@@ -76,8 +76,9 @@
   std::vector<lb_src_piece> pc;
   int K = 0, M = 0;
   bool scaled = false;
-};
-static lb_src lb_src_plain(const float* w, int K, int M) { return {{{w, 0, K, M, 0, M}}, K, M, false}; }
+  bool centred = false;
+};
+static lb_src lb_src_plain(const float* w, int K, int M) { return {{{w, 0, K, M, 0, M}}, K, M, false, false}; }
 static lb_src lb_src_padded(const lb_lin_view& l) {
   lb_src s;
   s.K = l.blocks * LB_D;
@@ -138,10 +139,19 @@
     j.perm = perm;
     j.at = at;
     j.scaled = s.scaled;
+    j.centred = s.centred;
     j.n_ent = (int32_t)((floats + 3) / 4);
     j.piece0 = (int32_t)rec->pieces.size();
     j.n_pieces = rec_pieces(s.pc);
     rec->jobs.push_back(j);
+  }
+  static void centre_rows(float* w, int K, int M) {
+    for (int k = 0; k < K; ++k) {
+      float* row = w + (size_t)k * M;
+      double sum = 0;
+      for (int m = 0; m < M; ++m) sum += (double)row[m];
+      for (int m = 0; m < M; ++m) row[m] = lb_pack_centre(row[m], sum, M);
+    }
   }
   std::vector<float> dense(const lb_src& s) const {
     std::vector<float> o((size_t)s.K * s.M, 0.f);
@@ -150,15 +160,20 @@
         memcpy(&o[(size_t)(p.row0 + r) * s.M + p.col0], p.w + (size_t)r * p.stride, sizeof(float) * p.cols);
     if (s.scaled)
       for (float& x : o) x = std::ldexp(x, sh);
+    if (s.centred) centre_rows(o.data(), s.K, s.M);
     return o;
   }
 
-  void vec(const float** field, size_t count, const float* src = nullptr, size_t n_src = 0, size_t at = 0) {
+  void vec(const float** field, size_t count, const float* src = nullptr, size_t n_src = 0, size_t at = 0, bool centred = false) {
     const size_t off = next(field, count);
-    if (rec)
-      rec_job(off, LB_PK_VEC, src ? lb_src_plain(src, 1, (int)n_src) : lb_src(), 1, (int)count, 0, false, (int)at, count);
-    else if (src)
+    if (rec) {
+      lb_src s = src ? lb_src_plain(src, 1, (int)n_src) : lb_src();
+      s.centred = centred;
+      rec_job(off, LB_PK_VEC, s, 1, (int)count, 0, false, (int)at, count);
+    } else if (src) {
       memcpy(host.data() + off + at, src, n_src * sizeof(float));
+      if (centred) centre_rows(host.data() + off + at, 1, (int)n_src);
+    }
   }
   void img(const float** field, int kind, const lb_src& s, int Kp, int Mp) {
     const size_t off = next(field, (size_t)Kp * Mp);
@@ -186,27 +201,34 @@
       off += kept;
     }
   }
-  void note_rms(const lb_lin_view& l) {
+  void note_rms(const lb_lin_view& l, bool centred = false) {
     if (rec) {
       std::vector<lb_src_piece> pc;
       for (int b = 0; b < l.blocks; ++b) pc.push_back({l.block(b), 0, l.rows, l.out, 0, l.out});
       const int32_t p0 = (int32_t)rec->pieces.size();
-      rec->rms.push_back({p0, rec_pieces(pc)});
+      rec->rms.push_back({p0, rec_pieces(pc), (int32_t)centred});
       return;
     }
     const size_t cnt = (size_t)l.blocks * l.rows * l.out;
+    std::vector<float> wc;
+    const float* lw = l.w;
+    if (centred) {
+      wc.assign(l.w, l.w + cnt);
+      centre_rows(wc.data(), l.blocks * l.rows, l.out);
+      lw = wc.data();
+    }
     double s2 = 0;
     size_t nz = 0;
     for (size_t i = 0; i < cnt; ++i) {
-      s2 += (double)l.w[i] * l.w[i];
-      nz += l.w[i] != 0.f;
+      s2 += (double)lw[i] * lw[i];
+      nz += lw[i] != 0.f;
     }
     if (nz) w_rms_min = std::min(w_rms_min, std::sqrt(s2 / (double)nz));
   }
   void head_shift(const lb_lin_view& l) {
     if (rec) {
       const int32_t p0 = (int32_t)rec->pieces.size();
-      rec->head = {p0, rec_pieces({{l.w, 0, l.rows, l.out, 0, l.out}})};
+      rec->head = {p0, rec_pieces({{l.w, 0, l.rows, l.out, 0, l.out}}), 0};
       return;
     }
     float mx = 0.f;
@@ -228,10 +250,16 @@
   auto p16 = [&](const float** f, const lb_src& s, int Kp) { st.img(f, LB_PK_P16, s, Kp, 128); };
   auto p16h = [&](const float** f, const lb_src& s, int Kp, int Mp = 128) { st.img(f, LB_PK_P16H, s, Kp, Mp); };
   auto lin = [&](const lb_lin_view& l, int b = 0) { return lb_src_plain(l.block(b), l.rows, l.out); };
+  auto lin_c = [&](const lb_lin_view& l) {
+    lb_src s = lin(l);
+    s.centred = true;
+    return s;
+  };
   auto vecs = [&](lb_mlp_w& m, const lb_mlp_view& s, bool b0, int b1_pad = LB_D) {
     if (b0) st.vec(&m.b0, D, s.lin[0].b, dl);
     st.vec(&m.b1, b1_pad, s.lin[1].b, s.lin[1].out);
     if (s.ln_s) {
+      st.vec(&m.b1c, D, s.lin[1].b, dl, 0, true);
       st.vec(&m.ln_s, D, s.ln_s, dl);
       st.vec(&m.ln_o, D, s.ln_o, dl);
     }
@@ -254,10 +282,11 @@
     lb_mlp_w& m = g->enc_edge;
     st.note_rms(l0);
     st.note_rms(l1);
+    st.note_rms(l1, true);
     p16(&m.w0_16, lin(l0), 16);
     p16h(&m.w0_16h, lin(l0), 32);
     p16(&m.w1_16, lin(l1), D);
-    p16h(&m.w1_16h, lin(l1), D);
+    p16h(&m.w1_16h, lin_c(l1), D);
     vecs(m, v.enc_edge, true);
     st.ms(&m.ms, {{lin(l0), 1, 1, false, 0}, {lin(l1), 4, 1, true, 0}});
   }
@@ -266,10 +295,11 @@
     const lb_lin_view& l1 = s.lin[1];
     st.note_rms(s.lin[0]);
     st.note_rms(l1);
+    st.note_rms(l1, true);
     p32(&m.w0, w0, K0p, D);
     p16h(&m.w0_16h, w0, K0p);
     p32(&m.w1, lin(l1), D, D);
-    p16h(&m.w1_16h, lin(l1), D);
+    p16h(&m.w1_16h, lin_c(l1), D);
     vecs(m, s, true);
     ms.insert(ms.begin(), {{w0, K0p / 32, 1, true, 0}, {lin(l1), 4, 1, true, 0}});
     st.ms(&m.ms, ms);
@@ -292,7 +322,7 @@
       p16(&m.w0_16, lin(l0, 2), D);
       p16h(&m.w0_16h, lin(l0, 2), D);
       p16(&m.w1_16, lin(l1), D);
-      p16h(&m.w1_16h, lin(l1), D);
+      p16h(&m.w1_16h, lin_c(l1), D);
       vecs(m, v.proc_edge[k], false);
       st.ms(&m.ms, {{lin(l0, 2), 4, 1, true, 0}, {lin(l1), 4, 1, true, 0}});
     }
@@ -499,6 +529,38 @@
   return diff;
 }
 
+extern "C" int64_t lb_gns_pack_host_image(const lb_gns_desc* d, const float* w, int64_t n_floats, int32_t mlp, int32_t field,
+                                          float* out, int64_t cap_floats) {
+  if (!d || !w || !out) return lb_fail(LB_ERR_ARG, "null argument");
+  LB_TRY(lb_gns_check_desc(d, nullptr));
+  if (d->blocks_per_step != 2) return lb_fail(LB_ERR_UNSUPPORTED, "lb_gns_pack_host_image: num_mlp_layers 2 only");
+  lb_gns_view v;
+  LB_TRY(lb_gns_walk(d, w, n_floats, &v));
+  lb_gns g{};
+  lb_gns_init(&g, d, nullptr, 0);
+  lb_stage st;
+  lb_gns_stage_all(st, v, &g);
+  for (const auto& f : st.fix) *f.first = st.host.data() + f.second;
+  const int L = d->num_mp_steps;
+  if (mlp < 0 || mlp >= 3 + 2 * L) return lb_fail(LB_ERR_ARG, "mlp %d out of range", (int)mlp);
+  const bool dec = mlp == 2;
+  const lb_mlp_w& m = mlp == 0 ? g.enc_node : mlp == 1 ? g.enc_edge : dec ? g.dec
+                      : (mlp - 3) % 2 == 0 ? g.proc_edge[(size_t)(mlp - 3) / 2] : g.proc_node[(size_t)(mlp - 3) / 2];
+  const float* src = nullptr;
+  int64_t n = 0;
+  switch (field) {
+    case 0: src = m.w1_16h; n = dec ? LB_D * 16 : LB_D * LB_D; break;
+    case 1: src = m.b1; n = dec ? 32 : LB_D; break;
+    case 2: src = m.b1c; n = LB_D; break;
+    case 3: src = dec ? m.w0_16h : nullptr; n = LB_D * LB_D; break;
+    default: return lb_fail(LB_ERR_ARG, "field %d out of range", (int)field);
+  }
+  if (!src) return 0;
+  if (n > cap_floats) return lb_fail(LB_ERR_ARG, "image of %lld floats, room for %lld", (long long)n, (long long)cap_floats);
+  memcpy(out, src, (size_t)n * sizeof(float));
+  return n;
+}
+
 extern "C" int64_t lb_gns_image_bytes(lb_gns* g) { return g ? g->blob_floats * (int64_t)sizeof(float) : -1; }
 extern "C" int lb_gns_image_read(lb_gns* g, void* out_host, int64_t n_bytes) {
   if (!g || !out_host || n_bytes != g->blob_floats * (int64_t)sizeof(float)) return lb_fail(LB_ERR_ARG, "bad argument");
diff --git a/lagrangebench_amd/csrc/lb_internal.h b/lagrangebench_amd/csrc/lb_internal.h
--- a/lagrangebench_amd/csrc/lb_internal.h
+++ b/lagrangebench_amd/csrc/lb_internal.h
@@ -204,6 +204,7 @@
 struct lb_mlp_w {
   const float* b0;
   const float* b1;
+  const float* b1c;
   const float* ln_s;
   const float* ln_o;
   const float* w0;
diff --git a/lagrangebench_amd/csrc/lb_node16s.hip b/lagrangebench_amd/csrc/lb_node16s.hip
--- a/lagrangebench_amd/csrc/lb_node16s.hip
+++ b/lagrangebench_amd/csrc/lb_node16s.hip
@@ -190,7 +190,7 @@
     for (int mb = 4; mb < 8; ++mb) res[mb] = xr[4 * mb];
   }
   f32x4 y[8];
-  lb_layernorm16(acc2, vecp + 64, vecp + 96, y, a.ctrl->ln_inv_d, a.ctrl->ln_pad);
+  lb_layernorm16<true, true>(acc2, vecp + 64, vecp + 96, y, a.ctrl->ln_inv_d);
   if constexpr (RESID) {
 #pragma unroll
     for (int mb = 0; mb < 8; ++mb) y[mb] = lb_pk_add(res[mb], y[mb]);
```

Measured after the change: 21.90 million, median of 6. About the same (+0.8%).
